# dasongli1/Shift-Net

Hardware: AMD Instinct MI355X
Metric: restored frames/sec at 1280x720 T=16 bf16 (higher is better)
Workload: dtype bf16; 1 GPU; Shift-Net-s (gshift_deblur2), 1280x720, one_len=16 (T_in=20), one window per GPU, synthetic checkpoint; parallelism=clip-parallel x1, gsts_schedule=unit-major, one stream

## Files before the change

include/shiftnet_hip.h:

```cpp
#ifndef SHIFTNET_HIP_H
#define SHIFTNET_HIP_H
#include <stdint.h>

#ifdef __cplusplus
extern "C" {
#endif

#define SN_ABI_VERSION 20

#define SN_F32 0
#define SN_F16 1
#define SN_BF16 2

int sn_abi_version(void);

int sn_selftest_mfma(const float* a, const float* b, float* d, void* stream);

int sn_ingest(const void* src, int src_dtype, const void* noise, void* dst, int T, int C, int H, int W, void* stream);

typedef struct sn_conv_desc {
    const void* in[3];
    int n_in;
    int cs_in;
    int T, h_in, w_in;
    int in_mode;
    int k, stride, pad;
    int h_out, w_out;
    const void* wfrag;
    int mt, ks;
    const float* bias;
    int act;
    float prelu;
    const void* res;
    void* out;
    int cs_out;
    int out_mode;
    int c_out;
    int nchw_dtype;
    const void* sc;
    int sc_dtype;
    float* pool;
    const float* oscale;
    int oscale_stride;
    const void* res2;
    int flags;
    int clip_n, clip_T, clip_lo;
} sn_conv_desc;
#define SN_CONV_TILE_KERNEL 1
int sn_conv2d(const sn_conv_desc* d, void* stream);
int sn_conv_pool_blocks(const sn_conv_desc* d);
#define SN_CONV_K_GENERIC 1
#define SN_CONV_K_FAST    2
#define SN_CONV_K_STATS   3
#define SN_CONV_K_STREAM  4
#define SN_CONV_ROUTE(kernel, mt, a, d, mode, rl) (((kernel) << 24) | ((mt) << 20) | ((a) << 12) | ((d) << 8) | ((mode) << 4) | (rl))
int sn_conv2d_route(const sn_conv_desc* d, int lines_len, int ncu, int* plan);

int sn_upsample2_add(const void* lo, const void* res, void* out, int T, int hs, int ws, int cs, void* stream);

int sn_ca_mlp(const float* partial, int nblk, int cpad, int c, int cr, float inv_hw,
              const float* wa, const float* wb, float* ca, int T, unsigned* bad, void* stream);

int sn_cab_ca_scratch_floats(int T);
int sn_cab_ca(const float* partial, int nblk, int cpad, const void* mid, int cs, int c, int cr, int h, int w,
              const float* w2, const float* wa, const float* wb, float* scratch, float* ca, int T, void* stream);
int sn_cab_fused_supported(const sn_conv_desc* conv1, const sn_conv_desc* conv2);
int sn_cab_stats(const sn_conv_desc* conv1, int lines_len, void* stream);
int sn_cab_ca_lines(const float* partial, int nblk, int cpad, const void* lines, int lines_len, int cs, int c, int cr, int h, int w,
                    const float* w2, const float* wa, const float* wb, float* scratch, float* ca, int T, void* stream);
int sn_cab_fused(const sn_conv_desc* conv1, const sn_conv_desc* conv2, int tile_rows, void* stream);

int sn32_cab_ca(const float* partial, int nblk, int cpad, const float* mid, int c, int cr, int h, int w,
                const float* w2, const float* wa, const float* wb, float* scratch, float* ca, int T, void* stream);

typedef struct sn_unit_src {
    const void* x;
    int T, h, w, C;
    int mode;
    int wrap;
    const void* halo;
    int t0, nt;
    int clip;
} sn_unit_src;

int sn_gsts_gather(const sn_unit_src* s, const int8_t* offs, void* u, void* stream);

int sn_temporal_roll(const sn_unit_src* s, void* y, void* stream);

int sn_gsts_shiftconv(const sn_unit_src* s, const int8_t* offs, const uint32_t* w1, void* hw, void* stream);
int sn_gsts_shiftconv_mfma(const sn_unit_src* s, const int8_t* offs, const uint32_t* w1, void* hw, void* stream);

int sn_ln_gemm_gate(const sn_unit_src* s, const void* hw, const void* wfrag, const float* bias, const uint32_t* wdw,
                    void* g1, float* pool, int g1_blocked, void* stream);
int sn_lngate_blocks(int h, int w);

int sn_grp5_gemm_gate(const void* g1, const float* ca_in, const void* wgrp, const void* wfrag, void* g2, float* pool,
                      int T, int h, int w, int C, void* stream);
int sn_grp5_blocks(int h, int w);

int sn_planar_pitch(int w);
int sn_nhwc_to_planar(const void* x, void* xp, int T, int h, int w, int C, void* stream);

int sn_dw5m_blocks(int h, int w);
int sn_dw5m_gemm_gate(const void* g1p, const float* ca_in, const void* ttab, const void* wfrag, void* g2, float* pool,
                      int T, int h, int w, int C, void* stream);

typedef struct sn_phase1_weights {
    const void* wfrag1;
    const uint32_t* w3;
    const void* wgrp;
    const void* wfrag2;
} sn_phase1_weights;
typedef struct sn_se_fold {
    const float* wa;
    const float* wb;
    int c, cr;
    unsigned* ticket;
    float* ca;
    unsigned* bad;
} sn_se_fold;
typedef struct sn_phase1_opts {
    const float* g1_scale;
    int g1_sums;
    int team;
    void* g1_store;
} sn_phase1_opts;
int sn_phase1_pool_blocks(int T, int h, int w);
int sn_phase1_g1_store_bytes(int T, int h, int w, int C, long long* bytes);
int sn_gsts_cab2_phase1(const sn_unit_src* s, const void* hw, const sn_phase1_weights* wt, void* g2, float* pool, const sn_se_fold* se,
                        const sn_phase1_opts* opt, void* stream);
int sn_cab1_phase1(const sn_unit_src* s, const sn_phase1_weights* wt, void* g2, float* pool, const sn_se_fold* se, const sn_phase1_opts* opt, void* stream);
int sn_p1r_plan(int nfr, int h, int w, int ncu, int team, int* out7);
int sn_p1r_strip_begin(const int* plan7, int s, int w);

int sn_gsts_cab2_phase2(const sn_unit_src* s, const void* g2, const float* ca, const void* wfrag, const float* bias, void* y, void* stream);
int sn_cab1_phase2(const sn_unit_src* s, const void* g2, const float* ca, const void* wfrag, const float* bias, void* y, void* stream);

int sn_cab2_phase2_cab1_phase1_supported(const sn_unit_src* s);
int sn_cab2_phase2_cab1_phase1(const sn_unit_src* s, const void* g2_in, const float* ca, const void* wfrag, const float* bias, void* y,
                               const sn_phase1_weights* wt, void* g2, float* pool, const sn_se_fold* se, const sn_phase1_opts* opt, void* stream);


typedef struct sn32_conv_desc {
    const float* in[3];
    int c_in[3];
    int cs_in[3];
    int n_in;
    int T, h_in, w_in;
    int in_mode;
    int k, stride, pad, groups;
    int h_out, w_out, c_out;
    const float* w;
    const float* bias;
    int act; float prelu;
    const float* oscale; int oscale_stride;
    const float* res; int cs_res;
    void* out; int cs_out;
    int out_mode;
    int nchw_dtype; const void* sc;
    const void* wsplit;
    const float* iscale; int iscale_stride;
    const float* rscale; int rscale_stride;
    const float* ln_w; const float* ln_b;
    float* csum; int csum_cpad;
    int clip_n, clip_T, clip_lo;
} sn32_conv_desc;
int sn32_conv_csum_tiles(int h_out, int w_out);
int sn32_conv2d(const sn32_conv_desc* d, void* stream);
#define SN32_K_1X1      1
#define SN32_K_SPLIT    2
#define SN32_K_SPLIT_G8 3
#define SN32_K_EXACT    4
#define SN32_K_DW       5
#define SN32_K_DIRECT   6
#define SN32_ROUTE(kernel, a, b) (((kernel) << 16) | ((a) << 8) | (b))
int sn32_conv2d_route(const sn32_conv_desc* d);
int sn32_gsts_gather(const sn_unit_src* s, const int8_t* offs, float* u, float* u2, void* stream);
int sn32_gsts_shiftconv(const sn_unit_src* s, const int8_t* offs, const float* w, float* vin, float* u, void* stream);
int sn32_layernorm(const float* x, int cs_x, int K, const float* w, const float* b, float* out, int cs_out, long long npix, void* stream);
int sn32_gate(const float* a, int C, int mode, float* out, long long npix, void* stream);
int sn32_gate_sum(const float* a, int C, int cpad, int mode, float* out, int T, int hw, int nblk, float* partial, void* stream);
int sn32_conv1x1_gate2(const float* x, int cs_x, int cin, const void* wsplit, int C, int cpad, float* out, int T, int hw, float* partial, void* stream);
int sn32_dw_gate(const float* a, int cs_a, const float* w, int C, int cpad, float* out, int T, int h, int wd, int nblk, float* partial, void* stream);
int sn32_chan_sum(const float* x, int cs, int C, int cpad, int T, int hw, int nblk, float* partial, void* stream);
int sn32_scale_residual(const float* r, const float* x, const float* ca, int ca_stride, float* out, int T, int hw, int C, void* stream);
int sn32_ingest(const void* src, int src_dtype, const void* noise, float* dst, int T, int C, int H, int W, void* stream);


int sn_ingest_u8(const uint8_t* src, void* dst, int dst_dtype, int T, int H, int W, void* stream);
int sn_egress_blocks(void);
int sn_egress_u8(const void* out, int out_dtype, const uint8_t* gt, uint8_t* img, float* sse, int T, int H, int W, void* stream);
int sn_ssim_blocks(void);
int sn_ssim_u8(const void* out, int out_dtype, const uint8_t* gt, float* scratch, float* partial, int T, int H, int W, void* stream);

#define SN_YUV_444 0
#define SN_YUV_420_CENTER 1
#define SN_YUV_420_LEFT 2
#define SN_YUV_BT601 0
#define SN_YUV_BT709 1
#define SN_YUV_LIMITED 0
#define SN_YUV_FULL 1
typedef struct sn_yuv_fmt {
    int bits;
    int chroma;
    int matrix;
    int range;
} sn_yuv_fmt;
int sn_ingest_yuv(const uint8_t* src, const sn_yuv_fmt* fmt, void* dst, int dst_dtype, int T, int H, int W, int Hp, int Wp, void* stream);
int sn_egress_yuv(const void* out, int out_dtype, const sn_yuv_fmt* fmt, uint8_t* dst, int T, int H, int W, int Hp, int Wp, void* stream);

int sn_yuv_thumb(const uint8_t* src, const sn_yuv_fmt* fmt, uint16_t* dst, int T, int H, int W, void* stream);

int sn_yuv_noise_hist(const uint8_t* src, const sn_yuv_fmt* fmt, uint32_t* dst, int lo, int hi, int T, int H, int W, void* stream);

#ifdef __cplusplus
}
#endif
#endif
```

shift-net_amd/csrc/sn_common.h:

```cpp
#pragma once
#include <hip/hip_runtime.h>
#include <hip/hip_fp16.h>
#include <stdint.h>

typedef __bf16 bf16x8_t __attribute__((ext_vector_type(8)));
typedef __bf16 bf16x2_t __attribute__((ext_vector_type(2)));
typedef float f32x4_t __attribute__((ext_vector_type(4)));
typedef float f32x2_t __attribute__((ext_vector_type(2)));
typedef uint16_t bf16_t;

#define SN_OK 0
#define SN_EINVAL (-22)
#define SN_ELAUNCH (-5)

__device__ __forceinline__ float bf_lo(uint32_t u) { return __uint_as_float(u << 16); }
__device__ __forceinline__ float bf_hi(uint32_t u) { return __uint_as_float(u & 0xffff0000u); }
__device__ __forceinline__ float bf_to_f(bf16_t h) { return __uint_as_float(((uint32_t)h) << 16); }

__device__ __forceinline__ uint32_t pack_bf2(float lo, float hi) {
    f32x2_t v = {lo, hi};
    bf16x2_t h = __builtin_convertvector(v, bf16x2_t);
    return __builtin_bit_cast(uint32_t, h);
}
typedef _Float16 h2_t __attribute__((ext_vector_type(2)));
__device__ __forceinline__ uint32_t pack_h2(float lo, float hi) {
    const h2_t h = {(_Float16)lo, (_Float16)hi};
    return __builtin_bit_cast(uint32_t, h);
}
__device__ __forceinline__ bf16_t f_to_bf(float f) { return (bf16_t)(pack_bf2(f, 0.f) & 0xffffu); }

__device__ __forceinline__ void unpack8(const uint4 q, float* v) {
    v[0] = bf_lo(q.x); v[1] = bf_hi(q.x); v[2] = bf_lo(q.y); v[3] = bf_hi(q.y);
    v[4] = bf_lo(q.z); v[5] = bf_hi(q.z); v[6] = bf_lo(q.w); v[7] = bf_hi(q.w);
}
__device__ __forceinline__ uint4 pack8(const float* v) {
    uint4 q;
    q.x = pack_bf2(v[0], v[1]); q.y = pack_bf2(v[2], v[3]); q.z = pack_bf2(v[4], v[5]); q.w = pack_bf2(v[6], v[7]);
    return q;
}
__device__ __forceinline__ bf16x8_t as_frag(const uint4 q) { return __builtin_bit_cast(bf16x8_t, q); }

__device__ __forceinline__ f32x4_t mfma16(const bf16x8_t a, const bf16x8_t b, const f32x4_t c) {
    return __builtin_amdgcn_mfma_f32_16x16x32_bf16(a, b, c, 0, 0, 0);
}

__device__ __forceinline__ float dot2bf(uint32_t a, uint32_t b, float acc) {
    return __builtin_amdgcn_fdot2_f32_bf16(__builtin_bit_cast(bf16x2_t, a), __builtin_bit_cast(bf16x2_t, b), acc, false);
}

__device__ __forceinline__ float sigmoidf_(float x) { return __builtin_amdgcn_rcpf(1.0f + __expf(-x)); }

template <int CTRL> __device__ __forceinline__ float dpp_mov(float x) {
    return __builtin_bit_cast(float, __builtin_amdgcn_update_dpp(0, __builtin_bit_cast(int, x), CTRL, 0xf, 0xf, true));
}
template <int CTRL> __device__ __forceinline__ int dpp_movi(int x) { return __builtin_amdgcn_update_dpp(0, x, CTRL, 0xf, 0xf, true); }
__device__ __forceinline__ float row_sum16(float x) {
    x += dpp_mov<0xB1>(x);
    x += dpp_mov<0x4E>(x);
    x += dpp_mov<0x141>(x);
    x += dpp_mov<0x140>(x);
    return x;
}

__device__ __forceinline__ float sum_rows4(float x) {
    float a = x, b = x;
    asm volatile("s_nop 1\n\tv_permlane16_swap_b32 %0, %1" : "+v"(a), "+v"(b));
    const float s = a + b;
    float c = s, d = s;
    asm volatile("s_nop 1\n\tv_permlane32_swap_b32 %0, %1" : "+v"(c), "+v"(d));
    return c + d;
}

#define SN_FRAME_RANGE(s, T0, NT) const int T0 = (s)->nt > 0 ? (s)->t0 : 0, NT = (s)->nt > 0 ? (s)->nt : (s)->T; \
    if (T0 < 0 || NT < 1 || T0 + NT > (s)->T || !sn_clip_ok((s)->T, (s)->clip, (s)->wrap)) return SN_EINVAL
static inline bool sn_clip_ok(int T, int clip, int wrap) { return clip == 0 || (clip > 0 && T % clip == 0 && wrap != 2); }
static inline int sn_clip_len(int T, int clip) { return clip > 0 ? clip : T; }
template <typename E> struct SnSlabs { const E* p0; const E* p1; const E* pb; int s0, s1, sb; };
template <typename E>
__device__ __forceinline__ SnSlabs<E> sn_unit_slabs(const E* x, const E* halo, int T, int hw, int C, int mode, int wrap, int clip, int t) {
    if (clip < T) {
        const int base = t / clip * clip;
        x += (ptrdiff_t)base * hw * C; t -= base; T = clip;
    }
    const int Ch = C >> 1;
    const E* xt = x + (ptrdiff_t)t * hw * C;
    SnSlabs<E> s;
    s.p0 = xt; s.p1 = xt + Ch; s.pb = xt; s.s0 = s.s1 = s.sb = C;
    if (mode == 1) {
        if (t > 0 || wrap == 1) { s.p0 = x + (ptrdiff_t)(t > 0 ? t - 1 : T - 1) * hw * C + Ch; s.p1 = xt; s.pb = s.p0; }
        else if (wrap == 2) { s.p0 = halo; s.s0 = Ch; s.p1 = xt; s.pb = halo; s.sb = Ch; }
        else s.pb = xt;
    } else if (mode == 2) {
        if (t < T - 1 || wrap == 1) { s.p0 = xt + Ch; s.p1 = x + (ptrdiff_t)(t < T - 1 ? t + 1 : 0) * hw * C; s.pb = s.p1; }
        else if (wrap == 2) { s.p0 = xt + Ch; s.p1 = halo; s.s1 = Ch; s.pb = halo; s.sb = Ch; }
        else s.pb = xt + Ch;
    }
    return s;
}

__host__ __device__ __forceinline__ int sn_remap_frame(int t, int n, int T, int lo) {
    if (n == 0) return t;
    const int q = t / n;
    return q * T + lo + (t - q * n);
}
static inline bool sn_remap_set(int n, int T, int lo) { return n != 0 || T != 0 || lo != 0; }
static inline bool sn_remap_ok(int Tout, int n, int T, int lo) { return !sn_remap_set(n, T, lo) || (n > 0 && lo >= 0 && lo + n <= T && Tout % n == 0); }

struct SeFold { const float* wa; const float* wb; float* ca; unsigned* ticket; unsigned* bad; float inv_hw; int c, cr; };
__device__ __forceinline__ void sn_flag_nonfinite(unsigned* bad, float v) {
    if (bad && !(fabsf(v) <= 3.0e38f)) __hip_atomic_store(bad, 1u, __ATOMIC_RELAXED, __HIP_MEMORY_SCOPE_AGENT);
}
__device__ __forceinline__ void sn_pool_store(float* p, float v) { __hip_atomic_store(p, v, __ATOMIC_RELAXED, __HIP_MEMORY_SCOPE_AGENT); }
__device__ __forceinline__ void sn_se_tail(const SeFold& S, const float* pool_t, int nblk, int narrive, int cpad, int t, float* lds, int tid, int nthreads) {
    asm volatile("s_waitcnt vmcnt(0)" ::: "memory");
    __syncthreads();
    unsigned* flag = (unsigned*)lds;
    if (tid == 0) *flag = __hip_atomic_fetch_add(S.ticket + t, 1u, __ATOMIC_RELAXED, __HIP_MEMORY_SCOPE_AGENT) == (unsigned)(narrive - 1) ? 1u : 0u;
    __syncthreads();
    if (!*flag) return;
    if (tid == 0) {
        __builtin_amdgcn_fence(__ATOMIC_ACQUIRE, "agent");
        __hip_atomic_store(S.ticket + t, 0u, __ATOMIC_RELAXED, __HIP_MEMORY_SCOPE_AGENT);
    }
    __syncthreads();
    const int nq = cpad >> 2, parts = nthreads / nq, cq = tid % nq, part = tid / nq;
    float* acc = lds + 16; float* mean = acc + parts * cpad; float* hid = mean + 128;
    if (part < parts) {
        float s0 = 0.f, s1 = 0.f, s2 = 0.f, s3 = 0.f;
#pragma unroll 4
        for (int b = part; b < nblk; b += parts) {
            const float* r = pool_t + (size_t)b * cpad + 4 * cq;
            s0 += __hip_atomic_load(r, __ATOMIC_RELAXED, __HIP_MEMORY_SCOPE_AGENT);
            s1 += __hip_atomic_load(r + 1, __ATOMIC_RELAXED, __HIP_MEMORY_SCOPE_AGENT);
            s2 += __hip_atomic_load(r + 2, __ATOMIC_RELAXED, __HIP_MEMORY_SCOPE_AGENT);
            s3 += __hip_atomic_load(r + 3, __ATOMIC_RELAXED, __HIP_MEMORY_SCOPE_AGENT);
        }
        float* a = acc + part * cpad + 4 * cq;
        a[0] = s0; a[1] = s1; a[2] = s2; a[3] = s3;
    }
    __syncthreads();
    if (tid < cpad) {
        float m = 0.f;
        for (int q = 0; q < parts; ++q) m += acc[q * cpad + tid];
        sn_flag_nonfinite(S.bad, m);
        mean[tid] = m * S.inv_hw;
    }
    __syncthreads();
    if (tid < S.cr) {
        float hsum = 0.f;
        for (int j = 0; j < S.c; ++j) hsum += S.wa[tid * S.c + j] * mean[j];
        hid[tid] = hsum > 0.f ? hsum : 0.f;
    }
    __syncthreads();
    if (tid < cpad) {
        float o = 0.f;
        if (tid < S.c) {
            for (int j = 0; j < S.cr; ++j) o += S.wb[tid * S.cr + j] * hid[j];
            o = sigmoidf_(o);
        }
        S.ca[(size_t)t * cpad + tid] = o;
    }
}

__device__ __forceinline__ int wave_id() { return __builtin_amdgcn_readfirstlane((int)(threadIdx.x >> 6)); }

#ifndef SN_XCD_TILES
#define SN_XCD_TILES 1
#endif
struct XcdTiles { int ntx, nty, nrf, chunk; uint32_t inv_nty; };
static inline XcdTiles sn_xcd_tiles(int ntx, int nty, int T) {
    XcdTiles g; g.ntx = ntx; g.nty = nty; g.nrf = nty * T;
    g.chunk = SN_XCD_TILES ? (g.nrf + 7) / 8 : g.nrf;
    g.inv_nty = nty > 1 ? (uint32_t)((0x100000000ull + (uint32_t)nty - 1) / (uint32_t)nty) : 0u;
    return g;
}
static inline dim3 sn_xcd_grid(const XcdTiles& g) { return SN_XCD_TILES ? dim3(8u * g.ntx, g.chunk, 1) : dim3(g.ntx, g.nrf, 1); }
__host__ __device__ inline bool sn_xcd_decode(const XcdTiles& g, uint32_t bx, uint32_t by, int& t, int& ty, int& tx) {
#if SN_XCD_TILES
    tx = (int)(bx >> 3);
    const uint32_t rf = (bx & 7) * (uint32_t)g.chunk + by;
#else
    tx = (int)bx;
    const uint32_t rf = by;
#endif
    if (rf >= (uint32_t)g.nrf) return false;
    t = g.inv_nty ? (int)(((uint64_t)rf * g.inv_nty) >> 32) : (int)rf;
    ty = (int)rf - t * g.nty;
    return true;
}
__device__ __forceinline__ bool sn_xcd_tile(const XcdTiles& g, int& t, int& ty, int& tx) {
    return sn_xcd_decode(g, blockIdx.x, blockIdx.y, t, ty, tx);
}

static inline void sn_clear_error() { (void)hipGetLastError(); }
static inline int sn_check_launch() {
    hipError_t e = hipGetLastError();
    return e == hipSuccess ? SN_OK : SN_ELAUNCH;
}
```

shift-net_amd/csrc/sn_conv.hip:

```cpp
#include "sn_common.h"
#include "../../include/shiftnet_hip.h"

int sn_conv3p_key(const sn_conv_desc* d, bool want_pool);
int sn_conv3p_pool_rows(const sn_conv_desc* d);
int sn_conv3p_route(const sn_conv_desc* d, int lines_len, int ncu, int* plan8);
int sn_conv3p_launch(const sn_conv_desc* d, int lines_len, int route, const int* plan8, void* stream);

namespace {

struct ConvK {
    const bf16_t* in0; const bf16_t* in1; const bf16_t* in2;
    int n_in, cs, cv;
    int hin, win, in_mode, k, stride, pad, hout, wout;
    const uint4* wfrag; int ks;
    const float* bias; int act; float prelu;
    const bf16_t* res; bf16_t* out; int cs_out, out_mode, c_out, nchw_dtype, sc_dtype;
    const void* sc; float* pool; const float* oscale; int oscale_stride; const bf16_t* res2;
    int rh, rw, ps;
    int clip_n, clip_T, clip_lo;
    int lines_len;
    XcdTiles xg;
    unsigned m_nblk8, m_rw, m_csb, m_cv, m_k;
};

constexpr __host__ __device__ int sn_lds_slots(int npb) {
    const int k = npb <= 2 ? 2 : 4 * ((npb - 2 + 3) / 4) + 2;
    return k <= npb + 1 ? k : ((npb & 1) ? npb : npb + 1);
}

__device__ __forceinline__ int fdiv(int x, unsigned magic) { return (int)(((unsigned)x * (unsigned long long)magic) >> 24); }

__device__ __forceinline__ uint4 ld_bilinear(const bf16_t* src, int t, int hs, int ws, int cs, int cb, int gy, int gx) {
    float sy = gy * 0.5f - 0.25f; if (sy < 0.f) sy = 0.f;
    float sx = gx * 0.5f - 0.25f; if (sx < 0.f) sx = 0.f;
    int y0 = (int)sy, x0 = (int)sx;
    int y1 = min(y0 + 1, hs - 1), x1 = min(x0 + 1, ws - 1);
    float ly = sy - y0, lx = sx - x0, hy = 1.f - ly, hx = 1.f - lx;
    const bf16_t* b = src + (size_t)t * hs * ws * cs + cb * 8;
    float v00[8], v01[8], v10[8], v11[8], o[8];
    unpack8(*(const uint4*)(b + ((size_t)y0 * ws + x0) * cs), v00);
    unpack8(*(const uint4*)(b + ((size_t)y0 * ws + x1) * cs), v01);
    unpack8(*(const uint4*)(b + ((size_t)y1 * ws + x0) * cs), v10);
    unpack8(*(const uint4*)(b + ((size_t)y1 * ws + x1) * cs), v11);
#pragma unroll
    for (int j = 0; j < 8; ++j) o[j] = hy * (hx * v00[j] + lx * v01[j]) + ly * (hx * v10[j] + lx * v11[j]);
    return pack8(o);
}

constexpr int sn_conv_waves(int mt) {
    return mt == 1 ? 6 : mt == 2 ? 5 : mt == 3 ? 4 : mt == 4 ? 3 : 2;
}
constexpr int sn_conv3_waves(int mt, int cs) {
    return mt == 1 ? 7 : mt == 2 ? 6 : mt == 3 ? (cs == 48 ? 3 : 4) : mt == 4 ? 3 : 2;
}

template <int MT, int TH, int TW>
__global__ __launch_bounds__(256, sn_conv_waves(MT)) void conv_mfma_kernel(const ConvK P) {
    extern __shared__ __attribute__((aligned(16))) char smem[];
    constexpr int NTW = (TH * TW) / 64;
    constexpr int XB = TW / 16;
    const int tid = threadIdx.x, lane = tid & 63, wv = wave_id();
    const int g = lane >> 4, p = lane & 15;
    int t, tyi, txi;
    if (!sn_xcd_tile(P.xg, t, tyi, txi)) return;
    const int ti = sn_remap_frame(t, P.clip_n, P.clip_T, P.clip_lo);
    const int oy0 = tyi * TH, ox0 = txi * TW;
    const int tile_bytes = P.rh * P.rw * P.ps;
    int* tapoff = (int*)(smem + tile_bytes);
    float* red = (float*)(smem + tile_bytes + ((P.ks * 4 * 4 + 15) & ~15));

    for (int e = tid; e < P.ks * 4; e += 256) {
        const int kk0 = e * 8, K = P.k * P.k * P.cv;
        int off = 0;
        if (kk0 < K) {
            const int tap = fdiv(kk0, P.m_cv), cc0 = kk0 - tap * P.cv;
            const int dy = fdiv(tap, P.m_k), dx = tap - dy * P.k;
            off = (dy * P.rw + dx) * P.ps + cc0 * 2;
        }
        tapoff[e] = off;
    }
    {
        const int nblk8 = P.cv >> 3, csb = P.cs >> 3, total = P.rh * P.rw * nblk8;
        const int iy0 = oy0 * P.stride - P.pad, ix0 = ox0 * P.stride - P.pad;
        for (int idx0 = tid; idx0 < total; idx0 += 4 * 256) {
            uint4 v[4];
            int dst[4];
#pragma unroll
            for (int u = 0; u < 4; ++u) {
                const int idx = idx0 + u * 256;
                const int idc = idx < total ? idx : tid;
                const int pix = fdiv(idc, P.m_nblk8), blk = idc - pix * nblk8;
                const int ry = fdiv(pix, P.m_rw), rx = pix - ry * P.rw;
                const int ii = fdiv(blk, P.m_csb), cb = blk - ii * csb;
                const bf16_t* src = ii == 0 ? P.in0 : (ii == 1 ? P.in1 : P.in2);
                const int gy = iy0 + ry, gx = ix0 + rx;
                const bool in = gy >= 0 && gy < P.hin && gx >= 0 && gx < P.win;
                dst[u] = idx < total ? (in ? pix * P.ps + blk * 16 : -(pix * P.ps + blk * 16) - 1) : 0x7fffffff;
                if (P.in_mode == 0) v[u] = *(const uint4*)(src + (in ? (((size_t)ti * P.hin + gy) * P.win + gx) * P.cs + cb * 8 : 0));
                else v[u] = in ? ld_bilinear(src, ti, P.hin >> 1, P.win >> 1, P.cs, cb, gy, gx) : make_uint4(0, 0, 0, 0);
            }
#pragma unroll
            for (int u = 0; u < 4; ++u) {
                if (dst[u] == 0x7fffffff) continue;
                const bool in = dst[u] >= 0;
                *(uint4*)(smem + (in ? dst[u] : -(dst[u] + 1))) = in ? v[u] : make_uint4(0, 0, 0, 0);
            }
        }
    }
    bf16x8_t a_cur[MT];
#pragma unroll
    for (int m = 0; m < MT; ++m) a_cur[m] = as_frag(P.wfrag[(m * P.ks) * 64 + lane]);
    __syncthreads();

    f32x4_t acc[MT][NTW];
#pragma unroll
    for (int m = 0; m < MT; ++m)
#pragma unroll
        for (int n = 0; n < NTW; ++n) acc[m][n] = (f32x4_t){0.f, 0.f, 0.f, 0.f};
    int pixbase[NTW];
#pragma unroll
    for (int n = 0; n < NTW; ++n) {
        const int nn = wv * NTW + n, row = nn / XB, xb = nn - row * XB;
        pixbase[n] = ((row * P.stride) * P.rw + (xb * 16 + p) * P.stride) * P.ps;
    }
    constexpr bool PRE_RES = MT == 1;
    uint2 rres[PRE_RES ? MT : 1][PRE_RES ? NTW : 1];
    if constexpr (PRE_RES) {
        const bf16_t* rb = P.res ? P.res : (const bf16_t*)P.wfrag;
#pragma unroll
        for (int n = 0; n < NTW; ++n) {
            const int nn = wv * NTW + n, row = nn / XB, xb = nn - row * XB;
            const int oy = oy0 + row, ox = ox0 + xb * 16 + p;
            const bool valid = P.res && (oy < P.hout) && (ox < P.wout);
            const size_t opix = ((size_t)t * P.hout + oy) * P.wout + ox;
#pragma unroll
            for (int m = 0; m < MT; ++m) {
                const int co0 = g * 4 * MT + m * 4;
                rres[m][n] = *(const uint2*)(rb + ((valid && co0 < P.cs_out) ? opix * P.cs_out + co0 : 0));
            }
        }
    }
    for (int s = 0; s < P.ks; ++s) {
        const int toff = tapoff[s * 4 + g];
        const int sn = s + 1 < P.ks ? s + 1 : s;
        bf16x8_t a_nxt[MT];
#pragma unroll
        for (int m = 0; m < MT; ++m) a_nxt[m] = as_frag(P.wfrag[(m * P.ks + sn) * 64 + lane]);
        bf16x8_t b[NTW];
#pragma unroll
        for (int n = 0; n < NTW; ++n) b[n] = as_frag(*(const uint4*)(smem + pixbase[n] + toff));
#pragma unroll
        for (int m = 0; m < MT; ++m)
#pragma unroll
            for (int n = 0; n < NTW; ++n) acc[m][n] = mfma16(a_cur[m], b[n], acc[m][n]);
#pragma unroll
        for (int m = 0; m < MT; ++m) a_cur[m] = a_nxt[m];
    }

    float psum[MT][4];
#pragma unroll
    for (int m = 0; m < MT; ++m)
#pragma unroll
        for (int r = 0; r < 4; ++r) psum[m][r] = 0.f;

    float4 bia[MT], osc[MT];
#pragma unroll
    for (int m = 0; m < MT; ++m) {
        const int co0 = g * 4 * MT + m * 4;
        bia[m] = P.bias ? *(const float4*)(P.bias + co0) : make_float4(0.f, 0.f, 0.f, 0.f);
        osc[m] = P.oscale ? *(const float4*)(P.oscale + (size_t)t * P.oscale_stride + co0) : make_float4(1.f, 1.f, 1.f, 1.f);
    }
#pragma unroll
    for (int n = 0; n < NTW; ++n) {
        const int nn = wv * NTW + n, row = nn / XB, xb = nn - row * XB;
        const int oy = oy0 + row, ox = ox0 + xb * 16 + p;
        const bool valid = (oy < P.hout) && (ox < P.wout);
        const size_t opix = ((size_t)t * P.hout + oy) * P.wout + ox;
        uint2 shuf[MT];
#pragma unroll
        for (int m = 0; m < MT; ++m) {
            const int co0 = g * 4 * MT + m * 4;
            float v[4] = {acc[m][n][0], acc[m][n][1], acc[m][n][2], acc[m][n][3]};
            v[0] += bia[m].x; v[1] += bia[m].y; v[2] += bia[m].z; v[3] += bia[m].w;
            if (P.act == 1) {
#pragma unroll
                for (int r = 0; r < 4; ++r) v[r] = v[r] >= 0.f ? v[r] : v[r] * P.prelu;
            }
            v[0] *= osc[m].x; v[1] *= osc[m].y; v[2] *= osc[m].z; v[3] *= osc[m].w;
            if constexpr (PRE_RES) {
                if (P.res && valid && co0 < P.cs_out) {
                    const uint2 rr = rres[m][n];
                    v[0] += bf_lo(rr.x); v[1] += bf_hi(rr.x); v[2] += bf_lo(rr.y); v[3] += bf_hi(rr.y);
                }
            } else if (P.res && valid && co0 < P.cs_out) {
                const uint2 rr = *(const uint2*)(P.res + opix * P.cs_out + co0);
                v[0] += bf_lo(rr.x); v[1] += bf_hi(rr.x); v[2] += bf_lo(rr.y); v[3] += bf_hi(rr.y);
            }
            if (P.res2 && valid && co0 < P.cs_out) {
                const uint2 rr = *(const uint2*)(P.res2 + opix * P.cs_out + co0);
                v[0] += bf_lo(rr.x); v[1] += bf_hi(rr.x); v[2] += bf_lo(rr.y); v[3] += bf_hi(rr.y);
            }
            if (valid) {
#pragma unroll
                for (int r = 0; r < 4; ++r) psum[m][r] += v[r];
                if (P.out_mode == 0) {
                    if (co0 < P.cs_out) {
                        uint2 o; o.x = pack_bf2(v[0], v[1]); o.y = pack_bf2(v[2], v[3]);
                        *(uint2*)(P.out + opix * P.cs_out + co0) = o;
                    }
                } else if (P.out_mode == 1) {
                    shuf[m].x = pack_bf2(v[0], v[1]); shuf[m].y = pack_bf2(v[2], v[3]);
                } else {
#pragma unroll
                    for (int r = 0; r < 4; ++r) {
                        const int co = co0 + r;
                        if (co < P.c_out) {
                            const size_t oi = (((size_t)t * P.c_out + co) * P.hout + oy) * P.wout + ox;
                            const float scv = P.sc_dtype == SN_F32 ? ((const float*)P.sc)[oi]
                                            : (P.sc_dtype == SN_F16 ? __half2float(((const __half*)P.sc)[oi]) : bf_to_f(((const bf16_t*)P.sc)[oi]));
                            if (P.nchw_dtype == SN_F32) ((float*)P.out)[oi] = v[r] + scv;
                            else if (P.nchw_dtype == SN_F16) ((__half*)P.out)[oi] = __float2half(v[r] + scv);
                            else ((bf16_t*)P.out)[oi] = f_to_bf(v[r] + scv);
                        }
                    }
                }
            }
        }
        if (P.out_mode == 1 && valid) {
            bf16_t* dst = P.out + (((size_t)t * 2 * P.hout + 2 * oy + (g >> 1)) * (2 * P.wout) + 2 * ox + (g & 1)) * P.cs_out;
#pragma unroll
            for (int m = 0; m + 1 < MT; m += 2) *(uint4*)(dst + m * 4) = make_uint4(shuf[m].x, shuf[m].y, shuf[m + 1].x, shuf[m + 1].y);
            if constexpr (MT & 1) *(uint2*)(dst + (MT - 1) * 4) = shuf[MT - 1];
        }
    }

    if (P.pool) {
#pragma unroll
        for (int m = 0; m < MT; ++m)
#pragma unroll
            for (int r = 0; r < 4; ++r) {
                float s = psum[m][r];
                s = row_sum16(s);
                if (p == 0) red[wv * 16 * MT + g * 4 * MT + m * 4 + r] = s;
            }
        __syncthreads();
        if (tid < 16 * MT) {
            const float s = red[tid] + red[16 * MT + tid] + red[2 * 16 * MT + tid] + red[3 * 16 * MT + tid];
            const int nblk = P.xg.ntx * P.xg.nty, blk = tyi * P.xg.ntx + txi;
            P.pool[((size_t)t * nblk + blk) * (16 * MT) + tid] = s;
        }
    }
}

template <int MT, int CS, int TH, bool STATS = false>
__global__ __launch_bounds__(256, sn_conv3_waves(MT, CS)) void conv3_fast_kernel(const ConvK P) {
    extern __shared__ __attribute__((aligned(16))) char smem[];
    constexpr int TW = 32, RH = TH + 2, RW = TW + 2, NPB = CS / 8;
    constexpr int PS = 16 * sn_lds_slots(NPB);
    constexpr int KTOT = 9 * CS, KS = (KTOT + 31) / 32;
    constexpr int NTW = (TH * TW) / 64, XB = TW / 16;
    constexpr int ROWP = RW * NPB, NITEM = RH * ROWP, NIT = (NITEM + 255) / 256;
    constexpr int TILE_BYTES = RH * RW * PS;
    const int tid = threadIdx.x & 255, lane = tid & 63, wv = wave_id();
    const int g = lane >> 4, p = lane & 15;
    int t, tyi, txi;
    if (!sn_xcd_tile(P.xg, t, tyi, txi)) return;
    const int oy0 = tyi * TH, ox0 = txi * TW;
    float* red = (float*)(smem + TILE_BYTES);

    {
        const int iy0 = oy0 - 1, ix0 = ox0 - 1;
        const bf16_t* inb = P.in0 + (size_t)t * P.hin * P.win * CS;
        const bool interior = iy0 >= 0 && iy0 + RH <= P.hin && ix0 >= 0 && ix0 + RW <= P.win;
        uint4 v[NIT];
        if (interior) {
#pragma unroll
            for (int k = 0; k < NIT; ++k) {
                const int idx = tid + k * 256, idc = idx < NITEM ? idx : NITEM - 1;
                const int r = idc / ROWP, i = idc - r * ROWP;
                v[k] = *(const uint4*)(inb + ((size_t)iy0 * P.win + ix0) * CS + (size_t)r * P.win * CS + i * 8);
            }
#pragma unroll
            for (int k = 0; k < NIT; ++k) {
                const int idx = tid + k * 256;
                const int r = idx / ROWP, i = idx - r * ROWP, px = i / NPB, blk = i - px * NPB;
                if (idx < NITEM) *(uint4*)(smem + (r * RW + px) * PS + blk * 16) = v[k];
            }
        } else {
            bool in[NIT];
#pragma unroll
            for (int k = 0; k < NIT; ++k) {
                const int idx = tid + k * 256, idc = idx < NITEM ? idx : NITEM - 1;
                const int r = idc / ROWP, i = idc - r * ROWP, px = i / NPB, blk = i - px * NPB;
                const int gy = iy0 + r, gx = ix0 + px;
                in[k] = gy >= 0 && gy < P.hin && gx >= 0 && gx < P.win;
                v[k] = *(const uint4*)(inb + (in[k] ? ((size_t)gy * P.win + gx) * CS + blk * 8 : 0));
            }
#pragma unroll
            for (int k = 0; k < NIT; ++k) {
                const int idx = tid + k * 256;
                const int r = idx / ROWP, i = idx - r * ROWP, px = i / NPB, blk = i - px * NPB;
                if (idx < NITEM) *(uint4*)(smem + (r * RW + px) * PS + blk * 16) = in[k] ? v[k] : make_uint4(0, 0, 0, 0);
            }
        }
    }

    const bool full = (oy0 + TH <= P.hout) && (ox0 + TW <= P.wout);
    const size_t tbase = (((size_t)t * P.hout + oy0) * P.wout + ox0) * P.cs_out;
    bf16_t* const outb = P.out + tbase;
    const bf16_t* const resb = P.res ? P.res + tbase : nullptr;
    const bf16_t* const res2b = P.res2 ? P.res2 + tbase : nullptr;
    const int c0 = g * 4 * MT;
    int loff[NTW];
    bool valid[NTW];
#pragma unroll
    for (int n = 0; n < NTW; ++n) {
        const int nn = wv * NTW + n, row = nn / XB, xb = nn - row * XB;
        loff[n] = (row * P.wout + xb * 16 + p) * P.cs_out + c0;
        valid[n] = full || ((oy0 + row < P.hout) && (ox0 + xb * 16 + p < P.wout));
    }
    constexpr bool PRE_RES = MT == 1;
    uint2 rres[PRE_RES ? NTW : 1];
    if constexpr (PRE_RES) {
        const bf16_t* rb = resb ? resb : (const bf16_t*)P.wfrag;
#pragma unroll
        for (int n = 0; n < NTW; ++n) rres[n] = *(const uint2*)(rb + ((resb && valid[n] && c0 < P.cs_out) ? loff[n] : 0));
    }
    __syncthreads();

    f32x4_t acc[MT][NTW];
#pragma unroll
    for (int m = 0; m < MT; ++m) {
        const float4 b4 = P.bias ? *(const float4*)(P.bias + c0 + m * 4) : make_float4(0.f, 0.f, 0.f, 0.f);
#pragma unroll
        for (int n = 0; n < NTW; ++n) acc[m][n] = (f32x4_t){b4.x, b4.y, b4.z, b4.w};
    }
    int pixbase[NTW];
#pragma unroll
    for (int n = 0; n < NTW; ++n) {
        const int nn = wv * NTW + n, row = nn / XB, xb = nn - row * XB;
        pixbase[n] = (row * RW + xb * 16 + p) * PS;
    }
#pragma unroll
    for (int s = 0; s < KS; ++s) {
        int toff = 0;
#pragma unroll
        for (int gg = 0; gg < 4; ++gg) {
            const int kk0 = (s * 4 + gg) * 8;
            const int tap = kk0 / CS, cc0 = kk0 - tap * CS, dy = tap / 3, dx = tap - dy * 3;
            const int o = kk0 < KTOT ? (dy * RW + dx) * PS + cc0 * 2 : 0;
            toff = g == gg ? o : toff;
        }
        bf16x8_t a[MT];
#pragma unroll
        for (int m = 0; m < MT; ++m) a[m] = as_frag(P.wfrag[(m * KS + s) * 64 + lane]);
        bf16x8_t b[NTW];
#pragma unroll
        for (int n = 0; n < NTW; ++n) b[n] = as_frag(*(const uint4*)(smem + pixbase[n] + toff));
#pragma unroll
        for (int m = 0; m < MT; ++m)
#pragma unroll
            for (int n = 0; n < NTW; ++n) acc[m][n] = mfma16(a[m], b[n], acc[m][n]);
    }

    float psum[MT][4];
#pragma unroll
    for (int m = 0; m < MT; ++m)
#pragma unroll
        for (int r = 0; r < 4; ++r) psum[m][r] = 0.f;
    float4 osc[MT];
    const bool has_osc = P.oscale != nullptr;
#pragma unroll
    for (int m = 0; m < MT; ++m)
        osc[m] = has_osc ? *(const float4*)(P.oscale + (size_t)t * P.oscale_stride + c0 + m * 4) : make_float4(1.f, 1.f, 1.f, 1.f);
    const float slope = P.prelu;
    const int act = P.act != 1 ? 0 : ((slope >= 0.f && slope <= 1.f) ? 1 : 2);
#pragma unroll
    for (int n = 0; n < NTW; ++n) {
        float v[MT][4];
#pragma unroll
        for (int m = 0; m < MT; ++m) {
            v[m][0] = acc[m][n][0]; v[m][1] = acc[m][n][1]; v[m][2] = acc[m][n][2]; v[m][3] = acc[m][n][3];
            if (act == 1) {
#pragma unroll
                for (int r = 0; r < 4; ++r) v[m][r] = fmaxf(v[m][r], slope * v[m][r]);
            } else if (act == 2) {
#pragma unroll
                for (int r = 0; r < 4; ++r) v[m][r] = fmaf(slope, fminf(v[m][r], 0.f), fmaxf(v[m][r], 0.f));
            }
            if (has_osc) { v[m][0] *= osc[m].x; v[m][1] *= osc[m].y; v[m][2] *= osc[m].z; v[m][3] *= osc[m].w; }
        }
        const bool ok = valid[n];
        if constexpr (PRE_RES) {
            if (resb && ok && c0 < P.cs_out) {
                const uint2 rr = rres[n];
                v[0][0] += bf_lo(rr.x); v[0][1] += bf_hi(rr.x); v[0][2] += bf_lo(rr.y); v[0][3] += bf_hi(rr.y);
            }
        }
        if (ok) {
            const bf16_t* rp[2] = {PRE_RES ? nullptr : resb, res2b};
#pragma unroll
            for (int q = 0; q < 2; ++q) {
                if (!rp[q]) continue;
                const bf16_t* src = rp[q] + loff[n];
                if constexpr (MT == 2 || MT == 4) {
#pragma unroll
                    for (int m = 0; m < MT; m += 2) {
                        if (c0 + m * 4 < P.cs_out) {
                            const uint4 rr = *(const uint4*)(src + m * 4);
                            v[m][0] += bf_lo(rr.x); v[m][1] += bf_hi(rr.x); v[m][2] += bf_lo(rr.y); v[m][3] += bf_hi(rr.y);
                            v[m + 1][0] += bf_lo(rr.z); v[m + 1][1] += bf_hi(rr.z); v[m + 1][2] += bf_lo(rr.w); v[m + 1][3] += bf_hi(rr.w);
                        }
                    }
                } else {
#pragma unroll
                    for (int m = 0; m < MT; ++m) {
                        if (c0 + m * 4 < P.cs_out) {
                            const uint2 rr = *(const uint2*)(src + m * 4);
                            v[m][0] += bf_lo(rr.x); v[m][1] += bf_hi(rr.x); v[m][2] += bf_lo(rr.y); v[m][3] += bf_hi(rr.y);
                        }
                    }
                }
            }
            bf16_t* dst = outb + loff[n];
            if (P.pool) {
#pragma unroll
                for (int m = 0; m < MT; ++m)
#pragma unroll
                    for (int r = 0; r < 4; ++r) psum[m][r] += v[m][r];
            }
            if constexpr (STATS) {
                const int nn = wv * NTW + n, row = nn / XB, xb = nn - row * XB;
                const int oy = oy0 + row, ox = ox0 + xb * 16 + p;
                bf16_t* const lb = P.out + (size_t)t * 4 * P.lines_len * P.cs_out + c0;
                bf16_t* tgt[4] = {oy == 0 ? lb + (size_t)ox * P.cs_out : nullptr,
                                  oy == P.hout - 1 ? lb + ((size_t)P.lines_len + ox) * P.cs_out : nullptr,
                                  ox == 0 ? lb + ((size_t)2 * P.lines_len + oy) * P.cs_out : nullptr,
                                  ox == P.wout - 1 ? lb + ((size_t)3 * P.lines_len + oy) * P.cs_out : nullptr};
#pragma unroll
                for (int q = 0; q < 4; ++q) {
                    if (!tgt[q]) continue;
#pragma unroll
                    for (int m = 0; m < MT; ++m)
                        if (c0 + m * 4 < P.cs_out) {
                            uint2 o; o.x = pack_bf2(v[m][0], v[m][1]); o.y = pack_bf2(v[m][2], v[m][3]);
                            *(uint2*)(tgt[q] + m * 4) = o;
                        }
                }
                continue;
            }
            if constexpr (MT == 2 || MT == 4) {
#pragma unroll
                for (int m = 0; m < MT; m += 2)
                    if (c0 + m * 4 < P.cs_out)
                        *(uint4*)(dst + m * 4) = make_uint4(pack_bf2(v[m][0], v[m][1]), pack_bf2(v[m][2], v[m][3]),
                                                            pack_bf2(v[m + 1][0], v[m + 1][1]), pack_bf2(v[m + 1][2], v[m + 1][3]));
            } else {
#pragma unroll
                for (int m = 0; m < MT; ++m)
                    if (c0 + m * 4 < P.cs_out) {
                        uint2 o; o.x = pack_bf2(v[m][0], v[m][1]); o.y = pack_bf2(v[m][2], v[m][3]);
                        *(uint2*)(dst + m * 4) = o;
                    }
            }
        }
    }
    if (P.pool) {
#pragma unroll
        for (int m = 0; m < MT; ++m)
#pragma unroll
            for (int r = 0; r < 4; ++r) {
                float sm = psum[m][r];
                sm = row_sum16(sm);
                if (p == 0) red[wv * 16 * MT + g * 4 * MT + m * 4 + r] = sm;
            }
        __syncthreads();
        if (tid < 16 * MT) {
            const float sm = red[tid] + red[16 * MT + tid] + red[2 * 16 * MT + tid] + red[3 * 16 * MT + tid];
            const int nblk = P.xg.ntx * P.xg.nty, blk = tyi * P.xg.ntx + txi;
            P.pool[((size_t)t * nblk + blk) * (16 * MT) + tid] = sm;
        }
    }
}


template <int MT, int CS, bool STATS = false>
int launch_conv3_fast(const ConvK& K, int T, hipStream_t st) {
    constexpr int TH = 8, TW = 32, NPB = CS / 8, PS = 16 * sn_lds_slots(NPB);
    ConvK P = K; P.xg = sn_xcd_tiles((K.wout + TW - 1) / TW, (K.hout + TH - 1) / TH, T);
    const dim3 grid = sn_xcd_grid(P.xg);
    const size_t lds = (size_t)(TH + 2) * (TW + 2) * PS + 4 * 16 * MT * sizeof(float);
    if (lds > 64 * 1024) {
        if (hipFuncSetAttribute((const void*)conv3_fast_kernel<MT, CS, TH, STATS>, hipFuncAttributeMaxDynamicSharedMemorySize, (int)lds) != hipSuccess)
            return SN_ELAUNCH;
    }
    hipLaunchKernelGGL((conv3_fast_kernel<MT, CS, TH, STATS>), grid, dim3(256), lds, st, P);
    return sn_check_launch();
}

size_t conv_generic_lds(int th, int tw, int stride, int k, int ps, int ks, int mt) {
    return (size_t)((th - 1) * stride + k) * ((tw - 1) * stride + k) * ps + ((ks * 16 + 15) & ~15) + 4 * 16 * mt * sizeof(float);
}

template <int TH, int TW>
int launch_conv(const ConvK& K, int mt, int T, hipStream_t st) {
    const int rh = (TH - 1) * K.stride + K.k, rw = (TW - 1) * K.stride + K.k;
    ConvK P = K; P.rh = rh; P.rw = rw;
    P.xg = sn_xcd_tiles((K.wout + TW - 1) / TW, (K.hout + TH - 1) / TH, T);
    const dim3 grid = sn_xcd_grid(P.xg);
    auto magic = [](int d) { return (unsigned)(((1u << 24) + d - 1) / d); };
    P.m_nblk8 = magic(P.cv >> 3); P.m_rw = magic(rw); P.m_csb = magic(P.cs >> 3); P.m_cv = magic(P.cv); P.m_k = magic(P.k);
    const size_t lds = conv_generic_lds(TH, TW, K.stride, K.k, P.ps, P.ks, mt);
#define SN_CONV_CASE(M) case M: \
        if (lds > 64 * 1024 && hipFuncSetAttribute((const void*)conv_mfma_kernel<M, TH, TW>, hipFuncAttributeMaxDynamicSharedMemorySize, (int)lds) != hipSuccess) return SN_ELAUNCH; \
        hipLaunchKernelGGL((conv_mfma_kernel<M, TH, TW>), grid, dim3(256), lds, st, P); break;
    switch (mt) {
        SN_CONV_CASE(1) SN_CONV_CASE(2) SN_CONV_CASE(3) SN_CONV_CASE(4) SN_CONV_CASE(5) SN_CONV_CASE(6)
        default: return SN_EINVAL;
    }
#undef SN_CONV_CASE
    return sn_check_launch();
}

__global__ void ingest_kernel(const void* src, int dt, const void* noise, uint4* dst, int C, int HW) {
    const int t = blockIdx.y;
    const int i = blockIdx.x * blockDim.x + threadIdx.x;
    if (i >= HW) return;
    float v[8] = {0, 0, 0, 0, 0, 0, 0, 0};
    for (int c = 0; c < C; ++c) {
        const size_t idx = ((size_t)t * C + c) * HW + i;
        v[c] = dt == SN_F32 ? ((const float*)src)[idx] : (dt == SN_F16 ? __half2float(((const __half*)src)[idx]) : bf_to_f(((const bf16_t*)src)[idx]));
    }
    if (noise) {
        const size_t idx = (size_t)t * HW + i;
        v[C] = dt == SN_F32 ? ((const float*)noise)[idx] : (dt == SN_F16 ? __half2float(((const __half*)noise)[idx]) : bf_to_f(((const bf16_t*)noise)[idx]));
    }
    dst[(size_t)t * HW + i] = pack8(v);
}

__global__ __launch_bounds__(1024) void ca_mlp_kernel(const float* partial, int nblk, int cpad, int c, int cr, float inv_hw,
                                                   const float* wa, const float* wb, float* ca, unsigned* bad) {
    __shared__ float acc[1024];
    __shared__ float mean[128];
    __shared__ float hid[128];
    const int t = blockIdx.x, tid = threadIdx.x;
    const int nsplit = 1024 / cpad;
    const int ch = tid % cpad, part = tid / cpad;
    float s = 0.f;
    if (part < nsplit) {
        const float* pp = partial + (size_t)t * nblk * cpad + ch;
        for (int b = part; b < nblk; b += nsplit) s += pp[(size_t)b * cpad];
    }
    acc[tid] = s;
    __syncthreads();
    if (tid < cpad) {
        float m = 0.f;
        for (int q = 0; q < nsplit; ++q) m += acc[q * cpad + tid];
        sn_flag_nonfinite(bad, m);
        mean[tid] = m * inv_hw;
    }
    __syncthreads();
    if (tid < cr) {
        float h = 0.f;
        for (int j = 0; j < c; ++j) h += wa[tid * c + j] * mean[j];
        hid[tid] = h > 0.f ? h : 0.f;
    }
    __syncthreads();
    if (tid < cpad) {
        float o = 0.f;
        if (tid < c) {
            for (int j = 0; j < cr; ++j) o += wb[tid * cr + j] * hid[j];
            o = sigmoidf_(o);
        }
        ca[(size_t)t * cpad + tid] = o;
    }
}

#define SN_CABCA_NS 16
__device__ __forceinline__ float cab_ldf(const bf16_t* p) { return bf_to_f(*p); }
__device__ __forceinline__ float cab_ldf(const float* p) { return *p; }
template <typename E>
__device__ __forceinline__ const E* cab_px(const E* mt, int L, int w, int cs, int line, int y, int x) {
    return L > 0 ? mt + ((size_t)line * L + (line < 2 ? x : y)) * cs : mt + ((size_t)y * w + x) * cs;
}
template <typename E>
__global__ __launch_bounds__(256) void cab_ca_part_kernel(const float* partial, int nblk, int cpad, const E* mid, int cs,
                                                        int h, int w, float* scratch, int L) {
    __shared__ float acc[256];
    const int t = blockIdx.y, sidx = blockIdx.x, tid = threadIdx.x;
    const E* mt = mid + (L > 0 ? (size_t)t * 4 * L * cs : (size_t)t * h * w * cs);
    float* out = scratch + ((size_t)t * SN_CABCA_NS + sidx) * 5 * 128;
    {
        const int nsplit = 256 / cpad, ch = tid % cpad, part = tid / cpad;
        float sm = 0.f;
        if (part < nsplit) {
            const float* pp = partial + (size_t)t * nblk * cpad + ch;
            for (int bb = sidx * nsplit + part; bb < nblk; bb += SN_CABCA_NS * nsplit) sm += pp[(size_t)bb * cpad];
        }
        acc[tid] = sm;
        __syncthreads();
        if (tid < cpad) {
            float m = 0.f;
            for (int q = 0; q < nsplit; ++q) m += acc[q * cpad + tid];
            if (tid < 128) out[tid] = m;
        }
        __syncthreads();
    }
    for (int line = 0; line < 4; ++line) {
        const int len = line < 2 ? w : h;
        const int nseg = 256 / cs, ch = tid % cs, seg = tid / cs;
        float sm = 0.f;
        if (seg < nseg)
            for (int i = sidx * nseg + seg; i < len; i += SN_CABCA_NS * nseg) {
                const int y = line == 0 ? 0 : (line == 1 ? h - 1 : i), x = line == 2 ? 0 : (line == 3 ? w - 1 : i);
                sm += cab_ldf(cab_px(mt, L, w, cs, line, y, x) + ch);
            }
        acc[tid] = sm;
        __syncthreads();
        if (tid < cs) {
            float m = 0.f;
            for (int q = 0; q < nseg; ++q) m += acc[q * cs + tid];
            out[(1 + line) * 128 + tid] = m;
        }
        __syncthreads();
    }
}

template <typename E>
__global__ __launch_bounds__(1024) void cab_ca_kernel(const float* scratch, int cpad, const E* mid, int cs, int c, int cr,
                                                     int h, int w, const float* w2, const float* wa, const float* wb, float* ca, int L) {
    __shared__ float acc[1024];
    __shared__ float S[9][128];
    __shared__ float mean[128];
    __shared__ float hid[128];
    const int t = blockIdx.x, tid = threadIdx.x;
    const E* mt = mid + (L > 0 ? (size_t)t * 4 * L * cs : (size_t)t * h * w * cs);
    if (tid < 5 * 128) {
        const int k = tid >> 7, ch = tid & 127;
        float m = 0.f;
        if (ch < (k == 0 ? cpad : cs)) {
            const float* sp = scratch + (size_t)t * SN_CABCA_NS * 5 * 128 + tid;
            for (int q = 0; q < SN_CABCA_NS; ++q) m += sp[q * 5 * 128];
        }
        S[k][ch] = m;
    }
    if (tid < cs) {
        S[5][tid] = cab_ldf(cab_px(mt, L, w, cs, 0, 0, 0) + tid);
        S[6][tid] = cab_ldf(cab_px(mt, L, w, cs, 0, 0, w - 1) + tid);
        S[7][tid] = cab_ldf(cab_px(mt, L, w, cs, 1, h - 1, 0) + tid);
        S[8][tid] = cab_ldf(cab_px(mt, L, w, cs, 1, h - 1, w - 1) + tid);
    }
    __syncthreads();
    {
        const int nsplit = 1024 / cpad, co = tid % cpad, part = tid / cpad;
        float r = 0.f;
        if (part < nsplit)
            for (int cin = part; cin < c; cin += nsplit) {
                const float tot = S[0][cin], r0 = S[1][cin], r1 = S[2][cin], c0 = S[3][cin], c1 = S[4][cin];
                const float k00 = S[5][cin], k01 = S[6][cin], k10 = S[7][cin], k11 = S[8][cin];
                const float* wk = w2 + (size_t)cin * 9 * cpad + co;
                const float rowex[3] = {r1, 0.f, r0}, colex[3] = {c1, 0.f, c0};
                const float cor[3][3] = {{k11, 0.f, k10}, {0.f, 0.f, 0.f}, {k01, 0.f, k00}};
#pragma unroll
                for (int ky = 0; ky < 3; ++ky)
#pragma unroll
                    for (int kx = 0; kx < 3; ++kx) r += wk[(ky * 3 + kx) * cpad] * (tot - rowex[ky] - colex[kx] + cor[ky][kx]);
            }
        acc[tid] = r;
        __syncthreads();
        if (tid < cpad) {
            float m = 0.f;
            for (int q = 0; q < nsplit; ++q) m += acc[q * cpad + tid];
            if (tid < 128) mean[tid] = m / ((float)h * (float)w);
        }
    }
    __syncthreads();
    if (tid < cr) {
        float hh = 0.f;
        for (int j = 0; j < c; ++j) hh += wa[tid * c + j] * mean[j];
        hid[tid] = hh > 0.f ? hh : 0.f;
    }
    __syncthreads();
    if (tid < cpad) {
        float o = 0.f;
        if (tid < c) {
            for (int j = 0; j < cr; ++j) o += wb[tid * cr + j] * hid[j];
            o = sigmoidf_(o);
        }
        ca[(size_t)t * cpad + tid] = o;
    }
}

__global__ void selftest_mfma_kernel(const float* a, const float* b, float* d) {
    const int lane = threadIdx.x, g = lane >> 4, m = lane & 15;
    float av[8], bv[8];
#pragma unroll
    for (int j = 0; j < 8; ++j) {
        av[j] = a[m * 32 + g * 8 + j];
        bv[j] = b[(g * 8 + j) * 16 + m];
    }
    f32x4_t acc = {0.f, 0.f, 0.f, 0.f};
    acc = mfma16(as_frag(pack8(av)), as_frag(pack8(bv)), acc);
#pragma unroll
    for (int r = 0; r < 4; ++r) d[(g * 4 + r) * 16 + m] = acc[r];
}

__global__ __launch_bounds__(256) void upsample2_add_kernel(const bf16_t* __restrict__ lo, const bf16_t* __restrict__ res, bf16_t* __restrict__ out,
                                                            int hs, int ws, int npb) {
    const int w2 = 2 * ws, cs = npb * 8, i = (int)blockIdx.y, t = (int)blockIdx.z;
    const int e = (int)blockIdx.x * 256 + (int)threadIdx.x;
    if (e >= w2 * npb) return;
    const int x = e / npb, piece = e - x * npb;
    float sx = x * 0.5f - 0.25f; if (sx < 0.f) sx = 0.f;
    const int x0 = (int)sx, x1 = min(x0 + 1, ws - 1);
    const float lx = sx - x0, hx = 1.f - lx;
    const int ra = max(i - 1, 0), rc = min(i + 1, hs - 1);
    const bf16_t* b = lo + (size_t)t * hs * ws * cs + piece * 8;
    const uint4 qa0 = *(const uint4*)(b + ((size_t)ra * ws + x0) * cs), qa1 = *(const uint4*)(b + ((size_t)ra * ws + x1) * cs);
    const uint4 qb0 = *(const uint4*)(b + ((size_t)i * ws + x0) * cs), qb1 = *(const uint4*)(b + ((size_t)i * ws + x1) * cs);
    const uint4 qc0 = *(const uint4*)(b + ((size_t)rc * ws + x0) * cs), qc1 = *(const uint4*)(b + ((size_t)rc * ws + x1) * cs);
    const size_t o0 = (((size_t)t * 2 * hs + 2 * i) * w2 + x) * cs + piece * 8, o1 = o0 + (size_t)w2 * cs;
    const uint4 r0 = *(const uint4*)(res + o0), r1 = *(const uint4*)(res + o1);
    float a0[8], a1[8], b0[8], b1[8], c0[8], c1[8], f0[8], f1[8], u0[8], u1[8];
    unpack8(qa0, a0); unpack8(qa1, a1); unpack8(qb0, b0); unpack8(qb1, b1); unpack8(qc0, c0); unpack8(qc1, c1); unpack8(r0, f0); unpack8(r1, f1);
    const float ly0 = i > 0 ? 0.75f : 0.f, hy0 = 1.f - ly0;
#pragma unroll
    for (int j = 0; j < 8; ++j) {
        const float va = hx * a0[j] + lx * a1[j], vb = hx * b0[j] + lx * b1[j], vc = hx * c0[j] + lx * c1[j];
        u0[j] = (hy0 * va + ly0 * vb) + f0[j];
        u1[j] = (0.75f * vb + 0.25f * vc) + f1[j];
    }
    *(uint4*)(out + o0) = pack8(u0);
    *(uint4*)(out + o1) = pack8(u1);
}

}

extern "C" {

int sn_abi_version(void) { return SN_ABI_VERSION; }

int sn_selftest_mfma(const float* a, const float* b, float* d, void* stream) {
    sn_clear_error();
    hipLaunchKernelGGL(selftest_mfma_kernel, dim3(1), dim3(64), 0, (hipStream_t)stream, a, b, d);
    return sn_check_launch();
}

int sn_ingest(const void* src, int dt, const void* noise, void* dst, int T, int C, int H, int W, void* stream) {
    sn_clear_error();
    if (!src || !dst || C < 1 || C + (noise ? 1 : 0) > 8 || dt < 0 || dt > 2) return SN_EINVAL;
    const int hw = H * W;
    hipLaunchKernelGGL(ingest_kernel, dim3((hw + 255) / 256, T), dim3(256), 0, (hipStream_t)stream, src, dt, noise, (uint4*)dst, C, hw);
    return sn_check_launch();
}

static int conv3_key(const sn_conv_desc* d) {
    if (!(d->k == 3 && d->stride == 1 && d->pad == 1 && d->in_mode == 0 && d->out_mode == 0 && d->n_in == 1 && d->ks == (9 * d->cs_in + 31) / 32)) return 0;
    const int key = d->mt * 1000 + d->cs_in;
    return (key == 1016 || key == 2024 || key == 4064 || key == 3040 || key == 3048 || key == 5080) ? key : 0;
}
static void conv_tile(const sn_conv_desc* d, int* th, int* tw) {
    if (d->stride == 1) { *tw = 32; *th = 8; }
    else if (d->n_in * d->cs_in <= 24 && !(d->flags & (1 << 15))) { *th = 8; *tw = 32; }
    else { *th = 4; *tw = 16; }
}

int sn_conv_pool_blocks(const sn_conv_desc* d) {
    if (!d) return SN_EINVAL;
    if (!(d->flags & SN_CONV_TILE_KERNEL)) {
        const int rows = sn_conv3p_pool_rows(d);
        if (rows > 0) return rows;
    }
    int th, tw; conv_tile(d, &th, &tw);
    return ((d->h_out + th - 1) / th) * ((d->w_out + tw - 1) / tw);
}

static int conv_ps(const sn_conv_desc* d) {
    const int blocks = d->n_in * d->cs_in >> 3;
    return d->stride == 1 ? 16 * sn_lds_slots(blocks) : ((blocks & 1) ? blocks * 16 : blocks * 16 + 16);
}

static int conv_route(const sn_conv_desc* d, int lines_len, int ncu, int* plan8) {
    if (!d) return SN_EINVAL;
    const bool stream_ok = !(d->flags & SN_CONV_TILE_KERNEL);
    if (lines_len > 0) {
        if (!d->out || !d->pool || !d->wfrag || !d->in[0] || d->res || d->res2 || d->oscale || d->cs_in != d->cs_out ||
            sn_remap_set(d->clip_n, d->clip_T, d->clip_lo)) return SN_EINVAL;
        if (lines_len < (d->h_out > d->w_out ? d->h_out : d->w_out) || d->h_out < 2 || d->w_out < 2) return SN_EINVAL;
        if (stream_ok) {
            const int r = sn_conv3p_route(d, lines_len, ncu, plan8);
            if (r >= 0) return r;
        }
        const int key = conv3_key(d);
        if (key != 1016 && key != 2024) return SN_EINVAL;
        return SN_CONV_ROUTE(SN_CONV_K_STATS, key / 1000, key % 1000, 0, 0, 0);
    }
    if (d->n_in < 1 || d->n_in > 3 || (d->cs_in & 7) || (d->cs_out & 7) || !d->wfrag) return SN_EINVAL;
    if (!d->out) return SN_EINVAL;
    if (d->k < 1 || d->k > 5 || (d->stride != 1 && d->stride != 2) || d->mt < 1 || d->mt > 6 || d->ks < 1) return SN_EINVAL;
    if (d->in_mode == 1 && ((d->h_in | d->w_in) & 1)) return SN_EINVAL;
    if (d->out_mode == 2 && (!d->sc || d->c_out > 4 * d->mt || d->nchw_dtype < 0 || d->nchw_dtype > 2 || d->sc_dtype < 0 || d->sc_dtype > 2)) return SN_EINVAL;
    if (d->ks * 32 < d->k * d->k * d->n_in * d->cs_in) return SN_EINVAL;
    if (d->oscale && d->oscale_stride < 16 * d->mt) return SN_EINVAL;
    if ((d->res || d->res2) && d->out_mode != 0) return SN_EINVAL;
    if (d->out_mode == 1 && d->cs_out != 4 * d->mt) return SN_EINVAL;
    const bool remap = sn_remap_set(d->clip_n, d->clip_T, d->clip_lo);
    if (!sn_remap_ok(d->T, d->clip_n, d->clip_T, d->clip_lo) || (remap && (conv3_key(d) || (stream_ok && sn_conv3p_key(d, false)))))
        return SN_EINVAL;
    if (stream_ok && sn_conv3p_key(d, false)) {
        const int r = sn_conv3p_route(d, 0, ncu, plan8);
        if (r >= 0) return r;
    }
    const int key = conv3_key(d);
    if (key) return SN_CONV_ROUTE(SN_CONV_K_FAST, key / 1000, key % 1000, 0, 0, 0);
    int th, tw; conv_tile(d, &th, &tw);
    if (conv_generic_lds(th, tw, d->stride, d->k, conv_ps(d), d->ks, d->mt) > 160 * 1024) return SN_EINVAL;
    return SN_CONV_ROUTE(SN_CONV_K_GENERIC, d->mt, th, 0, 0, 0);
}

int sn_conv2d_route(const sn_conv_desc* d, int lines_len, int ncu, int* plan) {
    sn_clear_error();
    return conv_route(d, lines_len, ncu, plan);
}

int sn_conv2d(const sn_conv_desc* d, void* stream) {
    sn_clear_error();
    int plan8[8];
    const int route = conv_route(d, 0, 0, plan8);
    if (route < 0) return route;
    ConvK K;
    K.in0 = (const bf16_t*)d->in[0]; K.in1 = (const bf16_t*)d->in[1]; K.in2 = (const bf16_t*)d->in[2];
    K.n_in = d->n_in; K.cs = d->cs_in; K.cv = d->n_in * d->cs_in;
    K.hin = d->h_in; K.win = d->w_in; K.in_mode = d->in_mode; K.k = d->k; K.stride = d->stride; K.pad = d->pad;
    K.hout = d->h_out; K.wout = d->w_out;
    K.wfrag = (const uint4*)d->wfrag; K.ks = d->ks; K.bias = d->bias; K.act = d->act; K.prelu = d->prelu;
    K.res = (const bf16_t*)d->res; K.out = (bf16_t*)d->out; K.cs_out = d->cs_out; K.out_mode = d->out_mode;
    K.c_out = d->c_out; K.nchw_dtype = d->nchw_dtype; K.sc_dtype = d->sc_dtype; K.sc = d->sc; K.pool = d->pool; K.oscale = d->oscale; K.oscale_stride = d->oscale_stride; K.res2 = (const bf16_t*)d->res2;
    K.ps = conv_ps(d);
    K.rh = K.rw = 0; K.lines_len = 0;
    K.clip_n = d->clip_n; K.clip_T = d->clip_T; K.clip_lo = d->clip_lo;
    hipStream_t st = (hipStream_t)stream;
    const int mt = (route >> 20) & 15, a = (route >> 12) & 255;
    switch (route >> 24) {
        case SN_CONV_K_STREAM: return sn_conv3p_launch(d, 0, route, plan8, stream);
        case SN_CONV_K_FAST:
            switch (mt * 1000 + a) {
                case 1016: return launch_conv3_fast<1, 16>(K, d->T, st);
                case 2024: return launch_conv3_fast<2, 24>(K, d->T, st);
                case 4064: return launch_conv3_fast<4, 64>(K, d->T, st);
                case 3040: return launch_conv3_fast<3, 40>(K, d->T, st);
                case 3048: return launch_conv3_fast<3, 48>(K, d->T, st);
                case 5080: return launch_conv3_fast<5, 80>(K, d->T, st);
                default: return SN_EINVAL;
            }
        case SN_CONV_K_GENERIC: return a == 8 ? launch_conv<8, 32>(K, mt, d->T, st) : launch_conv<4, 16>(K, mt, d->T, st);
        default: return SN_EINVAL;
    }
}


int sn_ca_mlp(const float* partial, int nblk, int cpad, int c, int cr, float inv_hw,
              const float* wa, const float* wb, float* ca, int T, unsigned* bad, void* stream) {
    sn_clear_error();
    if (!partial || !wa || !wb || !ca || cpad < 16 || cpad > 128 || c > cpad || cr > 128 || cr < 1 || nblk < 1) return SN_EINVAL;
    hipLaunchKernelGGL(ca_mlp_kernel, dim3(T), dim3(1024), 0, (hipStream_t)stream, partial, nblk, cpad, c, cr, inv_hw, wa, wb, ca, bad);
    return sn_check_launch();
}

int sn_cab_ca_scratch_floats(int T) { return T * SN_CABCA_NS * 5 * 128; }

static int cab_ca_launch(const float* partial, int nblk, int cpad, const void* mid, int lines_len, int cs, int c, int cr, int h, int w,
                         const float* w2, const float* wa, const float* wb, float* scratch, float* ca, int T, void* stream) {
    sn_clear_error();
    if (!partial || !mid || !w2 || !wa || !wb || !ca || !scratch || cpad < 16 || cpad > 128 || cs > 128 || (cs & 7) || c > cs ||
        c > cpad || cr < 1 || cr > 128 || nblk < 1 || h < 2 || w < 2 || (lines_len != 0 && lines_len < (h > w ? h : w))) return SN_EINVAL;
    hipLaunchKernelGGL(cab_ca_part_kernel<bf16_t>, dim3(SN_CABCA_NS, T), dim3(256), 0, (hipStream_t)stream, partial, nblk, cpad,
                       (const bf16_t*)mid, cs, h, w, scratch, lines_len);
    hipLaunchKernelGGL(cab_ca_kernel<bf16_t>, dim3(T), dim3(1024), 0, (hipStream_t)stream, (const float*)scratch, cpad, (const bf16_t*)mid, cs,
                       c, cr, h, w, w2, wa, wb, ca, lines_len);
    return sn_check_launch();
}

int sn_cab_ca(const float* partial, int nblk, int cpad, const void* mid, int cs, int c, int cr, int h, int w,
              const float* w2, const float* wa, const float* wb, float* scratch, float* ca, int T, void* stream) {
    return cab_ca_launch(partial, nblk, cpad, mid, 0, cs, c, cr, h, w, w2, wa, wb, scratch, ca, T, stream);
}

int sn_cab_ca_lines(const float* partial, int nblk, int cpad, const void* lines, int lines_len, int cs, int c, int cr, int h, int w,
                    const float* w2, const float* wa, const float* wb, float* scratch, float* ca, int T, void* stream) {
    if (lines_len < 1) return SN_EINVAL;
    return cab_ca_launch(partial, nblk, cpad, lines, lines_len, cs, c, cr, h, w, w2, wa, wb, scratch, ca, T, stream);
}

int sn_cab_stats(const sn_conv_desc* d, int lines_len, void* stream) {
    sn_clear_error();
    if (lines_len < 1) return SN_EINVAL;
    int plan8[8];
    const int route = conv_route(d, lines_len, 0, plan8);
    if (route < 0) return route;
    if ((route >> 24) == SN_CONV_K_STREAM) return sn_conv3p_launch(d, lines_len, route, plan8, stream);
    const int key = ((route >> 20) & 15) * 1000 + ((route >> 12) & 255);
    ConvK K;
    K.in0 = (const bf16_t*)d->in[0]; K.in1 = K.in2 = nullptr;
    K.n_in = 1; K.cs = d->cs_in; K.cv = d->cs_in;
    K.hin = d->h_in; K.win = d->w_in; K.in_mode = 0; K.k = 3; K.stride = 1; K.pad = 1; K.hout = d->h_out; K.wout = d->w_out;
    K.wfrag = (const uint4*)d->wfrag; K.ks = d->ks; K.bias = d->bias; K.act = d->act; K.prelu = d->prelu;
    K.res = nullptr; K.out = (bf16_t*)d->out; K.cs_out = d->cs_out; K.out_mode = 0; K.c_out = d->c_out; K.nchw_dtype = 0; K.sc_dtype = 0; K.sc = nullptr;
    K.pool = d->pool; K.oscale = nullptr; K.oscale_stride = 0; K.res2 = nullptr;
    K.ps = 16 * sn_lds_slots(K.cv >> 3); K.rh = K.rw = 0; K.lines_len = lines_len; K.clip_n = K.clip_T = K.clip_lo = 0;
    hipStream_t st = (hipStream_t)stream;
    return key == 1016 ? launch_conv3_fast<1, 16, true>(K, d->T, st) : launch_conv3_fast<2, 24, true>(K, d->T, st);
}

int sn32_cab_ca(const float* partial, int nblk, int cpad, const float* mid, int c, int cr, int h, int w,
                const float* w2, const float* wa, const float* wb, float* scratch, float* ca, int T, void* stream) {
    sn_clear_error();
    if (!partial || !mid || !w2 || !wa || !wb || !ca || !scratch || cpad < 16 || cpad > 128 || c < 1 || c > cpad || cr < 1 || cr > 128 ||
        nblk < 1 || h < 2 || w < 2) return SN_EINVAL;
    hipLaunchKernelGGL(cab_ca_part_kernel<float>, dim3(SN_CABCA_NS, T), dim3(256), 0, (hipStream_t)stream, partial, nblk, cpad, mid, c, h, w, scratch, 0);
    hipLaunchKernelGGL(cab_ca_kernel<float>, dim3(T), dim3(1024), 0, (hipStream_t)stream, (const float*)scratch, cpad, mid, c, c, cr, h, w, w2, wa, wb, ca, 0);
    return sn_check_launch();
}

}

int sn_upsample2_add(const void* lo, const void* res, void* out, int T, int hs, int ws, int cs, void* stream) {
    sn_clear_error();
    if (!lo || !res || !out || T < 1 || hs < 1 || ws < 1 || cs < 8 || (cs & 7)) return SN_EINVAL;
    if (hs > 65535 || T > 65535 || (long)2 * ws * (cs / 8) > 0x7fffffffL) return SN_EINVAL;
    hipLaunchKernelGGL(upsample2_add_kernel, dim3((unsigned)((2 * ws * (cs / 8) + 255) / 256), (unsigned)hs, (unsigned)T), dim3(256), 0, (hipStream_t)stream,
                       (const bf16_t*)lo, (const bf16_t*)res, (bf16_t*)out, hs, ws, cs / 8);
    return sn_check_launch();
}
```

shift-net_amd/csrc/sn_conv3p.hip:

```cpp
#include "sn_common.h"
#include "../../include/shiftnet_hip.h"

namespace {

typedef __attribute__((address_space(3))) void lds_void_t;

struct C3P {
    const bf16_t* in; const bf16_t* res; bf16_t* out;
    const uint4* wfrag; const float* bias; const float* oscale; int oscale_stride;
    const uint4* w2; const float* b2;
    float* pool; int pool_rows;
    int act; float prelu;
    int T, h, w, ntx, nty;
    int dbg;
    int lines_len;
    int S, nseg, nsg, qs;
};

__device__ __forceinline__ float max_bare(float a, float b) {
    float r;
    asm("v_max_f32 %0, %1, %2" : "=v"(r) : "v"(a), "v"(b));
    return r;
}

__device__ __forceinline__ float mul_then_add(float a, float b, float c) {
    float r;
    asm("v_mul_f32 %0, %1, %2\n\tv_add_f32 %0, %0, %3" : "=&v"(r) : "v"(a), "v"(b), "v"(c));
    return r;
}

__device__ __forceinline__ void dma16(const __amdgpu_buffer_rsrc_t rs, char* dst, int voffset) {
    __builtin_amdgcn_raw_ptr_buffer_load_lds(rs, (lds_void_t*)dst, 16, voffset, 0, 0, 0);
}

template <typename V> __device__ __forceinline__ void pin(V& x) { asm volatile("" : "+v"(x)); }

template <int N> __device__ __forceinline__ void wait_vmcnt() { asm volatile("s_waitcnt vmcnt(%0)" ::"n"(N) : "memory"); }

__device__ __forceinline__ __amdgpu_buffer_rsrc_t frame_rsrc(const bf16_t* base, int frame_bytes) {
    return __builtin_amdgcn_make_buffer_rsrc((void*)base, 0, frame_bytes, 0x00020000);
}

constexpr int c3p_waves(int mt) { return mt == 1 ? 4 : mt == 2 ? 3 : 2; }

template <int MT, int CS, int TH, int D, int MODE, bool RL = false>
__global__ __launch_bounds__(320, c3p_waves(MT)) void conv3p_kernel(const C3P P) {
    extern __shared__ __attribute__((aligned(16))) char smem[];
    constexpr int TW = 32, RH = TH + 2, RW = TW + 2, NPB = CS / 8, PSB = CS * 2;
    constexpr int KTOT = 9 * CS, KS = (KTOT + 31) / 32;
    constexpr int ROWP = RW * NPB, NITEM = RH * ROWP, NDMA = (NITEM + 63) / 64, XBUF = NDMA * 1024;
    static_assert(!RL || MODE == 2, "residual staging belongs to MODE 2");
    constexpr int RDMA = RL ? (TH * TW * NPB) / 64 : 0;
    constexpr int NBUF = D + 1, BUFSZ = XBUF + RDMA * 1024, NL = NDMA + RDMA;
    constexpr bool WLDS = MT * KS > 16;
    constexpr int WBYTES = WLDS ? MT * KS * 1024 : 0;
    constexpr int RPW = TH / 4, NTW = RPW * 2;
    constexpr int NH = MT == 1 ? (NTW < 4 ? NTW : 4) : 2;
    static_assert(NTW % NH == 0 && NTW <= 4 * NH, "passes");
    static_assert(TH % 4 == 0 && NL * (D - 1) <= 63 && D >= 1, "tile / prefetch shape");
    const int lane = threadIdx.x & 63, wv = wave_id();
    const int G = (int)gridDim.x, c = ((int)blockIdx.x & 7) * (G >> 3) + ((int)blockIdx.x >> 3);
    const int fseg = c * P.qs, nsegs = min(P.qs, P.nsg - fseg);
    if (nsegs <= 0) return;
    int t = fseg / (P.ntx * P.nseg), tx, ty, n = 0;
    {
        const int rem = fseg - t * (P.ntx * P.nseg);
        tx = rem / P.nseg;
        const int sg = rem - tx * P.nseg;
        ty = sg * P.S;
        const int tail = P.nty - (P.nseg - 1) * P.S;
        for (int k = 0, g2 = sg; k < nsegs; ++k) { n += g2 == P.nseg - 1 ? tail : P.S; if (++g2 == P.nseg) g2 = 0; }
    }
    n = __builtin_amdgcn_readfirstlane(n);
    t = __builtin_amdgcn_readfirstlane(t); tx = __builtin_amdgcn_readfirstlane(tx); ty = __builtin_amdgcn_readfirstlane(ty);
    const int rowpitch = P.w * PSB, frame_bytes = P.h * rowpitch;
    const size_t frame_elems = (size_t)P.h * P.w * CS;
    char* const xbufs = smem + WBYTES;
    if constexpr (WLDS) {
        for (int i = (int)threadIdx.x; i < MT * KS * 64; i += 320) *(uint4*)(smem + i * 16) = P.wfrag[i];
        __syncthreads();
    }

    if (wv == 4) {
        int voff[NDMA], pxk[NDMA];
#pragma unroll
        for (int k = 0; k < NDMA; ++k) {
            const int i = k * 64 + lane, ic = i < NITEM ? i : NITEM - 1;
            const int r = ic / ROWP, j = ic - r * ROWP;
            voff[k] = r * rowpitch + j * 16;
            pxk[k] = j / NPB;
        }
        int rvoff[RL ? RDMA : 1];
        if constexpr (RL) {
#pragma unroll
            for (int k = 0; k < RDMA; ++k) {
                const int i = k * 64 + lane, row = i / (TW * NPB), rem = i - row * (TW * NPB);
                rvoff[k] = row * rowpitch + rem * 16;
            }
        }
        int ft = t, ftx = tx, fty = ty;
        for (int i = -D; i < n; ++i) {
            if (i >= 0) {
                if (n - 1 - i >= D - 1) wait_vmcnt<NL * (D - 1)>(); else wait_vmcnt<0>();
                __builtin_amdgcn_s_barrier();
            }
            const int j = i + D;
            if (j < n && !(P.dbg & 1)) {
                const __amdgpu_buffer_rsrc_t rs = frame_rsrc(P.in + (size_t)ft * frame_elems, frame_bytes);
                const int ix0 = ftx * TW - 1;
                const int o = ((fty * TH - 1) * P.w + ix0) * PSB;
                const bool edge = ftx == 0 || ix0 + RW > P.w;
                char* const dst = xbufs + (j % NBUF) * BUFSZ;
#pragma unroll
                for (int k = 0; k < NDMA; ++k) {
                    int vo = voff[k] + o;
                    if (edge) { const int gx = ix0 + pxk[k]; vo = (gx < 0 || gx >= P.w) ? (int)0x80000000 : vo; }
                    dma16(rs, dst + k * 1024, vo);
                }
                if constexpr (RL) {
                    const __amdgpu_buffer_rsrc_t rr = frame_rsrc(P.res + (size_t)ft * frame_elems, frame_bytes);
                    const int o2 = ((fty * TH) * P.w + ftx * TW) * PSB;
#pragma unroll
                    for (int k = 0; k < RDMA; ++k)
                        dma16(rr, dst + XBUF + k * 1024, rvoff[k] + o2);
                }
                if (++fty == P.nty) { fty = 0; if (++ftx == P.ntx) { ftx = 0; ++ft; } }
            }
        }
        return;
    }

    const int g = lane >> 4, p = lane & 15;
    const int c0 = g * 4 * MT;
    int addr_s[KS];
    const int lane_base = ((wv * RPW) * RW + p) * PSB;
#pragma unroll
    for (int s = 0; s < KS; ++s) {
        int toff = 0;
#pragma unroll
        for (int gg = 0; gg < 4; ++gg) {
            const int kk0 = (s * 4 + gg) * 8;
            const int tap = kk0 / CS, cc0 = kk0 - tap * CS, dy = tap / 3, dx = tap - dy * 3;
            const int o = kk0 < KTOT ? (dy * RW + dx) * PSB + cc0 * 2 : 0;
            toff = g == gg ? o : toff;
        }
        addr_s[s] = lane_base + toff;
    }
    bf16x8_t A[WLDS ? 1 : MT][WLDS ? 1 : KS];
    if constexpr (!WLDS) {
#pragma unroll
        for (int m = 0; m < MT; ++m)
#pragma unroll
            for (int s = 0; s < KS; ++s) A[m][s] = as_frag(P.wfrag[(m * KS + s) * 64 + lane]);
    }
    const char* const wl = smem + lane * 16;
    f32x4_t biasv[MT];
#pragma unroll
    for (int m = 0; m < MT; ++m) {
        const float4 b4 = P.bias ? *(const float4*)(P.bias + c0 + m * 4) : make_float4(0.f, 0.f, 0.f, 0.f);
        biasv[m] = (f32x4_t){b4.x, b4.y, b4.z, b4.w};
    }
    const float slope = P.prelu;
    float4 osc[MT];
    auto load_osc = [&](int ft) {
        if constexpr (MODE == 2) {
#pragma unroll
            for (int m = 0; m < MT; ++m) osc[m] = *(const float4*)(P.oscale + (size_t)ft * P.oscale_stride + c0 + m * 4);
        }
    };
    load_osc(t);
    auto pin_loaded = [&]() __attribute__((always_inline)) {
        if constexpr (!WLDS) {
#pragma unroll
            for (int m = 0; m < MT; ++m)
#pragma unroll
                for (int s = 0; s < KS; ++s) pin(A[m][s]);
        }
#pragma unroll
        for (int m = 0; m < MT; ++m) {
            pin(biasv[m]);
            if constexpr (MODE == 2) { pin(osc[m].x); pin(osc[m].y); pin(osc[m].z); pin(osc[m].w); }
        }
    };
    pin_loaded();
    constexpr int OOR = (int)0x80000000;
    constexpr int PIECE = (MT == 2 || MT == 4) ? 16 : 8;
    constexpr int NP = (MT * 8) / PIECE;
    typedef unsigned rword_t __attribute__((ext_vector_type(PIECE / 4)));
    int ooff[RPW][NP];
#pragma unroll
    for (int rr = 0; rr < RPW; ++rr)
#pragma unroll
        for (int q = 0; q < NP; ++q)
            ooff[rr][q] = (c0 + q * (PIECE / 2) < CS) ? ((wv * RPW + rr) * P.w + p) * PSB + c0 * 2 + q * PIECE : OOR;
    typedef rword_t rset_t[(MODE == 2 && !RL) ? NTW : 1][(MODE == 2 && !RL) ? NP : 1];
    rset_t rA, rB;
    auto load_res = [&](rset_t& rnxt, int ft, int ftx, int fty) __attribute__((always_inline)) {
        if constexpr (MODE == 2 && !RL) {
            const __amdgpu_buffer_rsrc_t rr = frame_rsrc(P.res + (size_t)ft * frame_elems, frame_bytes);
            const int o2 = ((fty * TH) * P.w + ftx * TW) * PSB;
#pragma unroll
            for (int nn = 0; nn < NTW; ++nn)
#pragma unroll
                for (int q = 0; q < NP; ++q) {
                    const int vo = o2 + ooff[nn >> 1][q] + (nn & 1) * 16 * PSB;
                    if constexpr (PIECE == 16) rnxt[nn][q] = __builtin_amdgcn_raw_buffer_load_b128(rr, vo, 0, 0);
                    else rnxt[nn][q] = __builtin_amdgcn_raw_buffer_load_b64(rr, vo, 0, 0);
                }
        }
    };
    load_res(rA, t, tx, ty);
    float psum[MT][4];
#pragma unroll
    for (int m = 0; m < MT; ++m)
#pragma unroll
        for (int r = 0; r < 4; ++r) psum[m][r] = 0.f;
    auto flush_pool = [&](int ft, int ftx, int fsg) {
        if constexpr (MODE == 1 || MODE == 3) {
            const int row = (ftx * P.nseg + fsg) * 4 + wv;
            float* dst = P.pool + ((size_t)ft * P.pool_rows + row) * (16 * MT);
#pragma unroll
            for (int m = 0; m < MT; ++m)
#pragma unroll
                for (int r = 0; r < 4; ++r) {
                    const float sm = row_sum16(psum[m][r]);
                    if (p == 0) dst[c0 + m * 4 + r] = sm;
                    psum[m][r] = 0.f;
                }
        }
    };

    const int raddr = XBUF + ((wv * RPW) * TW + p) * PSB + c0 * 2;
    auto finish = [&](const f32x4_t (&acc)[MT][NH], const rset_t& rres, const char* xs, const int N0, const __amdgpu_buffer_rsrc_t ro, int o2, const bool MASKED,
                      int ylim, int xlim) __attribute__((always_inline)) {
#pragma unroll
        for (int nh = 0; nh < NH; ++nh) {
            const int nn = N0 + nh, rr = nn >> 1, xb = nn & 1;
            float v[MT][4];
#pragma unroll
            for (int m = 0; m < MT; ++m) {
                v[m][0] = acc[m][nh][0]; v[m][1] = acc[m][nh][1]; v[m][2] = acc[m][nh][2]; v[m][3] = acc[m][nh][3];
                if constexpr (MODE == 1 || MODE == 3) {
#pragma unroll
                    for (int r = 0; r < 4; ++r) {
                        v[m][r] = max_bare(v[m][r], slope * v[m][r]);
                    }
                }
            }
            if constexpr (MODE == 2) {
#pragma unroll
                for (int m = 0; m < MT; ++m) {
                    rword_t qv;
                    if constexpr (RL) qv = *(const rword_t*)(xs + raddr + (rr * TW + xb * 16) * PSB + ((m * 8) / PIECE) * PIECE);
                    else qv = rres[nn][(m * 8) / PIECE];
                    const unsigned lo = qv[((m * 8) % PIECE) / 4], hi = qv[((m * 8) % PIECE) / 4 + 1];
                    v[m][0] = mul_then_add(v[m][0], osc[m].x, bf_lo(lo)); v[m][1] = mul_then_add(v[m][1], osc[m].y, bf_hi(lo));
                    v[m][2] = mul_then_add(v[m][2], osc[m].z, bf_lo(hi)); v[m][3] = mul_then_add(v[m][3], osc[m].w, bf_hi(hi));
                }
            }
            bool ok = true;
            if (MASKED) ok = (rr < ylim) && (xb * 16 < xlim);
            if constexpr (MODE == 1 || MODE == 3) {
#pragma unroll
                for (int m = 0; m < MT; ++m)
#pragma unroll
                    for (int r = 0; r < 4; ++r) psum[m][r] += (MASKED && !ok) ? 0.f : v[m][r];
            }
            if constexpr (MODE == 3) {
                if (MASKED && ok && c0 < CS) {
                    const int oy = ty * TH + wv * RPW + rr, ox = tx * TW + xb * 16 + p;
                    bf16_t* const lb = P.out + (size_t)t * 4 * P.lines_len * CS + c0;
                    bf16_t* tgt[4] = {oy == 0 ? lb + (size_t)ox * CS : nullptr, oy == P.h - 1 ? lb + ((size_t)P.lines_len + ox) * CS : nullptr,
                                      ox == 0 ? lb + ((size_t)2 * P.lines_len + oy) * CS : nullptr, ox == P.w - 1 ? lb + ((size_t)3 * P.lines_len + oy) * CS : nullptr};
#pragma unroll
                    for (int e = 0; e < 4; ++e) {
                        if (!tgt[e]) continue;
#pragma unroll
                        for (int m = 0; m < MT; ++m)
                            if (c0 + m * 4 < CS) *(uint2*)(tgt[e] + m * 4) = make_uint2(pack_bf2(v[m][0], v[m][1]), pack_bf2(v[m][2], v[m][3]));
                    }
                }
                continue;
            }
#pragma unroll
            for (int q = 0; q < NP; ++q) {
                int vo = o2 + ooff[rr][q] + xb * 16 * PSB;
                if (MASKED) vo = ok ? vo : OOR;
                if (P.dbg & 4) vo = OOR;
                if constexpr (PIECE == 16) {
                    const int m = q * 2;
                    const rword_t d = {pack_bf2(v[m][0], v[m][1]), pack_bf2(v[m][2], v[m][3]), pack_bf2(v[m + 1][0], v[m + 1][1]), pack_bf2(v[m + 1][2], v[m + 1][3])};
                    __builtin_amdgcn_raw_buffer_store_b128(d, ro, vo, 0, 0);
                } else {
                    const rword_t d = {pack_bf2(v[q][0], v[q][1]), pack_bf2(v[q][2], v[q][3])};
                    __builtin_amdgcn_raw_buffer_store_b64(d, ro, vo, 0, 0);
                }
            }
        }
    };

    int sgi = ty / P.S, sleft = min(P.S, P.nty - ty);
    int t2 = t, tx2 = tx, ty2 = ty;
    auto advance2 = [&]() { if (++ty2 == P.nty) { ty2 = 0; if (++tx2 == P.ntx) { tx2 = 0; ++t2; } } };
    advance2();
    auto tile = [&](const int i, const rset_t& rres, rset_t& rnxt) __attribute__((always_inline)) {
        __builtin_amdgcn_s_barrier();
        const char* const xs = xbufs + (i % NBUF) * BUFSZ;
        if (i + 1 < n) load_res(rnxt, t2, tx2, ty2);
        const int oy0 = ty * TH, ox0 = tx * TW;
        const __amdgpu_buffer_rsrc_t ro = frame_rsrc(P.out + (size_t)t * frame_elems, frame_bytes);
        const int o2 = (oy0 * P.w + ox0) * PSB;
        const bool full = (oy0 + TH <= P.h) && (ox0 + TW <= P.w);
#pragma unroll
        for (int ps = 0; ps < NTW / NH; ++ps) {
            const int N0 = ps * NH;
            f32x4_t acc[MT][NH];
            bf16x8_t bq[2][NH], aq[2][WLDS ? MT : 1];
#pragma unroll
            for (int m = 0; m < MT; ++m)
#pragma unroll
                for (int nh = 0; nh < NH; ++nh) acc[m][nh] = biasv[m];
            if (!(P.dbg & 2)) {
#pragma unroll
            for (int nh = 0; nh < NH; ++nh)
                bq[0][nh] = as_frag(*(const uint4*)(xs + addr_s[0] + (((N0 + nh) >> 1) * RW + ((N0 + nh) & 1) * 16) * PSB));
            if constexpr (WLDS) {
#pragma unroll
                for (int m = 0; m < MT; ++m) aq[0][m] = as_frag(*(const uint4*)(wl + (m * KS) * 1024));
            }
#pragma unroll
            for (int s = 0; s < KS; ++s) {
                if (s + 1 < KS) {
#pragma unroll
                    for (int nh = 0; nh < NH; ++nh)
                        bq[(s + 1) & 1][nh] = as_frag(*(const uint4*)(xs + addr_s[s + 1] + (((N0 + nh) >> 1) * RW + ((N0 + nh) & 1) * 16) * PSB));
                    if constexpr (WLDS) {
#pragma unroll
                        for (int m = 0; m < MT; ++m) aq[(s + 1) & 1][m] = as_frag(*(const uint4*)(wl + (m * KS + s + 1) * 1024));
                    }
                }
                __builtin_amdgcn_sched_barrier(0);
#pragma unroll
                for (int m = 0; m < MT; ++m)
#pragma unroll
                    for (int nh = 0; nh < NH; ++nh)
                        acc[m][nh] = mfma16(WLDS ? aq[s & 1][m] : A[WLDS ? 0 : m][WLDS ? 0 : s], bq[s & 1][nh], s == 0 ? biasv[m] : acc[m][nh]);
                __builtin_amdgcn_sched_barrier(0);
            }
            }
            const bool plain = full && !(MODE == 3 && (ty == 0 || ty == P.nty - 1 || tx == 0 || tx == P.ntx - 1));
            if (plain) finish(acc, rres, xs, N0, ro, o2, false, 0, 0);
            else finish(acc, rres, xs, N0, ro, o2, true, P.h - oy0 - wv * RPW, P.w - ox0 - p);
        }
        if (--sleft == 0) {
            flush_pool(t, tx, sgi);
            ++sgi;
            sleft = min(P.S, P.nty - ty - 1);
        }
        if (++ty == P.nty) {
            ty = 0; sgi = 0; sleft = min(P.S, P.nty);
            if (++tx == P.ntx) {
                tx = 0;
                ++t;
                if (i + 1 < n) {
                    load_osc(t);
                    if constexpr (MODE == 2) {
#pragma unroll
                        for (int m = 0; m < MT; ++m) { pin(osc[m].x); pin(osc[m].y); pin(osc[m].z); pin(osc[m].w); }
                    }
                }
            }
        }
        advance2();
    };
    for (int i = 0; i < n; i += 2) {
        tile(i, rA, rB);
        if (i + 1 < n) tile(i + 1, rB, rA);
    }
}

template <int MT, int CS, int TH, int D, int WR>
__global__ __launch_bounds__(320, c3p_waves(MT)) void cabp_kernel(const C3P P) {
    extern __shared__ __attribute__((aligned(16))) char smem[];
    constexpr int TW = 32, RH = TH + 4, RW = TW + 4, MH = TH + 2, MW = TW + 2, NPB = CS / 8, PSB = CS * 2;
    constexpr int KTOT = 9 * CS, KS = (KTOT + 31) / 32;
    constexpr int ROWP = RW * NPB, NITEM = RH * ROWP, NDMA = (NITEM + 63) / 64, XBUF = NDMA * 1024;
    constexpr int NBUF = D + 1, NL = NDMA;
    constexpr bool W1L = !(WR & 1), W2L = !(WR & 2);
    constexpr int WSET = MT * KS * 1024, W2OFF = W1L ? WSET : 0, WBYTES = W2OFF + (W2L ? WSET : 0);
    constexpr int NM = MH * MW, NT1 = (NM + 15) / 16, PER1 = (NT1 + 3) / 4;
    constexpr int NH1 = MT == 1 ? 3 : 2;
    constexpr int RPW = TH / 4, NTW = RPW * 2, NH = MT == 1 ? (NTW < 4 ? NTW : 4) : 2;
    constexpr int MIDB = (NM * PSB + 15) / 16 * 16;
    static_assert(TH % 4 == 0 && NL * (D - 1) <= 63 && D >= 1 && PER1 % NH1 == 0 && NTW % NH == 0, "tile / prefetch shape");
    const int lane = threadIdx.x & 63, wv = wave_id();
    const int G = (int)gridDim.x, c = ((int)blockIdx.x & 7) * (G >> 3) + ((int)blockIdx.x >> 3);
    const int fseg = c * P.qs, nsegs = min(P.qs, P.nsg - fseg);
    if (nsegs <= 0) return;
    int t = fseg / (P.ntx * P.nseg), tx, ty, n = 0;
    {
        const int rem = fseg - t * (P.ntx * P.nseg);
        tx = rem / P.nseg;
        const int sg = rem - tx * P.nseg;
        ty = sg * P.S;
        const int tail = P.nty - (P.nseg - 1) * P.S;
        for (int k = 0, g2 = sg; k < nsegs; ++k) { n += g2 == P.nseg - 1 ? tail : P.S; if (++g2 == P.nseg) g2 = 0; }
    }
    n = __builtin_amdgcn_readfirstlane(n);
    t = __builtin_amdgcn_readfirstlane(t); tx = __builtin_amdgcn_readfirstlane(tx); ty = __builtin_amdgcn_readfirstlane(ty);
    const int rowpitch = P.w * PSB, frame_bytes = P.h * rowpitch;
    const size_t frame_elems = (size_t)P.h * P.w * CS;
    char* const mids = smem + WBYTES;
    char* const xbufs = mids + MIDB;
    if constexpr (W1L || W2L) {
        for (int i = (int)threadIdx.x; i < MT * KS * 64; i += 320) {
            if constexpr (W1L) *(uint4*)(smem + i * 16) = P.wfrag[i];
            if constexpr (W2L) *(uint4*)(smem + W2OFF + i * 16) = P.w2[i];
        }
        __syncthreads();
    }

    if (wv == 4) {
        int voff[NDMA], pxk[NDMA];
#pragma unroll
        for (int k = 0; k < NDMA; ++k) {
            const int i = k * 64 + lane, ic = i < NITEM ? i : NITEM - 1;
            const int r = ic / ROWP, j = ic - r * ROWP;
            voff[k] = r * rowpitch + j * 16;
            pxk[k] = j / NPB;
        }
        int ft = t, ftx = tx, fty = ty;
        for (int i = -D; i < n; ++i) {
            if (i >= 0) {
                if (n - 1 - i >= D - 1) wait_vmcnt<NL * (D - 1)>(); else wait_vmcnt<0>();
                __builtin_amdgcn_s_barrier();
            }
            const int j = i + D;
            if (j < n) {
                const __amdgpu_buffer_rsrc_t rs = frame_rsrc(P.in + (size_t)ft * frame_elems, frame_bytes);
                const int ix0 = ftx * TW - 2;
                const int o = ((fty * TH - 2) * P.w + ix0) * PSB;
                const bool edge = ftx == 0 || ix0 + RW > P.w;
                char* const dst = xbufs + (j % NBUF) * XBUF;
#pragma unroll
                for (int k = 0; k < NDMA; ++k) {
                    int vo = voff[k] + o;
                    if (edge) { const int gx = ix0 + pxk[k]; vo = (gx < 0 || gx >= P.w) ? (int)0x80000000 : vo; }
                    dma16(rs, dst + k * 1024, vo);
                }
                if (++fty == P.nty) { fty = 0; if (++ftx == P.ntx) { ftx = 0; ++ft; } }
            }
            if (i >= 0) __builtin_amdgcn_s_barrier();
        }
        return;
    }

    const int g = lane >> 4, p = lane & 15;
    const int c0 = g * 4 * MT;
    int toff1[KS], addr2[KS];
    const int lane_base2 = ((wv * RPW) * MW + p) * PSB;
#pragma unroll
    for (int s = 0; s < KS; ++s) {
        int o1 = 0, o2 = 0;
#pragma unroll
        for (int gg = 0; gg < 4; ++gg) {
            const int kk0 = (s * 4 + gg) * 8;
            const int tap = kk0 / CS, cc0 = kk0 - tap * CS, dy = tap / 3, dx = tap - dy * 3;
            const int a = kk0 < KTOT ? (dy * RW + dx) * PSB + cc0 * 2 : 0, b = kk0 < KTOT ? (dy * MW + dx) * PSB + cc0 * 2 : 0;
            o1 = g == gg ? a : o1; o2 = g == gg ? b : o2;
        }
        toff1[s] = o1;
        addr2[s] = lane_base2 + o2;
    }
    int pix1[PER1], mwr[PER1];
#pragma unroll
    for (int i = 0; i < PER1; ++i) {
        const int q = (wv + 4 * i) * 16 + p, qc = q < NM ? q : NM - 1;
        const int my = qc / MW, mx = qc - my * MW;
        pix1[i] = (my * RW + mx) * PSB;
        mwr[i] = (q < NM && c0 < CS) ? qc * PSB + c0 * 2 : -1;
    }
    bf16x8_t A1[W1L ? 1 : MT][W1L ? 1 : KS], A2[W2L ? 1 : MT][W2L ? 1 : KS];
    if constexpr (!W1L) {
#pragma unroll
        for (int m = 0; m < MT; ++m)
#pragma unroll
            for (int s = 0; s < KS; ++s) A1[m][s] = as_frag(P.wfrag[(m * KS + s) * 64 + lane]);
    }
    if constexpr (!W2L) {
#pragma unroll
        for (int m = 0; m < MT; ++m)
#pragma unroll
            for (int s = 0; s < KS; ++s) A2[m][s] = as_frag(P.w2[(m * KS + s) * 64 + lane]);
    }
    const char* const wl = smem + lane * 16;
    f32x4_t bias1[MT], bias2[MT];
#pragma unroll
    for (int m = 0; m < MT; ++m) {
        const float4 a4 = P.bias ? *(const float4*)(P.bias + c0 + m * 4) : make_float4(0.f, 0.f, 0.f, 0.f);
        const float4 b4 = P.b2 ? *(const float4*)(P.b2 + c0 + m * 4) : make_float4(0.f, 0.f, 0.f, 0.f);
        bias1[m] = (f32x4_t){a4.x, a4.y, a4.z, a4.w};
        bias2[m] = (f32x4_t){b4.x, b4.y, b4.z, b4.w};
    }
    const float slope = P.prelu;
    float4 osc[MT];
    auto load_osc = [&](int ft) {
#pragma unroll
        for (int m = 0; m < MT; ++m) osc[m] = *(const float4*)(P.oscale + (size_t)ft * P.oscale_stride + c0 + m * 4);
    };
    load_osc(t);
    auto pin_osc = [&]() __attribute__((always_inline)) {
#pragma unroll
        for (int m = 0; m < MT; ++m) { pin(osc[m].x); pin(osc[m].y); pin(osc[m].z); pin(osc[m].w); }
    };
#pragma unroll
    for (int m = 0; m < MT; ++m) {
        pin(bias1[m]); pin(bias2[m]);
        if constexpr (!W1L) {
#pragma unroll
            for (int s = 0; s < KS; ++s) pin(A1[m][s]);
        }
        if constexpr (!W2L) {
#pragma unroll
            for (int s = 0; s < KS; ++s) pin(A2[m][s]);
        }
    }
    pin_osc();
    constexpr int OOR = (int)0x80000000;
    constexpr int PIECE = (MT == 2 || MT == 4) ? 16 : 8, NP = (MT * 8) / PIECE;
    typedef unsigned rword_t __attribute__((ext_vector_type(PIECE / 4)));
    int ooff[RPW][NP];
#pragma unroll
    for (int rr = 0; rr < RPW; ++rr)
#pragma unroll
        for (int q = 0; q < NP; ++q)
            ooff[rr][q] = (c0 + q * (PIECE / 2) < CS) ? ((wv * RPW + rr) * P.w + p) * PSB + c0 * 2 + q * PIECE : OOR;
    const int raddr = ((wv * RPW + 2) * RW + p + 2) * PSB + c0 * 2;

    for (int i = 0; i < n; ++i) {
        __builtin_amdgcn_s_barrier();
        const char* const xs = xbufs + (i % NBUF) * XBUF;
        const int oy0 = ty * TH, ox0 = tx * TW;
        const bool inner = oy0 >= 1 && oy0 + TH + 1 <= P.h && ox0 >= 1 && ox0 + TW + 1 <= P.w;
#pragma unroll
        for (int ps = 0; ps < PER1 / NH1; ++ps) {
            f32x4_t acc[MT][NH1];
            bf16x8_t bq[2][NH1], aq[2][W1L ? MT : 1];
#pragma unroll
            for (int nh = 0; nh < NH1; ++nh) bq[0][nh] = as_frag(*(const uint4*)(xs + pix1[ps * NH1 + nh] + toff1[0]));
            if constexpr (W1L) {
#pragma unroll
                for (int m = 0; m < MT; ++m) aq[0][m] = as_frag(*(const uint4*)(wl + (m * KS) * 1024));
            }
#pragma unroll
            for (int s = 0; s < KS; ++s) {
                if (s + 1 < KS) {
#pragma unroll
                    for (int nh = 0; nh < NH1; ++nh) bq[(s + 1) & 1][nh] = as_frag(*(const uint4*)(xs + pix1[ps * NH1 + nh] + toff1[s + 1]));
                    if constexpr (W1L) {
#pragma unroll
                        for (int m = 0; m < MT; ++m) aq[(s + 1) & 1][m] = as_frag(*(const uint4*)(wl + (m * KS + s + 1) * 1024));
                    }
                }
                __builtin_amdgcn_sched_barrier(0);
#pragma unroll
                for (int m = 0; m < MT; ++m)
#pragma unroll
                    for (int nh = 0; nh < NH1; ++nh)
                        acc[m][nh] = mfma16(W1L ? aq[s & 1][m] : A1[W1L ? 0 : m][W1L ? 0 : s], bq[s & 1][nh], s == 0 ? bias1[m] : acc[m][nh]);
                __builtin_amdgcn_sched_barrier(0);
            }
#pragma unroll
            for (int nh = 0; nh < NH1; ++nh) {
                const int i1 = ps * NH1 + nh;
                bool in = true;
                if (!inner) {
                    const int pq = pix1[i1] / PSB, my = pq / RW, mx = pq - my * RW;
                    const int gy = oy0 - 1 + my, gx = ox0 - 1 + mx;
                    in = gy >= 0 && gy < P.h && gx >= 0 && gx < P.w;
                }
                unsigned wd[MT][2];
#pragma unroll
                for (int m = 0; m < MT; ++m) {
                    float v[4] = {acc[m][nh][0], acc[m][nh][1], acc[m][nh][2], acc[m][nh][3]};
#pragma unroll
                    for (int r = 0; r < 4; ++r) v[r] = max_bare(v[r], slope * v[r]);
                    wd[m][0] = in ? pack_bf2(v[0], v[1]) : 0u;
                    wd[m][1] = in ? pack_bf2(v[2], v[3]) : 0u;
                }
                if (mwr[i1] >= 0) {
                    char* dst = mids + mwr[i1];
                    if constexpr (MT == 2 || MT == 4) {
#pragma unroll
                        for (int m = 0; m < MT; m += 2)
                            if (c0 + m * 4 < CS) *(uint4*)(dst + m * 8) = make_uint4(wd[m][0], wd[m][1], wd[m + 1][0], wd[m + 1][1]);
                    } else {
#pragma unroll
                        for (int m = 0; m < MT; ++m)
                            if (c0 + m * 4 < CS) *(uint2*)(dst + m * 8) = make_uint2(wd[m][0], wd[m][1]);
                    }
                }
            }
        }
        __builtin_amdgcn_s_barrier();
        const __amdgpu_buffer_rsrc_t ro = frame_rsrc(P.out + (size_t)t * frame_elems, frame_bytes);
        const int o2 = (oy0 * P.w + ox0) * PSB;
        const bool full = (oy0 + TH <= P.h) && (ox0 + TW <= P.w);
        const int ylim = P.h - oy0 - wv * RPW, xlim = P.w - ox0 - p;
#pragma unroll
        for (int ps = 0; ps < NTW / NH; ++ps) {
            const int N0 = ps * NH;
            f32x4_t acc[MT][NH];
            bf16x8_t bq[2][NH], aq[2][W2L ? MT : 1];
#pragma unroll
            for (int nh = 0; nh < NH; ++nh)
                bq[0][nh] = as_frag(*(const uint4*)(mids + addr2[0] + (((N0 + nh) >> 1) * MW + ((N0 + nh) & 1) * 16) * PSB));
            if constexpr (W2L) {
#pragma unroll
                for (int m = 0; m < MT; ++m) aq[0][m] = as_frag(*(const uint4*)(wl + W2OFF + (m * KS) * 1024));
            }
#pragma unroll
            for (int s = 0; s < KS; ++s) {
                if (s + 1 < KS) {
#pragma unroll
                    for (int nh = 0; nh < NH; ++nh)
                        bq[(s + 1) & 1][nh] = as_frag(*(const uint4*)(mids + addr2[s + 1] + (((N0 + nh) >> 1) * MW + ((N0 + nh) & 1) * 16) * PSB));
                    if constexpr (W2L) {
#pragma unroll
                        for (int m = 0; m < MT; ++m) aq[(s + 1) & 1][m] = as_frag(*(const uint4*)(wl + W2OFF + (m * KS + s + 1) * 1024));
                    }
                }
                __builtin_amdgcn_sched_barrier(0);
#pragma unroll
                for (int m = 0; m < MT; ++m)
#pragma unroll
                    for (int nh = 0; nh < NH; ++nh)
                        acc[m][nh] = mfma16(W2L ? aq[s & 1][m] : A2[W2L ? 0 : m][W2L ? 0 : s], bq[s & 1][nh], s == 0 ? bias2[m] : acc[m][nh]);
                __builtin_amdgcn_sched_barrier(0);
            }
#pragma unroll
            for (int nh = 0; nh < NH; ++nh) {
                const int nn = N0 + nh, rr = nn >> 1, xb = nn & 1;
                float v[MT][4];
#pragma unroll
                for (int m = 0; m < MT; ++m) {
                    const rword_t qv = *(const rword_t*)(xs + raddr + (rr * RW + xb * 16) * PSB + ((m * 8) / PIECE) * PIECE);
                    const unsigned lo = qv[((m * 8) % PIECE) / 4], hi = qv[((m * 8) % PIECE) / 4 + 1];
                    v[m][0] = mul_then_add(acc[m][nh][0], osc[m].x, bf_lo(lo)); v[m][1] = mul_then_add(acc[m][nh][1], osc[m].y, bf_hi(lo));
                    v[m][2] = mul_then_add(acc[m][nh][2], osc[m].z, bf_lo(hi)); v[m][3] = mul_then_add(acc[m][nh][3], osc[m].w, bf_hi(hi));
                }
                const bool ok = full || ((rr < ylim) && (xb * 16 < xlim));
#pragma unroll
                for (int q = 0; q < NP; ++q) {
                    int vo = o2 + ooff[rr][q] + xb * 16 * PSB;
                    vo = ok ? vo : OOR;
                    if constexpr (PIECE == 16) {
                        const int m = q * 2;
                        const rword_t d = {pack_bf2(v[m][0], v[m][1]), pack_bf2(v[m][2], v[m][3]), pack_bf2(v[m + 1][0], v[m + 1][1]), pack_bf2(v[m + 1][2], v[m + 1][3])};
                        __builtin_amdgcn_raw_buffer_store_b128(d, ro, vo, 0, 0);
                    } else {
                        const rword_t d = {pack_bf2(v[q][0], v[q][1]), pack_bf2(v[q][2], v[q][3])};
                        __builtin_amdgcn_raw_buffer_store_b64(d, ro, vo, 0, 0);
                    }
                }
            }
        }
        if (++ty == P.nty) {
            ty = 0;
            if (++tx == P.ntx) { tx = 0; ++t; if (i + 1 < n) { load_osc(t); pin_osc(); } }
        }
    }
}

int c3p_segment(int h, int w, int th, int wgs_model) {
    const int ntx = (w + 31) / 32, nty = (h + th - 1) / th;
    const int cand[6] = {8, 6, 4, 3, 2, 1}, Ts[5] = {12, 16, 20, 36, 52};
    double best = 1e30;
    int bestS = 1;
    for (int k = 0; k < 6; ++k) {
        const int S = cand[k] < nty ? cand[k] : nty;
        const int nseg = (nty + S - 1) / S;
        double cost = 0.0;
        for (int j = 0; j < 5; ++j) {
            const long ntiles = (long)ntx * nty * Ts[j];
            long g = 256L * wgs_model;
            if (g > (ntiles + 7) / 8) g = (ntiles + 7) / 8;
            if (g < 1) g = 1;
            const long nsg = (long)nseg * ntx * Ts[j], qs = (nsg + g - 1) / g;
            cost += (1.0 + 0.25 / S) * (double)(qs * S) * (double)g / (double)ntiles;
        }
        if (cost < best - 1e-9) { best = cost; bestS = S; }
    }
    return bestS;
}

struct C3PPlan { int ntx, nty, S, nseg, nsg, qs, grid, pool_rows; };

C3PPlan c3p_plan(int T, int h, int w, int th, int ncu, int wgs, int S) {
    C3PPlan p;
    p.ntx = (w + 31) / 32; p.nty = (h + th - 1) / th;
    const long ntiles = (long)p.ntx * p.nty * T;
    long g = (long)ncu * wgs;
    if (g > (ntiles + 7) / 8) g = (ntiles + 7) / 8;
    if (g < 1) g = 1;
    p.S = S < p.nty ? S : p.nty;
    p.nseg = (p.nty + p.S - 1) / p.S;
    const long nsg = (long)p.nseg * p.ntx * T;
    p.nsg = (int)nsg;
    p.qs = (int)((nsg + g - 1) / g);
    const int chunks = (p.nsg + p.qs - 1) / p.qs;
    p.grid = (chunks + 7) / 8 * 8;
    p.pool_rows = 4 * p.ntx * p.nseg;
    return p;
}

template <int MT, int CS, int TH, int D, int MODE, bool RL>
int launch_conv3p_mode(const C3P& K, const C3PPlan& pl, hipStream_t st) {
    constexpr int NPB = CS / 8, NDMA = ((TH + 2) * 34 * NPB + 63) / 64, KS = (9 * CS + 31) / 32, RDMA = RL ? (TH * 32 * NPB) / 64 : 0;
    C3P P = K;
    P.ntx = pl.ntx; P.nty = pl.nty; P.S = pl.S; P.nseg = pl.nseg; P.nsg = pl.nsg; P.qs = pl.qs; P.pool_rows = pl.pool_rows;
    const size_t lds = (size_t)(D + 1) * (NDMA + RDMA) * 1024 + (MT * KS > 16 ? MT * KS * 1024 : 0);
    if (lds > 160 * 1024) return SN_EINVAL;
    if (lds > 64 * 1024 && hipFuncSetAttribute((const void*)conv3p_kernel<MT, CS, TH, D, MODE, RL>, hipFuncAttributeMaxDynamicSharedMemorySize, (int)lds) != hipSuccess)
        return SN_ELAUNCH;
    hipLaunchKernelGGL((conv3p_kernel<MT, CS, TH, D, MODE, RL>), dim3(pl.grid), dim3(320), lds, st, P);
    return sn_check_launch();
}

template <int MT, int CS, int TH, int D, int D2, bool RL2>
int launch_conv3p(const C3P& K, const C3PPlan& pl, int mode, hipStream_t st) {
    switch (mode) {
        case 0: return launch_conv3p_mode<MT, CS, TH, D, 0, false>(K, pl, st);
        case 1: return launch_conv3p_mode<MT, CS, TH, D, 1, false>(K, pl, st);
        case 2: return launch_conv3p_mode<MT, CS, TH, D2, 2, RL2>(K, pl, st);
        case 3: return launch_conv3p_mode<MT, CS, TH, D, 3, false>(K, pl, st);
        default: return SN_EINVAL;
    }
}

template <int MT, int CS, int TH, int D, int WR = 0>
int launch_cabp(const C3P& K, const C3PPlan& pl, hipStream_t st) {
    constexpr int NPB = CS / 8, NDMA = ((TH + 4) * 36 * NPB + 63) / 64, KS = (9 * CS + 31) / 32;
    C3P P = K;
    P.ntx = pl.ntx; P.nty = pl.nty; P.S = pl.S; P.nseg = pl.nseg; P.nsg = pl.nsg; P.qs = pl.qs; P.pool_rows = 0;
    const size_t lds = (size_t)(D + 1) * NDMA * 1024 + ((TH + 2) * 34 * CS * 2 + 15) / 16 * 16 + ((WR & 1) ? 0 : MT * KS * 1024) + ((WR & 2) ? 0 : MT * KS * 1024);
    if (lds > 160 * 1024) return SN_EINVAL;
    if (lds > 64 * 1024 && hipFuncSetAttribute((const void*)cabp_kernel<MT, CS, TH, D, WR>, hipFuncAttributeMaxDynamicSharedMemorySize, (int)lds) != hipSuccess)
        return SN_ELAUNCH;
    hipLaunchKernelGGL((cabp_kernel<MT, CS, TH, D, WR>), dim3(pl.grid), dim3(320), lds, st, P);
    return sn_check_launch();
}

int c3p_mode(const sn_conv_desc* d, bool want_pool = false) {
    if (d->res2) return -1;
    const bool pool = d->pool != nullptr || want_pool;
    if (d->act == 0 && !pool && !d->oscale && !d->res) return 0;
    if (d->act == 1 && d->prelu >= 0.f && d->prelu <= 1.f && pool && !d->oscale && !d->res) return 1;
    if (d->act == 0 && !pool && d->oscale && d->res) return 2;
    return -1;
}

}

int sn_conv3p_key(const sn_conv_desc* d, bool want_pool) {
    if (!(d->k == 3 && d->stride == 1 && d->pad == 1 && d->in_mode == 0 && d->out_mode == 0 && d->n_in == 1 && d->cs_in == d->cs_out &&
          d->ks == (9 * d->cs_in + 31) / 32 && d->h_in == d->h_out && d->w_in == d->w_out) || c3p_mode(d, want_pool) < 0) return 0;
    if ((size_t)d->h_out * d->w_out * d->cs_out * 2 >= 0x7fffffffull) return 0;
    const int key = d->mt * 1000 + d->cs_in;
    if (key == 1016 && c3p_mode(d, want_pool) == 2 && !(d->flags & 256)) return 0;
    return (key == 1016 || key == 2024 || key == 3040 || key == 3048 || key == 4064) ? key : 0;
}

static int c3p_ncu() {
    int dev = 0, ncu = 0;
    if (hipGetDevice(&dev) != hipSuccess || hipDeviceGetAttribute(&ncu, hipDeviceAttributeMultiprocessorCount, dev) != hipSuccess || ncu < 1) {
        (void)hipGetLastError();
        return 0;
    }
    return ncu;
}
static bool c3p_rl(const sn_conv_desc* d, int key, int mode) { return mode == 2 && (key == 1016 || key == 2024) && !(d->flags & 512); }
static int c3p_wgs_default(int key) { return key == 1016 ? 3 : key == 2024 ? 2 : 1; }
static int c3p_wgs(const sn_conv_desc* d, int key, int mode) {
    const int o = (d->flags >> 4) & 15;
    if (o) return o;
    if (key == 1016) return c3p_rl(d, key, mode) ? 2 : 3;
    return key == 2024 ? 2 : 1;
}

int sn_conv3p_pool_rows(const sn_conv_desc* d) {
    const int key = sn_conv3p_key(d, true), ncu = key ? c3p_ncu() : 0;
    if (!key || !ncu) return 0;
    return c3p_plan(d->T, d->h_out, d->w_out, 8, ncu, c3p_wgs(d, key, 1), c3p_segment(d->h_out, d->w_out, 8, c3p_wgs_default(key))).pool_rows;
}

int sn_conv3p_route(const sn_conv_desc* d, int lines_len, int ncu, int* plan8) {
    const int key = sn_conv3p_key(d, false);
    if (!key) return SN_EINVAL;
    if (ncu == 0) ncu = c3p_ncu();
    if (ncu < 1) return SN_EINVAL;
    const int mode = lines_len > 0 ? 3 : c3p_mode(d);
    if (mode < 0 || (lines_len > 0 && c3p_mode(d) != 1)) return SN_EINVAL;
    const int mt = key / 1000, cs = key % 1000, depth = (d->flags >> 10) & 3;
    bool rl = c3p_rl(d, key, mode);
    int D = 2;
    if (key == 1016 && (depth == 1 || depth == 2)) { D = depth + 2; rl = false; }
    else if (key == 2024 && rl) D = 1;
    else if (key == 4064) D = 1;
    const int npb = cs / 8, ndma = (10 * 34 * npb + 63) / 64, ks = (9 * cs + 31) / 32, rdma = rl ? (8 * 32 * npb) / 64 : 0;
    const size_t lds = (size_t)(D + 1) * (ndma + rdma) * 1024 + (mt * ks > 16 ? mt * ks * 1024 : 0);
    if (lds > 160 * 1024) return SN_EINVAL;
    if (plan8) {
        const C3PPlan pl = c3p_plan(d->T, d->h_out, d->w_out, 8, ncu, c3p_wgs(d, key, mode), c3p_segment(d->h_out, d->w_out, 8, c3p_wgs_default(key)));
        const int v[8] = {pl.ntx, pl.nty, pl.S, pl.nseg, pl.nsg, pl.qs, pl.grid, pl.pool_rows};
        for (int i = 0; i < 8; ++i) plan8[i] = v[i];
    }
    return SN_CONV_ROUTE(SN_CONV_K_STREAM, mt, cs, D, mode, rl ? 1 : 0);
}

template <int MT, int CS, int D>
int launch_conv3p_rf(const C3P& K, const C3PPlan& pl, int mode, hipStream_t st) {
    return launch_conv3p<MT, CS, 8, D, D, false>(K, pl, mode, st);
}

int sn_conv3p_launch(const sn_conv_desc* d, int lines_len, int route, const int* plan8, void* stream) {
    if ((route >> 24) != SN_CONV_K_STREAM || !plan8) return SN_EINVAL;
    C3P K;
    K.in = (const bf16_t*)d->in[0]; K.res = (const bf16_t*)d->res; K.out = (bf16_t*)d->out;
    K.wfrag = (const uint4*)d->wfrag; K.bias = d->bias; K.oscale = d->oscale; K.oscale_stride = d->oscale_stride;
    K.pool = d->pool; K.pool_rows = 0; K.act = d->act; K.prelu = d->prelu;
    K.T = d->T; K.h = d->h_out; K.w = d->w_out; K.lines_len = lines_len; K.dbg = (d->flags >> 12) & 7;
    const C3PPlan pl = {plan8[0], plan8[1], plan8[2], plan8[3], plan8[4], plan8[5], plan8[6], plan8[7]};
    hipStream_t st = (hipStream_t)stream;
    const int mt = (route >> 20) & 15, cs = (route >> 12) & 255, D = (route >> 8) & 15, mode = (route >> 4) & 15;
    const bool rl = route & 1;
    switch (mt * 1000 + cs) {
        case 1016:
            if (rl) return launch_conv3p_mode<1, 16, 8, 2, 2, true>(K, pl, st);
            return D == 3 ? launch_conv3p_rf<1, 16, 3>(K, pl, mode, st) : (D == 4 ? launch_conv3p_rf<1, 16, 4>(K, pl, mode, st)
                                                                                  : launch_conv3p_rf<1, 16, 2>(K, pl, mode, st));
        case 2024: return rl ? launch_conv3p_mode<2, 24, 8, 1, 2, true>(K, pl, st) : launch_conv3p_rf<2, 24, 2>(K, pl, mode, st);
        case 3040: return launch_conv3p_rf<3, 40, 2>(K, pl, mode, st);
        case 3048: return launch_conv3p_rf<3, 48, 2>(K, pl, mode, st);
        case 4064: return launch_conv3p_rf<4, 64, 1>(K, pl, mode, st);
        default: return SN_EINVAL;
    }
}

int sn_cabp_launch(const sn_conv_desc* a, const sn_conv_desc* b, void* stream) {
    const int key = a->mt * 1000 + a->cs_in, ncu = c3p_ncu();
    if (!ncu || !(key == 1016 || key == 2024) || a->act != 1 || !(a->prelu >= 0.f && a->prelu <= 1.f) || !b->oscale || b->res2) return SN_EINVAL;
    if ((size_t)a->h_out * a->w_out * a->cs_out * 2 >= 0x7fffffffull) return SN_EINVAL;
    C3P K;
    K.in = (const bf16_t*)a->in[0]; K.res = nullptr; K.out = (bf16_t*)b->out;
    K.wfrag = (const uint4*)a->wfrag; K.bias = a->bias; K.w2 = (const uint4*)b->wfrag; K.b2 = b->bias;
    K.oscale = b->oscale; K.oscale_stride = b->oscale_stride; K.pool = nullptr; K.pool_rows = 0; K.act = 1; K.prelu = a->prelu;
    K.T = a->T; K.h = a->h_out; K.w = a->w_out; K.lines_len = 0; K.dbg = 0;
    const int o = (a->flags >> 4) & 15;
    const bool shallow = ((a->flags >> 10) & 3) == 3;
    const C3PPlan pl = c3p_plan(a->T, a->h_out, a->w_out, 8, ncu, o ? o : (key == 1016 ? (shallow ? 3 : 2) : 1), c3p_segment(a->h_out, a->w_out, 8, c3p_wgs_default(key)));
    hipStream_t st = (hipStream_t)stream;
    if (shallow) return key == 1016 ? launch_cabp<1, 16, 8, 1>(K, pl, st) : launch_cabp<2, 24, 8, 1>(K, pl, st);
    if (key == 1016 && !((b->flags >> 12) & 1)) return launch_cabp<1, 16, 8, 2, 2>(K, pl, st);
    return key == 1016 ? launch_cabp<1, 16, 8, 2>(K, pl, st) : launch_cabp<2, 24, 8, 2>(K, pl, st);
}
```

shift-net_amd/shiftnet_amd/engine.py:

```python
from __future__ import annotations

import contextlib
import ctypes as C
import os
from collections import OrderedDict
from dataclasses import dataclass
from typing import Dict, List, Optional, Sequence, Tuple

import torch

from . import lib as L
from . import prep
from .spec import UNIT_NAMES, Variant, shift_table


@dataclass
class Act:
    t: torch.Tensor
    c: int

    @property
    def dims(self) -> Tuple[int, int, int, int]:
        return tuple(self.t.shape)


def _dtype_code(dt: torch.dtype) -> int:
    return {torch.float32: L.SN_F32, torch.float16: L.SN_F16, torch.bfloat16: L.SN_BF16}[dt]


def host_f32_copy(sd: Dict[str, torch.Tensor]) -> Dict[str, torch.Tensor]:
    keys = list(sd.keys())
    if not keys:
        return {}
    dev_keys = [k for k in keys if sd[k].device.type != "cpu"]
    out = {k: sd[k].detach().float() for k in keys if sd[k].device.type == "cpu"}
    if dev_keys:
        flat = torch.cat([sd[k].detach().reshape(-1).float() for k in dev_keys]).cpu()
        o = 0
        for k in dev_keys:
            n = sd[k].numel()
            out[k] = flat[o:o + n].reshape(sd[k].shape)
            o += n
    return {k: out[k] for k in keys}


class Plan:

    def __init__(self, V: Variant, sd: Dict[str, torch.Tensor], device: torch.device) -> None:
        self.V = V
        self.device = device
        self.sd = host_f32_copy(sd)
        self.convs: Dict[str, Dict[str, object]] = {}
        self.cas: Dict[str, Dict[str, object]] = {}
        self.units: Dict[str, Dict[str, object]] = {}
        self.offs = prep.shift_offsets_i8(shift_table(V.c1)).to(device)
        self.k0_mfma_ok = all(dx % 4 == 0 and abs(dy) <= 8 and abs(dx) <= 8 for dy, dx in shift_table(V.c1))
        self._build()

    def _dev(self, t: Optional[torch.Tensor]) -> Optional[torch.Tensor]:
        return None if t is None else t.contiguous().to(self.device)

    def add_conv(self, name: str, key: str, cins: Sequence[int], shuffle: bool = False) -> None:
        w = self.sd[key + "weight"]
        b = self.sd.get(key + "bias")
        cs_in = prep.ceil8(max(cins))
        p = prep.pack_conv(w, b, cins, cs_in, shuffle)
        p["wfrag"] = self._dev(p["wfrag"])
        p["bias"] = self._dev(p["bias"])
        self.convs[name] = p

    def add_ca(self, name: str, key: str) -> None:
        wa = self.sd[key + "conv_du.0.weight"]
        wb = self.sd[key + "conv_du.2.weight"]
        cr, c = wa.shape[0], wa.shape[1]
        self.cas[name] = {"wa": self._dev(wa.reshape(cr, c)), "wb": self._dev(wb.reshape(c, cr)), "c": c, "cr": cr}

    def scalar(self, key: str) -> float:
        return float(self.sd[key].reshape(-1)[0])

    def add_cab(self, pre: str, c: int) -> None:
        self.add_conv(pre + "body.0", pre + "body.0.", [c])
        self.add_conv(pre + "body.2", pre + "body.2.", [c])
        self.add_ca(pre + "CA", pre + "CA.")
        cpad = 16 * int(self.convs[pre + "body.2"]["mt"])
        w2 = torch.zeros((c, 9, cpad), dtype=torch.float32)
        w2[:, :, :c] = self.sd[pre + "body.2.weight"].to(torch.bfloat16).float().reshape(c, c, 9).permute(1, 2, 0)
        self.cas[pre + "CA"]["w2"] = self._dev(w2)

    def add_naf(self, pre: str, c: int, with_shift: bool) -> None:
        V, sd = self.V, self.sd
        u: Dict[str, object] = {}
        i = 0
        if with_shift:
            w1 = sd[pre + "conv1.weight"].reshape(c // 2, 9)
            u["w1"] = self._dev((w1.to(torch.bfloat16).view(torch.int16).to(torch.int32) & 0xFFFF).contiguous())
        g = prep.pack_ln_gemm(sd[f"{pre}body.{i}.weight"], sd[pre + "norm.weight"], sd[pre + "norm.bias"], c); i += 1
        u["w_ln"], u["b_ln"] = self._dev(g["wfrag"]), self._dev(g["bias"])
        w3 = prep.pack_dw3_gate(sd[f"{pre}body.{i}.conv_2.weight"], c); i += 1
        u["w_dw3_h2"] = self._dev(prep.pk_f16_words(w3))
        i += 1
        if V.denoise:
            self.add_ca(f"{pre}ca1", f"{pre}body.{i}."); i += 1
        if V.grouped_rep:
            u["w_grp"] = self._dev(prep.pack_grouped_frag(sd[f"{pre}body.{i}.conv_1.weight"], sd[f"{pre}body.{i}.conv_2.weight"]))
        else:
            w5 = prep.pack_dw5(sd[f"{pre}body.{i}.conv_1.weight"], sd[f"{pre}body.{i}.conv_2.weight"])
            u["w_toep5"] = self._dev(prep.pack_toeplitz(w5, 5))
        i += 1
        u["w_gate"] = self._dev(prep.pack_gate_gemm(sd[f"{pre}body.{i}.weight"], c))
        d = {k: self._dev(v) for k, v in prep.pack_phase1r(
            sd[f"{pre}body.0.weight"], sd[pre + "norm.weight"], sd[pre + "norm.bias"], sd[f"{pre}body.1.conv_2.weight"],
            sd[f"{pre}body.{i - 1}.conv_1.weight"], sd[f"{pre}body.{i - 1}.conv_2.weight"], sd[f"{pre}body.{i}.weight"], c).items()}
        d["desc"] = L.Phase1Weights(d["wfrag1"].data_ptr(), d["w3"].data_ptr(), d["wgrp"].data_ptr(), d["wfrag2"].data_ptr())
        u["p1r"] = d
        i += 1
        i += 1
        self.add_ca(f"{pre}ca2", f"{pre}body.{i}."); i += 1
        o = prep.pack_out_gemm(sd[f"{pre}body.{i}.weight"], sd[pre + "beta"], sd.get(f"{pre}body.{i}.bias"), c)
        u["w_out"], u["b_out"] = self._dev(o["wfrag"]), self._dev(o["bias"])
        self.units[pre] = u

    def add_shift_block(self, pre: str, c: int) -> None:
        for k in range(self.V.units):
            self.add_naf(f"{pre}{UNIT_NAMES[k]}.0.", c, True)
            self.add_naf(f"{pre}{UNIT_NAMES[k]}.1.", c, False)

    def add_down(self, pre: str, cin: int) -> None:
        self.add_conv(pre + "down", pre + ("down.0." if self.V.denoise else "down."), [cin])

    def add_unet(self, pre: str) -> None:
        V = self.V
        c = [V.c0, V.c0 + V.unet_step, V.c0 + 2 * V.unet_step]
        for lvl, n in ((1, 1), (2, 3), (3, 3)):
            for i in range(n):
                self.add_cab(f"{pre}encoder_level{lvl}.{i}.", c[lvl - 1])
                self.add_cab(f"{pre}decoder_level{lvl}.{i}.", c[lvl - 1])
        self.add_down(pre + "down12.", c[0])
        self.add_down(pre + "down23.", c[1])
        self.add_cab(pre + "skip_attn1.", c[0])
        self.add_cab(pre + "skip_attn2.", c[1])
        self.add_conv(pre + "up21", pre + "up21.up.1.", [c[1]])
        self.add_conv(pre + "up32", pre + "up32.up.1.", [c[2]])

    def _build(self) -> None:
        V = self.V
        c0, c1 = V.c0, V.c1
        self.add_conv("feat_extract.0", "feat_extract.0.", [V.in_ch])
        self.add_cab("feat_extract.1.", c0)
        self.add_conv("conv_trans", "conv_trans.", [c0])
        self.add_conv("conv_last", "conv_last.", [c0])
        self.add_conv("rconcat", "rconcat.", [c0, c0, c0])
        for i in range(1, V.n_orb + 1):
            self.add_unet(f"orb{i}.")
            self.add_unet(f"rorb{i}.")
        p = "stage1."
        self.add_cab(p + "concat.", c0)
        self.add_conv(p + "down01", p + "down01.0.", [c0])
        self.add_down(p + "down12.", c1)
        if V.topo == "small":
            blocks = ["encoder_level1", "encoder_level1_1", "encoder_level1_2", "encoder_level2", "encoder_level2_1",
                      "encoder_level2_2", "decoder_level2", "decoder_level2_1", "decoder_level2_2",
                      "decoder_level1", "decoder_level1_1", "decoder_level1_2"]
        else:
            self.add_down(p + "down23.", c1)
            if V.shift_cab:
                self.add_cab(p + "encoder_level0.", c0)
                self.add_cab(p + "encoder_level0_1.", c0)
            for n in ("encoder_level1", "encoder_level1_1", "encoder_level2", "encoder_level2_1",
                      "encoder_level3", "encoder_level3_1"):
                self.add_cab(f"{p}{n}.", c1)
            self.add_cab(p + "skip_attn2.", c1)
            self.add_conv(p + "up32", p + "up32.up.1.", [c1])
            blocks = ["decoder_level3", "decoder_level3_1", "decoder_level2", "decoder_level2_1",
                      "decoder_level1", "decoder_level1_1", "decoder_level1_2"]
        for b in blocks:
            self.add_shift_block(f"{p}{b}.", c1)
        self.add_cab(p + "skip_attn1.", c1)
        self.add_conv(p + "up21", p + "up21.up.1.", [c1])
        self.add_conv(p + "upsample0", p + "upsample0.upsample_conv.", [c1], shuffle=True)
        self.add_cab(p + "skip_conv.", c0)
        self.add_cab(p + "out_conv.", c0)
        self.add_conv(p + "conv_hr0", p + "conv_hr0.", [c0, c0] if V.hr_cat else [c0])


class Engine:

    def __init__(self, plan: Plan, dtype: torch.dtype = torch.bfloat16) -> None:
        self.P = plan
        self.dtype = dtype
        self.V = plan.V
        self.lib = L.load()
        self.dev = plan.device
        self.prof: Optional[list] = None
        self._meta: Tuple = ()
        self._unit: Optional[Tuple] = None
        self._k4_meta: Tuple = ()
        self.split = None
        self._side = None
        self._tickets = None
        self._old_tickets: List[torch.Tensor] = []
        self._clip = 0
        self._bad = None
        self.fallbacks = 0
        if self.phase1 not in ("auto", "r", "0"):
            raise ValueError(f"SN_PHASE1={self.phase1!r}: expected auto, r (fused kernel) or 0 (two-kernel bf16 chain)")
        if self.k4_fuse not in ("0", "1"):
            raise ValueError(f"SN_K4_FUSE={self.k4_fuse!r}: expected 1 (CAB2's phase 2 inside CAB1's phase 1, four launches per unit) or 0 (five launches)")
        g = os.environ.get("SN_GRAPH", "auto")
        self.use_graph = g == "1"
        self.graph_auto = g not in ("0", "1")
        self._graphs: "OrderedDict[Tuple, object]" = OrderedDict()

    def _stream(self) -> int:
        return torch.cuda.current_stream(self.dev).cuda_stream

    def _call(self, fn: str, label: str, *args) -> None:
        f = getattr(self.lib, fn)
        if self.prof is None:
            L.check(f(*args), label)
            return
        e0, e1 = torch.cuda.Event(enable_timing=True), torch.cuda.Event(enable_timing=True)
        e0.record()
        L.check(f(*args), label)
        e1.record()
        meta = self._meta
        if self._unit is not None and not (meta and meta[0] == "naf"):
            meta = tuple(meta) + ("unit",) + self._unit
        if fn == "sn_cab2_phase2_cab1_phase1":
            self.prof.append(("sn_gsts_cab2_phase2", "sn_gsts_cab2_phase2 [in sn_cab1_phase1]", self._k4_meta, e0, e0))
            fn = "sn_cab1_phase1"
        self.prof.append((fn, label, meta, e0, e1))

    act_dtype = torch.bfloat16

    def _new(self, T: int, h: int, w: int, cs: int) -> torch.Tensor:
        return torch.empty((T, h, w, cs), dtype=self.act_dtype, device=self.dev)

    conv_tiles = os.environ.get("SN_CONV_TILES", "0") == "1"
    conv_stream_all = os.environ.get("SN_CONV_STREAM_ALL", "0") == "1"
    conv_res_regs = os.environ.get("SN_CONV_RES_REGS", "0") == "1"
    conv_dbg = int(os.environ.get("SN_CONV_DBG", "0"))
    conv_depth = int(os.environ.get("SN_CONV_DEPTH", "0"))
    conv_wgs = int(os.environ.get("SN_CONV_WGS", "0"))
    conv_s2_small = os.environ.get("SN_CONV_S2_SMALL", "0") == "1"

    def conv(self, name: str, ins: Sequence[Act], *, stride: int = 1, pad: Optional[int] = None, prelu: Optional[float] = None,
             res: Optional[Act] = None, out_mode: int = 0, pool: bool = False, in_mode: int = 0, oscale: Optional[torch.Tensor] = None,
             nchw_out: Optional[torch.Tensor] = None, nchw_sc: Optional[torch.Tensor] = None, res2: Optional[Act] = None,
             remap: Optional[Tuple[int, int, int]] = None):
        p = self.P.convs[name]
        k, cout = int(p["k"]), int(p["cout"])
        T, hs, ws, cs_in = ins[0].dims
        if remap is not None:
            T = T // remap[1] * remap[0]
        assert cs_in == p["cs_in"] and len(ins) == p["n_in"], (name, cs_in, p["cs_in"])
        h_in, w_in = (2 * hs, 2 * ws) if in_mode == 1 else (hs, ws)
        if pad is None:
            pad = k // 2
        h_out = (h_in + 2 * pad - k) // stride + 1
        w_out = (w_in + 2 * pad - k) // stride + 1
        d = L.ConvDesc()
        for i in range(3):
            d.inp[i] = ins[i].t.data_ptr() if i < len(ins) else None
        d.n_in, d.cs_in, d.T, d.h_in, d.w_in, d.in_mode = len(ins), cs_in, T, h_in, w_in, in_mode
        d.k, d.stride, d.pad, d.h_out, d.w_out = k, stride, pad, h_out, w_out
        d.wfrag, d.mt, d.ks = p["wfrag"].data_ptr(), int(p["mt"]), int(p["ks"])
        d.bias = p["bias"].data_ptr() if p["bias"] is not None else None
        d.act, d.prelu = (1, prelu) if prelu is not None else (0, 0.0)
        pool_buf = None
        out_act: Optional[Act] = None
        if out_mode == 2:
            assert nchw_out is not None and nchw_sc is not None
            d.out, d.sc, d.cs_out = nchw_out.data_ptr(), nchw_sc.data_ptr(), 8
            d.c_out, d.nchw_dtype, d.sc_dtype = cout, _dtype_code(nchw_out.dtype), _dtype_code(nchw_sc.dtype)
        else:
            c_log = cout // 4 if out_mode == 1 else cout
            cs_out = prep.ceil8(c_log)
            o = self._new(T, 2 * h_out, 2 * w_out, cs_out) if out_mode == 1 else self._new(T, h_out, w_out, cs_out)
            out_act = Act(o, c_log)
            d.out, d.cs_out, d.c_out = o.data_ptr(), cs_out, cout
        d.out_mode = out_mode
        d.flags = L.SN_CONV_TILE_KERNEL if self.conv_tiles else ((self.conv_wgs << 4) | (256 if self.conv_stream_all else 0) | (512 if self.conv_res_regs else 0) | (self.conv_depth << 10) | (self.conv_dbg << 12))
        if self.conv_s2_small:
            d.flags |= 1 << 15
        if res is not None:
            assert out_mode == 0 and res.dims == out_act.dims
            d.res = res.t.data_ptr()
        if res2 is not None:
            assert out_mode == 0 and res2.dims == out_act.dims
            d.res2 = res2.t.data_ptr()
        if oscale is not None:
            d.oscale, d.oscale_stride = oscale.data_ptr(), oscale.shape[1]
        if remap is not None:
            d.clip_n, d.clip_T, d.clip_lo = remap
        if pool:
            nblk = self.lib.sn_conv_pool_blocks(C.byref(d))
            pool_buf = torch.empty((T, nblk, 16 * d.mt), dtype=torch.float32, device=self.dev)
            d.pool = pool_buf.data_ptr()
        self._meta = ("conv", T, h_out, w_out, len(ins) * cs_in, int(d.cs_out), k, stride, in_mode, out_mode)
        self._call("sn_conv2d", f"sn_conv2d[{name}]", C.byref(d), self._stream())
        if pool:
            return out_act, pool_buf, h_out * w_out
        return out_act

    def ca_mlp(self, name: str, pool: torch.Tensor, npix: int) -> torch.Tensor:
        p = self.P.cas[name]
        T, nblk, cpad = pool.shape
        ca = torch.empty((T, cpad), dtype=torch.float32, device=self.dev)
        self._call("sn_ca_mlp", f"sn_ca_mlp[{name}]", pool.data_ptr(), nblk, cpad, p["c"], p["cr"], 1.0 / npix, p["wa"].data_ptr(),
                                   p["wb"].data_ptr(), ca.data_ptr(), T, None, self._stream())
        return ca

    k0_mfma = os.environ.get("SN_K0_MFMA", "1") != "0"
    g1_store = os.environ.get("SN_G1_STORE", "1") != "0"
    fold_se = True
    phase1 = os.environ.get("SN_PHASE1", "auto")
    k4_fuse = os.environ.get("SN_K4_FUSE", "1")
    range_guard = os.environ.get("SN_RANGE_GUARD", "1") != "0"
    range_guard_async = os.environ.get("SN_RANGE_GUARD", "1") == "async"
    fused_cab_tail = True

    def cab(self, pre: str, x: Act, extra: Optional[Act] = None) -> Act:
        if self.fused_cab_tail:
            p = self.P.cas[pre + "CA"]
            T, h, w, cs = x.dims
            slope = self.P.scalar(pre + "body.1.weight")
            if self.cab_fused in ("8", "16", "s8", "s16") or (self.cab_fused[0] == "p" and extra is None and not self.conv_tiles and
                                                              (self.cab_fused == "p" or (cs == 16 and T * h * w >= self.CAB_FUSED_MIN_PX))):
                out = self._cab_fused(pre, x, extra, slope)
                if out is not None:
                    return out
            scratch = torch.empty((self.lib.sn_cab_ca_scratch_floats(T),), dtype=torch.float32, device=self.dev)
            mid, pool, _ = self.conv(pre + "body.0", [x], prelu=slope, pool=True)
            _, nblk, cpad = pool.shape
            ca = torch.empty((T, cpad), dtype=torch.float32, device=self.dev)
            self._call("sn_cab_ca", f"sn_cab_ca[{pre}]", pool.data_ptr(), nblk, cpad, mid.t.data_ptr(), cs, p["c"], p["cr"], h, w,
                       p["w2"].data_ptr(), p["wa"].data_ptr(), p["wb"].data_ptr(), scratch.data_ptr(), ca.data_ptr(), T, self._stream())
            return self.conv(pre + "body.2", [mid], res=x, oscale=ca, res2=extra)
        r = self.conv(pre + "body.0", [x], prelu=self.P.scalar(pre + "body.1.weight"))
        r, pool, npix = self.conv(pre + "body.2", [r], pool=True)
        return self.scale_residual(r, x, self.ca_mlp(pre + "CA", pool, npix), extra)

    cab_fused = os.environ.get("SN_CAB_FUSED", "p16")
    CAB_FUSED_MIN_PX = 4 << 20

    def _conv_desc(self, name: str, x: Act, *, prelu: Optional[float] = None) -> L.ConvDesc:
        p = self.P.convs[name]
        T, h, w, cs = x.dims
        assert cs == p["cs_in"] and p["n_in"] == 1 and int(p["k"]) == 3
        d = L.ConvDesc()
        d.inp[0] = x.t.data_ptr()
        d.n_in, d.cs_in, d.T, d.h_in, d.w_in, d.in_mode = 1, cs, T, h, w, 0
        d.k, d.stride, d.pad, d.h_out, d.w_out = 3, 1, 1, h, w
        d.wfrag, d.mt, d.ks = p["wfrag"].data_ptr(), int(p["mt"]), int(p["ks"])
        d.bias = p["bias"].data_ptr() if p["bias"] is not None else None
        d.act, d.prelu = (1, prelu) if prelu is not None else (0, 0.0)
        d.cs_out, d.c_out, d.out_mode = prep.ceil8(int(p["cout"])), int(p["cout"]), 0
        d.flags = L.SN_CONV_TILE_KERNEL
        return d

    def _cab_fused(self, pre: str, x: Act, extra: Optional[Act], slope: float) -> Optional[Act]:
        lib = self.lib
        T, h, w, cs = x.dims
        if h < 2 or w < 2:
            return None
        if self.cab_fused[0] == "p" and not 0.0 <= slope <= 1.0:
            return None
        d1 = self._conv_desc(pre + "body.0", x, prelu=slope)
        d2 = self._conv_desc(pre + "body.2", x)
        if self.cab_fused[0] in "sp" and not self.conv_tiles:
            d1.flags = (self.conv_wgs << 4) | (self.conv_depth << 10) | (0 if self.cab_fused[0] == "p" else self.conv_dbg << 12)
            if self.cab_fused[0] == "p":
                d2.flags = (self.conv_dbg & 1) << 12
        if d1.cs_out != cs or d2.cs_out != cs or not lib.sn_cab_fused_supported(C.byref(d1), C.byref(d2)):
            return None
        p = self.P.cas[pre + "CA"]
        ll = max(h, w)
        lines = torch.empty((T, 4, ll, cs), dtype=self.act_dtype, device=self.dev)
        nblk = lib.sn_conv_pool_blocks(C.byref(d1))
        pool = torch.empty((T, nblk, 16 * d1.mt), dtype=torch.float32, device=self.dev)
        scratch = torch.empty((lib.sn_cab_ca_scratch_floats(T),), dtype=torch.float32, device=self.dev)
        ca = torch.empty((T, 16 * d1.mt), dtype=torch.float32, device=self.dev)
        out = self._new(T, h, w, cs)
        d1.out, d1.pool = lines.data_ptr(), pool.data_ptr()
        d2.out, d2.res, d2.oscale, d2.oscale_stride = out.data_ptr(), x.t.data_ptr(), ca.data_ptr(), ca.shape[1]
        if extra is not None:
            assert extra.dims == x.dims
            d2.res2 = extra.t.data_ptr()
        rows = 0 if self.cab_fused[0] == "p" else 16 if self.cab_fused.endswith("16") else 8
        st = self._stream()
        self._meta = ("cabf", T, h, w, cs, 1)
        self._call("sn_cab_stats", f"sn_cab_stats[{pre}]", C.byref(d1), ll, st)
        self._meta = ()
        self._call("sn_cab_ca_lines", f"sn_cab_ca[{pre}]", pool.data_ptr(), nblk, 16 * d1.mt, lines.data_ptr(), ll, cs, p["c"], p["cr"], h, w,
                   p["w2"].data_ptr(), p["wa"].data_ptr(), p["wb"].data_ptr(), scratch.data_ptr(), ca.data_ptr(), T, st)
        self._meta = ("cabf", T, h, w, cs, 3 if extra is not None else 2)
        self._call("sn_cab_fused", f"sn_cab_fused[{pre}]", C.byref(d1), C.byref(d2), rows, st)
        return Act(out, x.c)

    def _wrap_flag(self, mode: int, circular: bool) -> int:
        if self.split is not None and mode:
            return self.split.wrap_flag(mode, circular)
        return 1 if circular else 0

    def _unit_src(self, x: Act, mode: int, *, wrap: Optional[int] = None, halo: Optional[torch.Tensor] = None, t0: int = 0, nt: int = 0) -> L.UnitSrc:
        T, h, w, cs = x.dims
        assert cs == x.c
        wrap = self._wrap_flag(mode, self.V.wrap) if wrap is None else wrap
        return L.UnitSrc(x.t.data_ptr(), T, h, w, x.c, mode, wrap, halo.data_ptr() if halo is not None else None, t0, nt, self._clip)

    def _split_pieces(self, x: Act, mode: int, circular: bool):
        T = x.dims[0]
        flag = self._wrap_flag(mode, circular)
        if self.split is None:
            yield (flag, None, 0, 0)
            return
        main = torch.cuda.current_stream(self.dev)
        ready = main.record_event()
        recv = flag == 2
        bt = 0 if mode == 1 else T - 1
        if recv and T > 1:
            yield (0, None, 1 if mode == 1 else 0, T - 1)
        if self._side is None:
            self._side = torch.cuda.Stream(self.dev)
        with torch.cuda.stream(self._side):
            self._side.wait_event(ready)
            x.t.record_stream(self._side)
            halo = self.split.exchange(x.t, mode, circular)
        if recv:
            main.wait_stream(self._side)
            halo.record_stream(main)
            yield (2, halo, bt, 1)
        else:
            yield (flag, None, 0, 0)

    def temporal_roll(self, x: Act, reverse: bool) -> Act:
        T, h, w, cs = x.dims
        assert cs == x.c, "Shift_CAB widths (24, 80) are stored unpadded"
        y = self._new(T, h, w, cs)
        mode = 2 if reverse else 1
        self._meta = ("roll", T, h, w, cs)
        for wrap, halo, t0, nt in self._split_pieces(x, mode, False):
            s = self._unit_src(x, mode, wrap=wrap, halo=halo, t0=t0, nt=nt)
            self._call("sn_temporal_roll", "sn_temporal_roll", C.byref(s), y.data_ptr(), self._stream())
        return Act(y, x.c)

    def shift_cab(self, pre: str, x: Act, reverse: bool) -> Act:
        return self.cab(pre, self.temporal_roll(x, reverse))

    def _guard_ptr(self) -> Optional[int]:
        if not self.range_guard:
            return None
        if self._bad is None:
            self._bad = torch.zeros((1,), dtype=torch.int32, device=self.dev)
        return self._bad.data_ptr()

    def _fold_ok(self, T: int) -> bool:
        return self.fold_se and (self._clip or T) <= self.MAX_TICKETS

    def _ticket_ptr(self, T: int) -> int:
        if self._tickets is None or self._tickets.numel() < T:
            if self._tickets is not None:
                self._old_tickets.append(self._tickets)
            self._tickets = torch.zeros((max(self.MAX_TICKETS, T),), dtype=torch.int32, device=self.dev)
        return self._tickets.data_ptr()

    def _fused_phase1(self, T: int) -> bool:
        if self.phase1 == "0":
            return False
        return not (self.V.denoise and not self._fold_ok(T))

    def k4_fused(self, T: int, c: int) -> bool:
        return (self.k4_fuse == "1" and self._fused_phase1(T) and self._fold_ok(T) and c == 64 and not self.V.denoise and self.split is None
                and not self._clip and self.schedule == "unit")

    def naf(self, pre: str, x: Act, mode: int, *, frames: Optional[Tuple[int, int]] = None, bufs: Optional[Dict[str, torch.Tensor]] = None,
            defer_k4: bool = False, k4: Optional[Tuple] = None):
        lib, V, P = self.lib, self.V, self.P
        u = P.units[pre]
        T, h, w, c = x.dims
        self._meta = ("naf", frames[1] if frames is not None else T, h, w, c, mode, T)
        fused = self._fused_phase1(T)
        mstencil = not V.grouped_rep
        B = bufs if bufs is not None else self.naf_buffers(T, h, w, c, mode)
        hwb, g2, y, pool2, ca2, ca1, g1, pool1, g1s = (B.get(k) for k in ("hwb", "g2", "y", "pool2", "ca2", "ca1", "g1", "pool1", "g1s"))
        nb2 = pool2.shape[1]
        tickets = self._ticket_ptr(T) if fused and self._fold_ok(T) else None
        b_out = u["b_out"].data_ptr() if u["b_out"] is not None else None
        es = 2
        bad = self._guard_ptr()

        def ca_mlp(name: str, pool: torch.Tensor, ca: torch.Tensor, f0: int, n: int) -> None:
            q = P.cas[name]
            nblk = pool.shape[1]
            self._call("sn_ca_mlp", f"sn_ca_mlp[{name}]", pool.data_ptr() + f0 * nblk * c * 4, nblk, c, q["c"], q["cr"], 1.0 / (h * w),
                       q["wa"].data_ptr(), q["wb"].data_ptr(), ca.data_ptr() + f0 * c * 4, n, bad, self._stream())

        if frames is not None:
            assert self.split is None
            pieces = [(self._wrap_flag(mode, V.wrap) if mode else 0, None, frames[0], frames[1])]
        else:
            pieces = self._split_pieces(x, mode, V.wrap) if mode else [(0, None, 0, 0)]
        for wrap, halo, t0, nt in pieces:
            st = self._stream()
            src = self._unit_src(x, mode, wrap=wrap, halo=halo, t0=t0, nt=nt)
            f0, n = (t0, nt) if nt else (0, T)
            if mode:
                if self.k0_mfma and P.k0_mfma_ok:
                    self._call("sn_gsts_shiftconv_mfma", "sn_gsts_shiftconv", C.byref(src), P.offs.data_ptr(), u["w1"].data_ptr(), hwb.data_ptr(), st)
                else:
                    self._call("sn_gsts_shiftconv", "sn_gsts_shiftconv", C.byref(src), P.offs.data_ptr(), u["w1"].data_ptr(), hwb.data_ptr(), st)
            hw_ptr = hwb.data_ptr() if mode else None
            folded = False
            if fused:
                wt = C.byref(u["p1r"]["desc"])
                sep = None
                if tickets is not None:
                    q = P.cas[pre + "ca2"]
                    se = L.SeFold(q["wa"].data_ptr(), q["wb"].data_ptr(), q["c"], q["cr"], tickets, ca2.data_ptr(), bad)
                    sep = C.byref(se)
                opt = None
                if V.denoise:
                    q1 = P.cas[pre + "ca1"]
                    se1 = L.SeFold(q1["wa"].data_ptr(), q1["wb"].data_ptr(), q1["c"], q1["cr"], tickets, ca1.data_ptr(), bad)
                    g1s_ptr = g1s.data_ptr() if (g1s is not None and self.g1_store) else None
                    o1 = L.Phase1Opts(None, 1, 0, g1s_ptr)
                    fn1 = "sn_gsts_cab2_phase1" if mode else "sn_cab1_phase1"
                    a1 = (C.byref(src), hw_ptr, wt, None, pool2.data_ptr(), C.byref(se1), C.byref(o1), st) if mode else \
                         (C.byref(src), wt, None, pool2.data_ptr(), C.byref(se1), C.byref(o1), st)
                    self._call(fn1, fn1 + "[g1 sums]", *a1)
                    opt = C.byref(L.Phase1Opts(ca1.data_ptr(), 0, 0, g1s_ptr))
                if mode:
                    self._call("sn_gsts_cab2_phase1", "sn_gsts_cab2_phase1", C.byref(src), hw_ptr, wt, g2.data_ptr(), pool2.data_ptr(), sep, opt, st)
                elif k4 is not None:
                    src2, g2_2, ca2_2, w_out2, b_out2, self._k4_meta = k4[:6]
                    self._call("sn_cab2_phase2_cab1_phase1", "sn_cab2_phase2_cab1_phase1", C.byref(src2), g2_2.data_ptr(), ca2_2.data_ptr(), w_out2.data_ptr(),
                               b_out2, x.t.data_ptr(), wt, g2.data_ptr(), pool2.data_ptr(), sep, None, st)
                else:
                    self._call("sn_cab1_phase1", "sn_cab1_phase1", C.byref(src), wt, g2.data_ptr(), pool2.data_ptr(), sep, opt, st)
                folded = sep is not None
            else:
                self._call("sn_ln_gemm_gate", "sn_ln_gemm_gate", C.byref(src), hw_ptr, u["w_ln"].data_ptr(), u["b_ln"].data_ptr(),
                           u["w_dw3_h2"].data_ptr(), g1.data_ptr(), pool1.data_ptr() if pool1 is not None else None, 2 if mstencil else 0, st)
                ca1_ptr = None
                if V.denoise:
                    ca_mlp(pre + "ca1", pool1, ca1, f0, n)
                    ca1_ptr = ca1.data_ptr() + f0 * c * 4
                fr1 = g1.stride(0) * es * f0
                fr2 = g2.stride(0) * es * f0
                k3 = "sn_dw5m_gemm_gate" if mstencil else "sn_grp5_gemm_gate"
                self._call(k3, k3, g1.data_ptr() + fr1, ca1_ptr, u["w_toep5" if mstencil else "w_grp"].data_ptr(), u["w_gate"].data_ptr(),
                           g2.data_ptr() + fr2, pool2.data_ptr() + f0 * nb2 * c * 4, n, h, w, c, st)
            if not folded:
                ca_mlp(pre + "ca2", pool2, ca2, f0, n)
            if defer_k4:
                return Act(y, c), (src, g2, ca2, u["w_out"], b_out, self._meta, B)
            fn4 = "sn_gsts_cab2_phase2" if mode else "sn_cab1_phase2"
            self._call(fn4, fn4, C.byref(src), g2.data_ptr(), ca2.data_ptr(), u["w_out"].data_ptr(), b_out, y.data_ptr(), st)
        return Act(y, c)

    def naf_buffers(self, T: int, h: int, w: int, c: int, mode: int) -> Dict[str, torch.Tensor]:
        lib, V = self.lib, self.V
        fused = self._fused_phase1(T)
        mstencil = not V.grouped_rep
        B: Dict[str, torch.Tensor] = {}
        if mode:
            B["hwb"] = self._new(T, h, w, c // 2)
        B["g2"] = self._new(T, h, w, c)
        B["y"] = self._new(T, h, w, c)
        if fused:
            nb2 = lib.sn_phase1_pool_blocks(T, h, w)
            if nb2 < 1:
                raise L.ShiftNetLibError(f"sn_phase1_pool_blocks failed with code {nb2}")
            if V.denoise and self.g1_store:
                nbytes = C.c_longlong(0)
                L.check(lib.sn_phase1_g1_store_bytes(T, h, w, c, C.byref(nbytes)), "sn_phase1_g1_store_bytes")
                B["g1s"] = torch.empty((nbytes.value,), dtype=torch.uint8, device=self.dev)
        else:
            B["g1"] = (torch.empty((T, h, c, lib.sn_planar_pitch(w)), dtype=torch.bfloat16, device=self.dev) if mstencil else self._new(T, h, w, c))
            nb2 = lib.sn_dw5m_blocks(h, w) if mstencil else lib.sn_grp5_blocks(h, w)
            if V.denoise:
                B["pool1"] = torch.empty((T, lib.sn_lngate_blocks(h, w), c), dtype=torch.float32, device=self.dev)
        if V.denoise:
            B["ca1"] = torch.empty((T, c), dtype=torch.float32, device=self.dev)
        B["pool2"] = torch.empty((T, nb2, c), dtype=torch.float32, device=self.dev)
        B["ca2"] = torch.empty((T, c), dtype=torch.float32, device=self.dev)
        return B

    def gsts_unit(self, pre: str, x: Act, reverse: bool) -> Act:
        if self.k4_fused(x.dims[0], x.c):
            y2, k4 = self.naf(pre + "0.", x, 2 if reverse else 1, defer_k4=True)
            return self.naf(pre + "1.", y2, 0, k4=k4)
        return self.naf(pre + "1.", self.naf(pre + "0.", x, 2 if reverse else 1), 0)

    def shift_block(self, pre: str, x: Act) -> Act:
        for i in range(self.V.units):
            x = self.gsts_unit(f"{pre}{UNIT_NAMES[i]}.", x, reverse=(i % 2 == 1))
        return x

    schedule = os.environ.get("SN_SCHEDULE", "unit")
    frame_group = int(os.environ.get("SN_FRAME_GROUP", "4"))
    stream_groups = int(os.environ.get("SN_STREAM_GROUPS", "2"))
    STREAMS_MIN_PXF = 400_000

    def shift_chain(self, pres: Sequence[str], x: Act) -> Act:
        T = x.dims[0]
        if self.schedule not in ("unit", "frame", "streams") or self.frame_group < 1 or self.stream_groups < 1:
            raise ValueError(f"SN_SCHEDULE={self.schedule!r} / SN_FRAME_GROUP={self.frame_group} / SN_STREAM_GROUPS={self.stream_groups}: "
                             "expected unit, frame or streams, and groups of >= 1 frames")
        ev = None
        if self.prof is not None:
            ev = (torch.cuda.Event(enable_timing=True), torch.cuda.Event(enable_timing=True))
            ev[0].record()
        y = self._shift_chain(pres, x)
        if ev is not None:
            ev[1].record()
            self.prof.append(("gsts_chain", "gsts_chain", ("chain",) + tuple(x.dims) + (len(pres) * self.V.units,), ev[0], ev[1]))
        return y

    def _shift_chain(self, pres: Sequence[str], x: Act) -> Act:
        T = x.dims[0]
        if self.schedule == "streams" and self.split is None and not self._clip and not torch.cuda.is_current_stream_capturing():
            ng = min(self.stream_groups, T // 2)
            if ng >= 2 and (T // ng) * x.dims[1] * x.dims[2] >= self.STREAMS_MIN_PXF:
                return self._shift_chain_streams(pres, x, ng)
        if self.schedule != "frame" or self.split is not None or self._clip or T <= self.frame_group:
            for pre in pres:
                x = self.shift_block(pre, x)
            return x
        _, h, w, c = x.dims
        units = [(f"{pre}{UNIT_NAMES[i]}.", i % 2 == 1) for pre in pres for i in range(self.V.units)]
        G = self.frame_group
        groups = [(t0, min(G, T - t0)) for t0 in range(0, T, G)]
        bufs = [(self.naf_buffers(T, h, w, c, 2 if rev else 1), self.naf_buffers(T, h, w, c, 0)) for _, rev in units]
        ins = [x] + [Act(b1["y"], c) for _, b1 in bufs]
        for u, j in wavefront_order([rev for _, rev in units], T, G, self.V.wrap):
            pre, rev = units[u]
            y2 = self.naf(pre + "0.", ins[u], 2 if rev else 1, frames=groups[j], bufs=bufs[u][0])
            self.naf(pre + "1.", y2, 0, frames=groups[j], bufs=bufs[u][1])
        return ins[-1]

    STREAM_RING = 3

    def _shift_chain_streams(self, pres: Sequence[str], x: Act, ng: int) -> Act:
        T, h, w, c = x.dims
        units = [(f"{pre}{UNIT_NAMES[i]}.", i % 2 == 1) for pre in pres for i in range(self.V.units)]
        R = min(self.STREAM_RING, max(len(units), 2))
        groups, plan = stream_plan([rev for _, rev in units], T, ng, self.V.wrap, R)
        if getattr(self, "_gstreams", None) is None or len(self._gstreams) < ng:
            self._gstreams = [torch.cuda.Stream(self.dev) for _ in range(ng)]
        streams = self._gstreams[:ng]
        main = torch.cuda.current_stream(self.dev)
        sets = [(self.naf_buffers(T, h, w, c, 1), self.naf_buffers(T, h, w, c, 0)) for _ in range(R)]
        if self._fused_phase1(T) and self._fold_ok(T):
            self._ticket_ptr(T)
        self._guard_ptr()
        ready = main.record_event()
        done: List[List[Optional[torch.cuda.Event]]] = [[None] * ng for _ in units]
        cab2: List[List[Optional[torch.cuda.Event]]] = [[None] * ng for _ in units]
        cur = x
        for u, (pre, rev) in enumerate(units):
            b2, b1 = sets[u % R]
            for g, fr in enumerate(groups):
                raw, war = plan[u][g]
                with torch.cuda.stream(streams[g]):
                    s = streams[g]
                    if u == 0:
                        s.wait_event(ready)
                    for uu, gg in raw:
                        s.wait_event(done[uu][gg])
                    for uu, gg in war:
                        s.wait_event(cab2[uu][gg])
                    y2 = self.naf(pre + "0.", cur, 2 if rev else 1, frames=fr, bufs=b2)
                    cab2[u][g] = s.record_event()
                    self.naf(pre + "1.", y2, 0, frames=fr, bufs=b1)
                    done[u][g] = s.record_event()
            cur = Act(b1["y"], c)
        for g in range(ng):
            main.wait_event(done[-1][g])
        return cur

    def down(self, pre: str, x: Act) -> Act:
        if self.V.denoise:
            return self.conv(pre + "down", [x], stride=2, prelu=self.P.scalar(pre + "down.1.weight"))
        return self.conv(pre + "down", [x], stride=2)

    skip_up_lowres = os.environ.get("SN_SKIPUP_LOWRES", "1") != "0"

    def skip_up(self, name: str, x: Act, y: Act) -> Act:
        if not self.skip_up_lowres:
            return self.conv(name, [x], in_mode=1, res=y)
        lo = self.conv(name, [x])
        T, hs, ws, cs = lo.dims
        assert y.dims == (T, 2 * hs, 2 * ws, cs), (y.dims, lo.dims)
        out = self._new(T, 2 * hs, 2 * ws, cs)
        self._meta = ("up2add", T, hs, ws, cs)
        self._call("sn_upsample2_add", f"sn_upsample2_add[{name}]", lo.t.data_ptr(), y.t.data_ptr(), out.data_ptr(), T, hs, ws, cs, self._stream())
        return Act(out, lo.c)
# ... 373 lines not shown
```

shift-net_amd/shiftnet_amd/lib.py:

```python
from __future__ import annotations

import ctypes as C
import os
from typing import Optional

_HERE = os.path.dirname(os.path.abspath(__file__))
LIB_PATH = os.path.join(os.path.dirname(_HERE), "lib", "libshiftnet_hip.so")

SN_F32, SN_F16, SN_BF16 = 0, 1, 2

ABI_VERSION = 20

SYMBOLS = [
    "sn_abi_version", "sn_selftest_mfma", "sn_ingest", "sn_conv2d", "sn_conv_pool_blocks", "sn_conv2d_route","sn_upsample2_add", "sn_ca_mlp",
    "sn_cab_ca", "sn_cab_ca_scratch_floats", "sn_cab_fused_supported", "sn_cab_stats", "sn_cab_ca_lines", "sn_cab_fused", "sn_planar_pitch", "sn_nhwc_to_planar", "sn_dw5m_blocks",
    "sn_dw5m_gemm_gate", "sn_gsts_gather", "sn_temporal_roll", "sn_gsts_shiftconv", "sn_gsts_shiftconv_mfma", "sn_gsts_cab2_phase2", "sn_cab1_phase2",
    "sn_ingest_u8", "sn_egress_blocks", "sn_egress_u8", "sn_ssim_blocks", "sn_ssim_u8",
    "sn_ingest_yuv", "sn_egress_yuv", "sn_yuv_thumb", "sn_yuv_noise_hist",
    "sn32_conv2d", "sn32_conv2d_route", "sn32_gsts_gather", "sn32_layernorm", "sn32_gate", "sn32_gate_sum", "sn32_chan_sum", "sn32_scale_residual", "sn32_ingest", "sn32_cab_ca", "sn32_dw_gate", "sn32_conv1x1_gate2", "sn32_gsts_shiftconv", "sn32_conv_csum_tiles",
    "sn_ln_gemm_gate", "sn_lngate_blocks", "sn_grp5_gemm_gate", "sn_grp5_blocks", "sn_gsts_cab2_phase1", "sn_cab1_phase1", "sn_phase1_pool_blocks", "sn_phase1_g1_store_bytes", "sn_p1r_plan", "sn_p1r_strip_begin",
    "sn_cab2_phase2_cab1_phase1", "sn_cab2_phase2_cab1_phase1_supported",
]


class Phase1Weights(C.Structure):
    _fields_ = [("wfrag1", C.c_void_p), ("w3", C.c_void_p), ("wgrp", C.c_void_p), ("wfrag2", C.c_void_p)]


class SeFold(C.Structure):
    _fields_ = [("wa", C.c_void_p), ("wb", C.c_void_p), ("c", C.c_int), ("cr", C.c_int), ("ticket", C.c_void_p), ("ca", C.c_void_p), ("bad", C.c_void_p)]


class Phase1Opts(C.Structure):
    _fields_ = [("g1_scale", C.c_void_p), ("g1_sums", C.c_int), ("team", C.c_int), ("g1_store", C.c_void_p)]


def cab_phase1(lib, src: "UnitSrc", hw_ptr, wt: "Phase1Weights", g2_ptr, pool_ptr, stream, se: "SeFold" = None, opt: "Phase1Opts" = None) -> int:
    sep = C.byref(se) if se is not None else None
    op = C.byref(opt) if opt is not None else None
    if src.mode:
        return lib.sn_gsts_cab2_phase1(C.byref(src), hw_ptr, C.byref(wt), g2_ptr, pool_ptr, sep, op, stream)
    return lib.sn_cab1_phase1(C.byref(src), C.byref(wt), g2_ptr, pool_ptr, sep, op, stream)


class ConvDesc(C.Structure):
    _fields_ = [
        ("inp", C.c_void_p * 3), ("n_in", C.c_int), ("cs_in", C.c_int),
        ("T", C.c_int), ("h_in", C.c_int), ("w_in", C.c_int), ("in_mode", C.c_int),
        ("k", C.c_int), ("stride", C.c_int), ("pad", C.c_int), ("h_out", C.c_int), ("w_out", C.c_int),
        ("wfrag", C.c_void_p), ("mt", C.c_int), ("ks", C.c_int), ("bias", C.c_void_p),
        ("act", C.c_int), ("prelu", C.c_float), ("res", C.c_void_p), ("out", C.c_void_p),
        ("cs_out", C.c_int), ("out_mode", C.c_int), ("c_out", C.c_int), ("nchw_dtype", C.c_int),
        ("sc", C.c_void_p), ("sc_dtype", C.c_int), ("pool", C.c_void_p), ("oscale", C.c_void_p), ("oscale_stride", C.c_int), ("res2", C.c_void_p),
        ("flags", C.c_int), ("clip_n", C.c_int), ("clip_T", C.c_int), ("clip_lo", C.c_int),
    ]


SN_CONV_TILE_KERNEL = 1

SN_CONV_K_GENERIC, SN_CONV_K_FAST, SN_CONV_K_STATS, SN_CONV_K_STREAM = 1, 2, 3, 4
CONV_KERNEL_NAMES = {SN_CONV_K_GENERIC: "conv_mfma", SN_CONV_K_FAST: "conv3_fast", SN_CONV_K_STATS: "conv3_fast_stats", SN_CONV_K_STREAM: "conv3p"}
CONV_PLAN_FIELDS = ("ntx", "nty", "S", "nseg", "nsg", "qs", "grid", "pool_rows")


def conv_route(kernel: int, mt: int, a: int, d: int = 0, mode: int = 0, rl: int = 0) -> int:
    return (kernel << 24) | (mt << 20) | (a << 12) | (d << 8) | (mode << 4) | rl


def conv_route_name(r: int) -> str:
    if r < 0:
        return f"EINVAL({r})"
    k, mt, a, d, mode, rl = r >> 24, (r >> 20) & 15, (r >> 12) & 255, (r >> 8) & 15, (r >> 4) & 15, r & 15
    name = CONV_KERNEL_NAMES.get(k, str(k))
    if k == SN_CONV_K_GENERIC:
        return f"{name}<{mt},{a},{4 * a}>"
    if k == SN_CONV_K_STREAM:
        return f"{name}<{mt},{a},D{d},MODE{mode},RL{rl}>"
    return f"{name}<{mt},{a}>"


class Conv32Desc(C.Structure):
    _fields_ = [
        ("inp", C.c_void_p * 3), ("c_in", C.c_int * 3), ("cs_in", C.c_int * 3), ("n_in", C.c_int),
        ("T", C.c_int), ("h_in", C.c_int), ("w_in", C.c_int), ("in_mode", C.c_int),
        ("k", C.c_int), ("stride", C.c_int), ("pad", C.c_int), ("groups", C.c_int),
        ("h_out", C.c_int), ("w_out", C.c_int), ("c_out", C.c_int),
        ("w", C.c_void_p), ("bias", C.c_void_p), ("act", C.c_int), ("prelu", C.c_float),
        ("oscale", C.c_void_p), ("oscale_stride", C.c_int), ("res", C.c_void_p), ("cs_res", C.c_int),
        ("out", C.c_void_p), ("cs_out", C.c_int), ("out_mode", C.c_int), ("nchw_dtype", C.c_int), ("sc", C.c_void_p),
        ("wsplit", C.c_void_p), ("iscale", C.c_void_p), ("iscale_stride", C.c_int), ("rscale", C.c_void_p), ("rscale_stride", C.c_int),
        ("ln_w", C.c_void_p), ("ln_b", C.c_void_p), ("csum", C.c_void_p), ("csum_cpad", C.c_int),
        ("clip_n", C.c_int), ("clip_T", C.c_int), ("clip_lo", C.c_int),
    ]


class UnitSrc(C.Structure):
    _fields_ = [("x", C.c_void_p), ("T", C.c_int), ("h", C.c_int), ("w", C.c_int), ("C", C.c_int),
                ("mode", C.c_int), ("wrap", C.c_int), ("halo", C.c_void_p), ("t0", C.c_int), ("nt", C.c_int),
                ("clip", C.c_int)]


SN_YUV_444, SN_YUV_420_CENTER, SN_YUV_420_LEFT = 0, 1, 2
SN_YUV_BT601, SN_YUV_BT709 = 0, 1
SN_YUV_LIMITED, SN_YUV_FULL = 0, 1


class YuvFmt(C.Structure):
    _fields_ = [("bits", C.c_int), ("chroma", C.c_int), ("matrix", C.c_int), ("range", C.c_int)]

    def frame_bytes(self, H: int, W: int) -> int:
        c = H * W if self.chroma == SN_YUV_444 else ((H + 1) // 2) * ((W + 1) // 2)
        return (H * W + 2 * c) * (1 if self.bits == 8 else 2)


class ShiftNetLibError(RuntimeError):
    pass


_lib: Optional[C.CDLL] = None


def load() -> C.CDLL:
    global _lib
    if _lib is not None:
        return _lib
    import torch
    if not os.path.exists(LIB_PATH):
        raise ShiftNetLibError(
            f"{LIB_PATH} not found: build it with `python shift-net_amd/build.py` (hipcc, gfx950). "
            "There is no CPU fallback for the Shift-Net HIP path.")
    lib = C.CDLL(LIB_PATH)
    missing = [s for s in SYMBOLS if not hasattr(lib, s)]
    if missing:
        raise ShiftNetLibError(f"{LIB_PATH} lacks symbols {missing}")
    vp, ci, cf = C.c_void_p, C.c_int, C.c_float
    lib.sn_abi_version.restype = ci
    lib.sn_selftest_mfma.argtypes = [vp, vp, vp, vp]
    lib.sn_ingest.argtypes = [vp, ci, vp, vp, ci, ci, ci, ci, vp]
    lib.sn_conv2d.argtypes = [C.POINTER(ConvDesc), vp]
    lib.sn_conv_pool_blocks.argtypes = [C.POINTER(ConvDesc)]
    lib.sn_conv2d_route.argtypes = [C.POINTER(ConvDesc), ci, ci, C.POINTER(ci * 8)]
    lib.sn_upsample2_add.argtypes = [vp, vp, vp, ci, ci, ci, ci, vp]
    lib.sn_ca_mlp.argtypes = [vp, ci, ci, ci, ci, cf, vp, vp, vp, ci, vp, vp]
    lib.sn_planar_pitch.argtypes = [ci]
    lib.sn_nhwc_to_planar.argtypes = [vp, vp, ci, ci, ci, ci, vp]
    lib.sn_dw5m_blocks.argtypes = [ci, ci]
    lib.sn_dw5m_gemm_gate.argtypes = [vp, vp, vp, vp, vp, vp, ci, ci, ci, ci, vp]
    lib.sn_cab_ca.argtypes = [vp, ci, ci, vp, ci, ci, ci, ci, ci, vp, vp, vp, vp, vp, ci, vp]
    lib.sn_cab_ca_scratch_floats.argtypes = [ci]
    lib.sn_cab_fused_supported.argtypes = [C.POINTER(ConvDesc), C.POINTER(ConvDesc)]
    lib.sn_cab_stats.argtypes = [C.POINTER(ConvDesc), ci, vp]
    lib.sn_cab_ca_lines.argtypes = [vp, ci, ci, vp, ci, ci, ci, ci, ci, ci, vp, vp, vp, vp, vp, ci, vp]
    lib.sn_cab_fused.argtypes = [C.POINTER(ConvDesc), C.POINTER(ConvDesc), ci, vp]
    lib.sn32_cab_ca.argtypes = [vp, ci, ci, vp, ci, ci, ci, ci, vp, vp, vp, vp, vp, ci, vp]
    lib.sn_gsts_gather.argtypes = [C.POINTER(UnitSrc), vp, vp, vp]
    lib.sn_temporal_roll.argtypes = [C.POINTER(UnitSrc), vp, vp]
    lib.sn_gsts_shiftconv.argtypes = [C.POINTER(UnitSrc), vp, vp, vp, vp]
    lib.sn_gsts_shiftconv_mfma.argtypes = [C.POINTER(UnitSrc), vp, vp, vp, vp]
    lib.sn_ln_gemm_gate.argtypes = [C.POINTER(UnitSrc), vp, vp, vp, vp, vp, vp, ci, vp]
    lib.sn_lngate_blocks.argtypes = [ci, ci]
    lib.sn_grp5_gemm_gate.argtypes = [vp, vp, vp, vp, vp, vp, ci, ci, ci, ci, vp]
    lib.sn_grp5_blocks.argtypes = [ci, ci]
    lib.sn_phase1_pool_blocks.argtypes = [ci, ci, ci]
    lib.sn_phase1_g1_store_bytes.argtypes = [ci, ci, ci, ci, C.POINTER(C.c_longlong)]
    lib.sn_p1r_plan.argtypes = [ci, ci, ci, ci, ci, C.POINTER(ci * 7)]
    lib.sn_p1r_strip_begin.argtypes = [C.POINTER(ci * 7), ci, ci]
    lib.sn_gsts_cab2_phase1.argtypes = [C.POINTER(UnitSrc), vp, C.POINTER(Phase1Weights), vp, vp, C.POINTER(SeFold), C.POINTER(Phase1Opts), vp]
    lib.sn_cab1_phase1.argtypes = [C.POINTER(UnitSrc), C.POINTER(Phase1Weights), vp, vp, C.POINTER(SeFold), C.POINTER(Phase1Opts), vp]
    lib.sn_gsts_cab2_phase2.argtypes = [C.POINTER(UnitSrc), vp, vp, vp, vp, vp, vp]
    lib.sn_cab1_phase2.argtypes = [C.POINTER(UnitSrc), vp, vp, vp, vp, vp, vp]
    lib.sn_cab2_phase2_cab1_phase1_supported.argtypes = [C.POINTER(UnitSrc)]
    lib.sn_cab2_phase2_cab1_phase1.argtypes = [C.POINTER(UnitSrc), vp, vp, vp, vp, vp, C.POINTER(Phase1Weights), vp, vp, C.POINTER(SeFold), C.POINTER(Phase1Opts), vp]
    lib.sn_ingest_u8.argtypes = [vp, vp, ci, ci, ci, ci, vp]
    lib.sn_egress_blocks.argtypes = []
    lib.sn_egress_u8.argtypes = [vp, ci, vp, vp, vp, ci, ci, ci, vp]
    lib.sn_ssim_blocks.argtypes = []
    lib.sn_ssim_u8.argtypes = [vp, ci, vp, vp, vp, ci, ci, ci, vp]
    lib.sn_ingest_yuv.argtypes = [vp, C.POINTER(YuvFmt), vp, ci, ci, ci, ci, ci, ci, vp]
    lib.sn_egress_yuv.argtypes = [vp, ci, C.POINTER(YuvFmt), vp, ci, ci, ci, ci, ci, vp]
    lib.sn_yuv_thumb.argtypes = [vp, C.POINTER(YuvFmt), vp, ci, ci, ci, vp]
    lib.sn_yuv_noise_hist.argtypes = [vp, C.POINTER(YuvFmt), vp, ci, ci, ci, ci, ci, vp]
    ll = C.c_longlong
    lib.sn32_conv2d.argtypes = [C.POINTER(Conv32Desc), vp]
    lib.sn32_conv2d_route.argtypes = [C.POINTER(Conv32Desc)]
    lib.sn32_gsts_gather.argtypes = [C.POINTER(UnitSrc), vp, vp, vp, vp]
    lib.sn32_layernorm.argtypes = [vp, ci, ci, vp, vp, vp, ci, ll, vp]
    lib.sn32_gate.argtypes = [vp, ci, ci, vp, ll, vp]
    lib.sn32_gate_sum.argtypes = [vp, ci, ci, ci, vp, ci, ci, ci, vp, vp]
    lib.sn32_dw_gate.argtypes = [vp, ci, vp, ci, ci, vp, ci, ci, ci, ci, vp, vp]
    lib.sn32_conv_csum_tiles.argtypes = [ci, ci]
    lib.sn32_gsts_shiftconv.argtypes = [vp, vp, vp, vp, vp, vp]
    lib.sn32_conv1x1_gate2.argtypes = [vp, ci, ci, vp, ci, ci, vp, ci, ci, vp, vp]
    lib.sn32_chan_sum.argtypes = [vp, ci, ci, ci, ci, ci, ci, vp, vp]
    lib.sn32_scale_residual.argtypes = [vp, vp, vp, ci, vp, ci, ci, ci, vp]
    lib.sn32_ingest.argtypes = [vp, ci, vp, vp, ci, ci, ci, ci, vp]
    for s in SYMBOLS:
        getattr(lib, s).restype = ci
    if lib.sn_abi_version() != ABI_VERSION:
        raise ShiftNetLibError(f"ABI version mismatch: {LIB_PATH} reports {lib.sn_abi_version()}, shiftnet_amd/lib.py expects {ABI_VERSION} "
                               "(stale build: run `python shift-net_amd/build.py`)")
    _lib = lib
    return lib


def check(rc: int, what: str) -> None:
    if rc != 0:
        raise ShiftNetLibError(f"{what} failed with code {rc}")
```

Before: 166.1 frames/s.

## Fold CAB channel-attention reduction into conv tail via last-arriving-block tickets

Adds a fold path where the conv3p streaming kernel (and the stats kernel) computes the CAB channel-attention gate in-kernel. Each block takes an atomic ticket and the last block to arrive for a frame reduces the pool and line partials, runs the folded 3x3 tap math and the MLP, and writes ca. This removes the separate sn_cab_ca launch and its scratch pass. In exchange it adds atomic loads and stores, a tail serialised on one block per frame, and ticket state that must be reset correctly. It is enabled by default through SN_CAB_CA_FOLD.

```diff
diff --git a/include/shiftnet_hip.h b/include/shiftnet_hip.h
--- a/include/shiftnet_hip.h
+++ b/include/shiftnet_hip.h
@@ -69,6 +69,18 @@
 int sn_cab_ca_lines(const float* partial, int nblk, int cpad, const void* lines, int lines_len, int cs, int c, int cr, int h, int w,
                     const float* w2, const float* wa, const float* wb, float* scratch, float* ca, int T, void* stream);
 int sn_cab_fused(const sn_conv_desc* conv1, const sn_conv_desc* conv2, int tile_rows, void* stream);
+
+typedef struct sn_cab_fold {
+    const float* w2; const float* wa; const float* wb;
+    float* ca;
+    unsigned* tickets;
+    void* lines; int lines_len;
+    int c, cr;
+} sn_cab_fold;
+int sn_cab_fold_supported(const sn_conv_desc* d, int lines_len);
+int sn_cab_fold_narrive(const int* plan, int t);
+int sn_conv2d_fold(const sn_conv_desc* d, const sn_cab_fold* f, void* stream);
+int sn_cab_stats_fold(const sn_conv_desc* conv1, int lines_len, const sn_cab_fold* f, void* stream);
 
 int sn32_cab_ca(const float* partial, int nblk, int cpad, const float* mid, int c, int cr, int h, int w,
                 const float* w2, const float* wa, const float* wb, float* scratch, float* ca, int T, void* stream);
diff --git a/shift-net_amd/csrc/sn_common.h b/shift-net_amd/csrc/sn_common.h
--- a/shift-net_amd/csrc/sn_common.h
+++ b/shift-net_amd/csrc/sn_common.h
@@ -160,6 +160,167 @@
         }
         S.ca[(size_t)t * cpad + tid] = o;
     }
+}
+
+__device__ __forceinline__ float sn_cabca_taps(const float* S, const float* wk, int cin, int cpad, float r) {
+    const float tot = S[cin], r0 = S[128 + cin], r1 = S[2 * 128 + cin], c0 = S[3 * 128 + cin], c1 = S[4 * 128 + cin];
+    const float k00 = S[5 * 128 + cin], k01 = S[6 * 128 + cin], k10 = S[7 * 128 + cin], k11 = S[8 * 128 + cin];
+    const float rowex[3] = {r1, 0.f, r0}, colex[3] = {c1, 0.f, c0};
+    const float cor[3][3] = {{k11, 0.f, k10}, {0.f, 0.f, 0.f}, {k01, 0.f, k00}};
+#pragma unroll
+    for (int ky = 0; ky < 3; ++ky)
+#pragma unroll
+        for (int kx = 0; kx < 3; ++kx) r += wk[(ky * 3 + kx) * cpad] * (tot - rowex[ky] - colex[kx] + cor[ky][kx]);
+    return r;
+}
+__device__ __forceinline__ float sn_cabca_hidden(const float* wa, const float* mean, int c, int row) {
+    float hh = 0.f;
+    for (int j = 0; j < c; ++j) hh += wa[row * c + j] * mean[j];
+    return hh > 0.f ? hh : 0.f;
+}
+__device__ __forceinline__ float sn_cabca_gate(const float* wb, const float* hid, int cr, int row) {
+    float o = 0.f;
+    for (int j = 0; j < cr; ++j) o += wb[row * cr + j] * hid[j];
+    return sigmoidf_(o);
+}
+
+#define SN_CABCA_NS 16
+struct CabFold { const float* w2; const float* wa; const float* wb; float* ca; unsigned* ticket; const bf16_t* lines; int lines_len, c, cr; };
+__host__ __device__ inline int sn_cabfold_narrive(int t, int fsegs, int qs) { return (t * fsegs + fsegs - 1) / qs - (t * fsegs) / qs + 1; }
+__host__ __device__ inline int sn_cabfold_lds_floats(int cpad, int cs) {
+    const int scr = SN_CABCA_NS * (cpad + 4 * cs);
+    return 16 + 9 * 128 + 2 * 128 + (scr > 1024 ? scr : 1024);
+}
+__device__ __forceinline__ void sn_cabfold_chains(const float* col, int i0, int nq, int step, int n, int stride, float (&sm)[4]) {
+#pragma unroll
+    for (int a = 0; a < 4; ++a) sm[a] = 0.f;
+    for (int b = i0; b < n; b += 8 * step) {
+        float v[4][8];
+#pragma unroll
+        for (int a = 0; a < 4; ++a)
+#pragma unroll
+            for (int j = 0; j < 8; ++j) {
+                const int k = b + a + j * step;
+                const bool ok = a < nq && k < n;
+                const float x = __hip_atomic_load(col + (size_t)(ok ? k : 0) * stride, __ATOMIC_RELAXED, __HIP_MEMORY_SCOPE_AGENT);
+                v[a][j] = ok ? x : 0.f;
+            }
+#pragma unroll
+        for (int a = 0; a < 4; ++a)
+#pragma unroll
+            for (int j = 0; j < 8; ++j) sm[a] += v[a][j];
+    }
+}
+__device__ __forceinline__ void sn_cabfold_chains(const bf16_t* col, int i0, int nq, int step, int n, int stride, float (&sm)[4][4]) {
+#pragma unroll
+    for (int a = 0; a < 4; ++a)
+#pragma unroll
+        for (int c = 0; c < 4; ++c) sm[a][c] = 0.f;
+    for (int b = i0; b < n; b += 6 * step) {
+        unsigned long long v[4][6];
+#pragma unroll
+        for (int a = 0; a < 4; ++a)
+#pragma unroll
+            for (int j = 0; j < 6; ++j) {
+                const int k = b + a + j * step;
+                const bool ok = a < nq && k < n;
+                const unsigned long long x = __hip_atomic_load((const unsigned long long*)(col + (size_t)(ok ? k : 0) * stride), __ATOMIC_RELAXED, __HIP_MEMORY_SCOPE_AGENT);
+                v[a][j] = ok ? x : 0ull;
+            }
+#pragma unroll
+        for (int a = 0; a < 4; ++a)
+#pragma unroll
+            for (int j = 0; j < 6; ++j) {
+                const uint32_t lo = (uint32_t)v[a][j], hi = (uint32_t)(v[a][j] >> 32);
+                sm[a][0] += bf_lo(lo); sm[a][1] += bf_hi(lo); sm[a][2] += bf_lo(hi); sm[a][3] += bf_hi(hi);
+            }
+    }
+}
+__device__ __forceinline__ void sn_cabfold_tail(const CabFold& F, const float* pool_t, int nblk, int narrive, int cpad, int cs, int h, int w, int t,
+                                                float* lds, int tid) {
+    asm volatile("s_waitcnt vmcnt(0)" ::: "memory");
+    __syncthreads();
+    unsigned* flag = (unsigned*)lds;
+    if (tid == 0) *flag = __hip_atomic_fetch_add(F.ticket + t, 1u, __ATOMIC_RELAXED, __HIP_MEMORY_SCOPE_AGENT) == (unsigned)(narrive - 1) ? 1u : 0u;
+    __syncthreads();
+    if (!*flag) return;
+    if (tid == 0) {
+        __builtin_amdgcn_fence(__ATOMIC_ACQUIRE, "agent");
+        __hip_atomic_store(F.ticket + t, 0u, __ATOMIC_RELAXED, __HIP_MEMORY_SCOPE_AGENT);
+    }
+    __syncthreads();
+    float* S = lds + 16; float* mean = S + 9 * 128; float* hid = mean + 128; float* scr = hid + 128; float* acc = scr;
+    const int SW = cpad + 4 * cs, L = F.lines_len;
+    const bf16_t* lt = F.lines + (size_t)t * 4 * L * cs;
+    if (tid < 256) {
+        const int nsplit = 256 / cpad;
+        for (int i = tid; i < SN_CABCA_NS * cpad; i += 256) {
+            const int s = i / cpad, ch = i - s * cpad;
+            float m = 0.f;
+            for (int q = 0; q < nsplit; q += 4) {
+                float sm[4];
+                sn_cabfold_chains(pool_t + ch, s * nsplit + q, nsplit - q, SN_CABCA_NS * nsplit, nblk, cpad, sm);
+#pragma unroll
+                for (int a = 0; a < 4; ++a) m += sm[a];
+            }
+            scr[s * SW + ch] = m;
+        }
+        const int nseg = 256 / cs, c4s = cs >> 2;
+        for (int i = tid; i < 4 * SN_CABCA_NS * c4s; i += 256) {
+            const int line = i / (SN_CABCA_NS * c4s), r = i - line * (SN_CABCA_NS * c4s), s = r / c4s, ch = (r - s * c4s) * 4;
+            float m[4] = {0.f, 0.f, 0.f, 0.f};
+            for (int q = 0; q < nseg; q += 4) {
+                float sm[4][4];
+                sn_cabfold_chains(lt + (size_t)line * L * cs + ch, s * nseg + q, nseg - q, SN_CABCA_NS * nseg, line < 2 ? w : h, cs, sm);
+#pragma unroll
+                for (int a = 0; a < 4; ++a)
+#pragma unroll
+                    for (int c = 0; c < 4; ++c) m[c] += sm[a][c];
+            }
+#pragma unroll
+            for (int c = 0; c < 4; ++c) scr[s * SW + cpad + line * cs + ch + c] = m[c];
+        }
+    }
+    __syncthreads();
+    if (tid < 256) {
+        for (int i = tid; i < 5 * 128; i += 256) {
+            const int k = i >> 7, ch = i & 127;
+            float m = 0.f;
+            if (ch < (k == 0 ? cpad : cs)) {
+                const float* sp = scr + (k == 0 ? 0 : cpad + (k - 1) * cs) + ch;
+                for (int q = 0; q < SN_CABCA_NS; ++q) m += sp[q * SW];
+            }
+            S[i] = m;
+        }
+        if (tid < cs) {
+            const bf16_t* lc = lt + tid;
+            S[5 * 128 + tid] = bf_to_f(__hip_atomic_load(lc, __ATOMIC_RELAXED, __HIP_MEMORY_SCOPE_AGENT));
+            S[6 * 128 + tid] = bf_to_f(__hip_atomic_load(lc + (size_t)(w - 1) * cs, __ATOMIC_RELAXED, __HIP_MEMORY_SCOPE_AGENT));
+            S[7 * 128 + tid] = bf_to_f(__hip_atomic_load(lc + (size_t)L * cs, __ATOMIC_RELAXED, __HIP_MEMORY_SCOPE_AGENT));
+            S[8 * 128 + tid] = bf_to_f(__hip_atomic_load(lc + ((size_t)L + w - 1) * cs, __ATOMIC_RELAXED, __HIP_MEMORY_SCOPE_AGENT));
+        }
+    }
+    __syncthreads();
+    const int nsplit2 = 1024 / cpad;
+    if (tid < 256) {
+        for (int v = tid; v < 1024; v += 256) {
+            const int co = v % cpad, part = v / cpad;
+            float r = 0.f;
+            if (part < nsplit2)
+                for (int cin = part; cin < F.c; cin += nsplit2) r = sn_cabca_taps(S, F.w2 + (size_t)cin * 9 * cpad + co, cin, cpad, r);
+            acc[v] = r;
+        }
+    }
+    __syncthreads();
+    if (tid < cpad) {
+        float m = 0.f;
+        for (int q = 0; q < nsplit2; ++q) m += acc[q * cpad + tid];
+        mean[tid] = m / ((float)h * (float)w);
+    }
+    __syncthreads();
+    if (tid < F.cr) hid[tid] = sn_cabca_hidden(F.wa, mean, F.c, tid);
+    __syncthreads();
+    if (tid < cpad) F.ca[(size_t)t * cpad + tid] = tid < F.c ? sn_cabca_gate(F.wb, hid, F.cr, tid) : 0.f;
 }
 
 __device__ __forceinline__ int wave_id() { return __builtin_amdgcn_readfirstlane((int)(threadIdx.x >> 6)); }
diff --git a/shift-net_amd/csrc/sn_conv.hip b/shift-net_amd/csrc/sn_conv.hip
--- a/shift-net_amd/csrc/sn_conv.hip
+++ b/shift-net_amd/csrc/sn_conv.hip
@@ -4,7 +4,8 @@
 int sn_conv3p_key(const sn_conv_desc* d, bool want_pool);
 int sn_conv3p_pool_rows(const sn_conv_desc* d);
 int sn_conv3p_route(const sn_conv_desc* d, int lines_len, int ncu, int* plan8);
-int sn_conv3p_launch(const sn_conv_desc* d, int lines_len, int route, const int* plan8, void* stream);
+int sn_conv3p_launch(const sn_conv_desc* d, int lines_len, int route, const int* plan8, const sn_cab_fold* f, void* stream);
+bool sn_conv3p_fold_ok(const sn_conv_desc* d, int lines_len, int route, const sn_cab_fold* f);
 
 namespace {
 
@@ -576,7 +577,6 @@
     }
 }
 
-#define SN_CABCA_NS 16
 __device__ __forceinline__ float cab_ldf(const bf16_t* p) { return bf_to_f(*p); }
 __device__ __forceinline__ float cab_ldf(const float* p) { return *p; }
 template <typename E>
@@ -655,17 +655,7 @@
         const int nsplit = 1024 / cpad, co = tid % cpad, part = tid / cpad;
         float r = 0.f;
         if (part < nsplit)
-            for (int cin = part; cin < c; cin += nsplit) {
-                const float tot = S[0][cin], r0 = S[1][cin], r1 = S[2][cin], c0 = S[3][cin], c1 = S[4][cin];
-                const float k00 = S[5][cin], k01 = S[6][cin], k10 = S[7][cin], k11 = S[8][cin];
-                const float* wk = w2 + (size_t)cin * 9 * cpad + co;
-                const float rowex[3] = {r1, 0.f, r0}, colex[3] = {c1, 0.f, c0};
-                const float cor[3][3] = {{k11, 0.f, k10}, {0.f, 0.f, 0.f}, {k01, 0.f, k00}};
-#pragma unroll
-                for (int ky = 0; ky < 3; ++ky)
-#pragma unroll
-                    for (int kx = 0; kx < 3; ++kx) r += wk[(ky * 3 + kx) * cpad] * (tot - rowex[ky] - colex[kx] + cor[ky][kx]);
-            }
+            for (int cin = part; cin < c; cin += nsplit) r = sn_cabca_taps(&S[0][0], w2 + (size_t)cin * 9 * cpad + co, cin, cpad, r);
         acc[tid] = r;
         __syncthreads();
         if (tid < cpad) {
@@ -675,20 +665,9 @@
         }
     }
     __syncthreads();
-    if (tid < cr) {
-        float hh = 0.f;
-        for (int j = 0; j < c; ++j) hh += wa[tid * c + j] * mean[j];
-        hid[tid] = hh > 0.f ? hh : 0.f;
-    }
+    if (tid < cr) hid[tid] = sn_cabca_hidden(wa, mean, c, tid);
     __syncthreads();
-    if (tid < cpad) {
-        float o = 0.f;
-        if (tid < c) {
-            for (int j = 0; j < cr; ++j) o += wb[tid * cr + j] * hid[j];
-            o = sigmoidf_(o);
-        }
-        ca[(size_t)t * cpad + tid] = o;
-    }
+    if (tid < cpad) ca[(size_t)t * cpad + tid] = tid < c ? sn_cabca_gate(wb, hid, cr, tid) : 0.f;
 }
 
 __global__ void selftest_mfma_kernel(const float* a, const float* b, float* d) {
@@ -823,11 +802,24 @@
     return conv_route(d, lines_len, ncu, plan);
 }
 
-int sn_conv2d(const sn_conv_desc* d, void* stream) {
+int sn_cab_fold_supported(const sn_conv_desc* d, int lines_len) {
+    sn_clear_error();
+    int plan8[8];
+    const int route = conv_route(d, lines_len, 0, plan8);
+    return route >= 0 && sn_conv3p_fold_ok(d, lines_len, route, nullptr) ? 1 : 0;
+}
+
+int sn_cab_fold_narrive(const int* plan8, int t) {
+    if (!plan8 || t < 0 || plan8[0] < 1 || plan8[3] < 1 || plan8[5] < 1 || (long)(t + 1) * plan8[0] * plan8[3] > plan8[4]) return SN_EINVAL;
+    return sn_cabfold_narrive(t, plan8[0] * plan8[3], plan8[5]);
+}
+
+static int conv2d_run(const sn_conv_desc* d, const sn_cab_fold* f, void* stream) {
     sn_clear_error();
     int plan8[8];
     const int route = conv_route(d, 0, 0, plan8);
     if (route < 0) return route;
+    if (f && !sn_conv3p_fold_ok(d, 0, route, f)) return SN_EINVAL;
     ConvK K;
     K.in0 = (const bf16_t*)d->in[0]; K.in1 = (const bf16_t*)d->in[1]; K.in2 = (const bf16_t*)d->in[2];
     K.n_in = d->n_in; K.cs = d->cs_in; K.cv = d->n_in * d->cs_in;
@@ -842,7 +834,7 @@
     hipStream_t st = (hipStream_t)stream;
     const int mt = (route >> 20) & 15, a = (route >> 12) & 255;
     switch (route >> 24) {
-        case SN_CONV_K_STREAM: return sn_conv3p_launch(d, 0, route, plan8, stream);
+        case SN_CONV_K_STREAM: return sn_conv3p_launch(d, 0, route, plan8, f, stream);
         case SN_CONV_K_FAST:
             switch (mt * 1000 + a) {
                 case 1016: return launch_conv3_fast<1, 16>(K, d->T, st);
@@ -858,6 +850,8 @@
     }
 }
 
+int sn_conv2d(const sn_conv_desc* d, void* stream) { return conv2d_run(d, nullptr, stream); }
+int sn_conv2d_fold(const sn_conv_desc* d, const sn_cab_fold* f, void* stream) { return f ? conv2d_run(d, f, stream) : SN_EINVAL; }
 
 int sn_ca_mlp(const float* partial, int nblk, int cpad, int c, int cr, float inv_hw,
               const float* wa, const float* wb, float* ca, int T, unsigned* bad, void* stream) {
@@ -892,13 +886,14 @@
     return cab_ca_launch(partial, nblk, cpad, lines, lines_len, cs, c, cr, h, w, w2, wa, wb, scratch, ca, T, stream);
 }
 
-int sn_cab_stats(const sn_conv_desc* d, int lines_len, void* stream) {
+static int cab_stats_run(const sn_conv_desc* d, int lines_len, const sn_cab_fold* f, void* stream) {
     sn_clear_error();
     if (lines_len < 1) return SN_EINVAL;
     int plan8[8];
     const int route = conv_route(d, lines_len, 0, plan8);
     if (route < 0) return route;
-    if ((route >> 24) == SN_CONV_K_STREAM) return sn_conv3p_launch(d, lines_len, route, plan8, stream);
+    if (f && !sn_conv3p_fold_ok(d, lines_len, route, f)) return SN_EINVAL;
+    if ((route >> 24) == SN_CONV_K_STREAM) return sn_conv3p_launch(d, lines_len, route, plan8, f, stream);
     const int key = ((route >> 20) & 15) * 1000 + ((route >> 12) & 255);
     ConvK K;
     K.in0 = (const bf16_t*)d->in[0]; K.in1 = K.in2 = nullptr;
@@ -912,6 +907,9 @@
     return key == 1016 ? launch_conv3_fast<1, 16, true>(K, d->T, st) : launch_conv3_fast<2, 24, true>(K, d->T, st);
 }
 
+int sn_cab_stats(const sn_conv_desc* d, int lines_len, void* stream) { return cab_stats_run(d, lines_len, nullptr, stream); }
+int sn_cab_stats_fold(const sn_conv_desc* d, int lines_len, const sn_cab_fold* f, void* stream) { return f ? cab_stats_run(d, lines_len, f, stream) : SN_EINVAL; }
+
 int sn32_cab_ca(const float* partial, int nblk, int cpad, const float* mid, int c, int cr, int h, int w,
                 const float* w2, const float* wa, const float* wb, float* scratch, float* ca, int T, void* stream) {
     sn_clear_error();
diff --git a/shift-net_amd/csrc/sn_conv3p.hip b/shift-net_amd/csrc/sn_conv3p.hip
--- a/shift-net_amd/csrc/sn_conv3p.hip
+++ b/shift-net_amd/csrc/sn_conv3p.hip
@@ -15,6 +15,8 @@
     int dbg;
     int lines_len;
     int S, nseg, nsg, qs;
+    bf16_t* lines;
+    CabFold fold;
 };
 
 __device__ __forceinline__ float max_bare(float a, float b) {
@@ -80,6 +82,17 @@
         for (int i = (int)threadIdx.x; i < MT * KS * 64; i += 320) *(uint4*)(smem + i * 16) = P.wfrag[i];
         __syncthreads();
     }
+    const int tfirst = t;
+    auto fold_tail = [&]() __attribute__((always_inline)) {
+        if constexpr (MODE == 1 || MODE == 3) {
+            if (P.fold.ticket) {
+                const int fsegs = P.ntx * P.nseg, tlast = (fseg + nsegs - 1) / fsegs;
+                for (int f = tfirst; f <= tlast; ++f)
+                    sn_cabfold_tail(P.fold, P.pool + (size_t)f * P.pool_rows * (16 * MT), P.pool_rows, sn_cabfold_narrive(f, fsegs, P.qs), 16 * MT, CS,
+                                    P.h, P.w, f, (float*)smem, (int)threadIdx.x);
+            }
+        }
+    };
 
     if (wv == 4) {
         int voff[NDMA], pxk[NDMA];
@@ -127,6 +140,7 @@
                 if (++fty == P.nty) { fty = 0; if (++ftx == P.ntx) { ftx = 0; ++ft; } }
             }
         }
+        fold_tail();
         return;
     }
 
@@ -224,7 +238,7 @@
 #pragma unroll
                 for (int r = 0; r < 4; ++r) {
                     const float sm = row_sum16(psum[m][r]);
-                    if (p == 0) dst[c0 + m * 4 + r] = sm;
+                    if (p == 0) sn_pool_store(dst + c0 + m * 4 + r, sm);
                     psum[m][r] = 0.f;
                 }
         }
@@ -266,10 +280,10 @@
 #pragma unroll
                     for (int r = 0; r < 4; ++r) psum[m][r] += (MASKED && !ok) ? 0.f : v[m][r];
             }
-            if constexpr (MODE == 3) {
-                if (MASKED && ok && c0 < CS) {
+            if constexpr (MODE == 1 || MODE == 3) {
+                if (MASKED && ok && c0 < CS && (MODE == 3 || P.lines)) {
                     const int oy = ty * TH + wv * RPW + rr, ox = tx * TW + xb * 16 + p;
-                    bf16_t* const lb = P.out + (size_t)t * 4 * P.lines_len * CS + c0;
+                    bf16_t* const lb = P.lines + (size_t)t * 4 * P.lines_len * CS + c0;
                     bf16_t* tgt[4] = {oy == 0 ? lb + (size_t)ox * CS : nullptr, oy == P.h - 1 ? lb + ((size_t)P.lines_len + ox) * CS : nullptr,
                                       ox == 0 ? lb + ((size_t)2 * P.lines_len + oy) * CS : nullptr, ox == P.w - 1 ? lb + ((size_t)3 * P.lines_len + oy) * CS : nullptr};
 #pragma unroll
@@ -277,10 +291,12 @@
                         if (!tgt[e]) continue;
 #pragma unroll
                         for (int m = 0; m < MT; ++m)
-                            if (c0 + m * 4 < CS) *(uint2*)(tgt[e] + m * 4) = make_uint2(pack_bf2(v[m][0], v[m][1]), pack_bf2(v[m][2], v[m][3]));
+                            if (c0 + m * 4 < CS)
+                                __hip_atomic_store((unsigned long long*)(tgt[e] + m * 4), (unsigned long long)pack_bf2(v[m][0], v[m][1]) | ((unsigned long long)pack_bf2(v[m][2], v[m][3]) << 32),
+                                                   __ATOMIC_RELAXED, __HIP_MEMORY_SCOPE_AGENT);
                     }
                 }
-                continue;
+                if constexpr (MODE == 3) continue;
             }
 #pragma unroll
             for (int q = 0; q < NP; ++q) {
@@ -348,7 +364,7 @@
                 __builtin_amdgcn_sched_barrier(0);
             }
             }
-            const bool plain = full && !(MODE == 3 && (ty == 0 || ty == P.nty - 1 || tx == 0 || tx == P.ntx - 1));
+            const bool plain = full && !((MODE == 3 || (MODE == 1 && P.lines)) && (ty == 0 || ty == P.nty - 1 || tx == 0 || tx == P.ntx - 1));
             if (plain) finish(acc, rres, xs, N0, ro, o2, false, 0, 0);
             else finish(acc, rres, xs, N0, ro, o2, true, P.h - oy0 - wv * RPW, P.w - ox0 - p);
         }
@@ -377,6 +393,7 @@
         tile(i, rA, rB);
         if (i + 1 < n) tile(i + 1, rB, rA);
     }
+    fold_tail();
 }
 
 template <int MT, int CS, int TH, int D, int WR>
@@ -818,18 +835,38 @@
     return SN_CONV_ROUTE(SN_CONV_K_STREAM, mt, cs, D, mode, rl ? 1 : 0);
 }
 
+bool sn_conv3p_fold_ok(const sn_conv_desc* d, int lines_len, int route, const sn_cab_fold* f) {
+    if ((route >> 24) != SN_CONV_K_STREAM) return false;
+    const int mt = (route >> 20) & 15, cs = (route >> 12) & 255, D = (route >> 8) & 15, mode = (route >> 4) & 15;
+    if (mode != (lines_len > 0 ? 3 : 1) || (d->flags & (7 << 12))) return false;
+    const int npb = cs / 8, ndma = (10 * 34 * npb + 63) / 64, ks = (9 * cs + 31) / 32;
+    const size_t lds = (size_t)(D + 1) * ndma * 1024 + (mt * ks > 16 ? mt * ks * 1024 : 0);
+    if ((size_t)sn_cabfold_lds_floats(16 * mt, cs) * 4 > lds || d->h_out < 2 || d->w_out < 2) return false;
+    if (!f) return true;
+    if (!f->w2 || !f->wa || !f->wb || !f->ca || !f->tickets || f->c < 1 || f->c > cs || f->c > 16 * mt || f->cr < 1 || f->cr > 128) return false;
+    if (lines_len == 0 && (!f->lines || f->lines_len < (d->h_out > d->w_out ? d->h_out : d->w_out))) return false;
+    return true;
+}
+
 template <int MT, int CS, int D>
 int launch_conv3p_rf(const C3P& K, const C3PPlan& pl, int mode, hipStream_t st) {
     return launch_conv3p<MT, CS, 8, D, D, false>(K, pl, mode, st);
 }
 
-int sn_conv3p_launch(const sn_conv_desc* d, int lines_len, int route, const int* plan8, void* stream) {
+int sn_conv3p_launch(const sn_conv_desc* d, int lines_len, int route, const int* plan8, const sn_cab_fold* f, void* stream) {
     if ((route >> 24) != SN_CONV_K_STREAM || !plan8) return SN_EINVAL;
+    if (f && !sn_conv3p_fold_ok(d, lines_len, route, f)) return SN_EINVAL;
     C3P K;
     K.in = (const bf16_t*)d->in[0]; K.res = (const bf16_t*)d->res; K.out = (bf16_t*)d->out;
     K.wfrag = (const uint4*)d->wfrag; K.bias = d->bias; K.oscale = d->oscale; K.oscale_stride = d->oscale_stride;
     K.pool = d->pool; K.pool_rows = 0; K.act = d->act; K.prelu = d->prelu;
     K.T = d->T; K.h = d->h_out; K.w = d->w_out; K.lines_len = lines_len; K.dbg = (d->flags >> 12) & 7;
+    K.lines = lines_len > 0 ? K.out : nullptr;
+    K.fold = CabFold{nullptr, nullptr, nullptr, nullptr, nullptr, nullptr, 0, 0, 0};
+    if (f) {
+        if (lines_len == 0) { K.lines = (bf16_t*)f->lines; K.lines_len = f->lines_len; }
+        K.fold = CabFold{f->w2, f->wa, f->wb, f->ca, f->tickets, K.lines, K.lines_len, f->c, f->cr};
+    }
     const C3PPlan pl = {plan8[0], plan8[1], plan8[2], plan8[3], plan8[4], plan8[5], plan8[6], plan8[7]};
     hipStream_t st = (hipStream_t)stream;
     const int mt = (route >> 20) & 15, cs = (route >> 12) & 255, D = (route >> 8) & 15, mode = (route >> 4) & 15;
@@ -856,6 +893,7 @@
     K.wfrag = (const uint4*)a->wfrag; K.bias = a->bias; K.w2 = (const uint4*)b->wfrag; K.b2 = b->bias;
     K.oscale = b->oscale; K.oscale_stride = b->oscale_stride; K.pool = nullptr; K.pool_rows = 0; K.act = 1; K.prelu = a->prelu;
     K.T = a->T; K.h = a->h_out; K.w = a->w_out; K.lines_len = 0; K.dbg = 0;
+    K.lines = nullptr; K.fold = CabFold{nullptr, nullptr, nullptr, nullptr, nullptr, nullptr, 0, 0, 0};
     const int o = (a->flags >> 4) & 15;
     const bool shallow = ((a->flags >> 10) & 3) == 3;
     const C3PPlan pl = c3p_plan(a->T, a->h_out, a->w_out, 8, ncu, o ? o : (key == 1016 ? (shallow ? 3 : 2) : 1), c3p_segment(a->h_out, a->w_out, 8, c3p_wgs_default(key)));
diff --git a/shift-net_amd/shiftnet_amd/engine.py b/shift-net_amd/shiftnet_amd/engine.py
--- a/shift-net_amd/shiftnet_amd/engine.py
+++ b/shift-net_amd/shiftnet_amd/engine.py
@@ -199,6 +199,7 @@
         self._side = None
         self._tickets = None
         self._old_tickets: List[torch.Tensor] = []
+        self._cab_tickets = None
         self._clip = 0
         self._bad = None
         self.fallbacks = 0
@@ -214,8 +215,12 @@
     def _stream(self) -> int:
         return torch.cuda.current_stream(self.dev).cuda_stream
 
+    _entry: Optional[str] = None
+    _last_ca: Optional[torch.Tensor] = None
+
     def _call(self, fn: str, label: str, *args) -> None:
-        f = getattr(self.lib, fn)
+        f = getattr(self.lib, self._entry or fn)
+        self._entry = None
         if self.prof is None:
             L.check(f(*args), label)
             return
@@ -247,7 +252,7 @@
     def conv(self, name: str, ins: Sequence[Act], *, stride: int = 1, pad: Optional[int] = None, prelu: Optional[float] = None,
              res: Optional[Act] = None, out_mode: int = 0, pool: bool = False, in_mode: int = 0, oscale: Optional[torch.Tensor] = None,
              nchw_out: Optional[torch.Tensor] = None, nchw_sc: Optional[torch.Tensor] = None, res2: Optional[Act] = None,
-             remap: Optional[Tuple[int, int, int]] = None):
+             remap: Optional[Tuple[int, int, int]] = None, fold: Optional[Dict[str, object]] = None):
         p = self.P.convs[name]
         k, cout = int(p["k"]), int(p["cout"])
         T, hs, ws, cs_in = ins[0].dims
@@ -298,10 +303,36 @@
             pool_buf = torch.empty((T, nblk, 16 * d.mt), dtype=torch.float32, device=self.dev)
             d.pool = pool_buf.data_ptr()
         self._meta = ("conv", T, h_out, w_out, len(ins) * cs_in, int(d.cs_out), k, stride, in_mode, out_mode)
+        if fold is not None:
+            assert pool and out_mode == 0
+            ca = None
+            if self._cab_fold_ok(T) and self.lib.sn_cab_fold_supported(C.byref(d), 0):
+                ll = max(h_out, w_out)
+                lines = torch.empty((T, 4, ll, int(d.cs_out)), dtype=self.act_dtype, device=self.dev)
+                ca = torch.empty((T, 16 * d.mt), dtype=torch.float32, device=self.dev)
+                f = L.CabFold(fold["w2"].data_ptr(), fold["wa"].data_ptr(), fold["wb"].data_ptr(), ca.data_ptr(), self._cab_ticket_ptr(T),
+                              lines.data_ptr(), ll, fold["c"], fold["cr"])
+                self._entry = "sn_conv2d_fold"
+                self._call("sn_conv2d", f"sn_conv2d[{name}]", C.byref(d), C.byref(f), self._stream())
+            else:
+                self._call("sn_conv2d", f"sn_conv2d[{name}]", C.byref(d), self._stream())
+            return out_act, pool_buf, h_out * w_out, ca
         self._call("sn_conv2d", f"sn_conv2d[{name}]", C.byref(d), self._stream())
         if pool:
             return out_act, pool_buf, h_out * w_out
         return out_act
+
+    cab_ca_fold = os.environ.get("SN_CAB_CA_FOLD", "1") != "0"
+
+    def _cab_fold_ok(self, T: int) -> bool:
+        return self.cab_ca_fold and T <= self.MAX_TICKETS
+
+    def _cab_ticket_ptr(self, T: int) -> int:
+        if self._cab_tickets is None or self._cab_tickets.numel() < T:
+            if self._cab_tickets is not None:
+                self._old_tickets.append(self._cab_tickets)
+            self._cab_tickets = torch.zeros((max(self.MAX_TICKETS, T),), dtype=torch.int32, device=self.dev)
+        return self._cab_tickets.data_ptr()
 
     def ca_mlp(self, name: str, pool: torch.Tensor, npix: int) -> torch.Tensor:
         p = self.P.cas[name]
@@ -330,12 +361,14 @@
                 out = self._cab_fused(pre, x, extra, slope)
                 if out is not None:
                     return out
-            scratch = torch.empty((self.lib.sn_cab_ca_scratch_floats(T),), dtype=torch.float32, device=self.dev)
-            mid, pool, _ = self.conv(pre + "body.0", [x], prelu=slope, pool=True)
-            _, nblk, cpad = pool.shape
-            ca = torch.empty((T, cpad), dtype=torch.float32, device=self.dev)
-            self._call("sn_cab_ca", f"sn_cab_ca[{pre}]", pool.data_ptr(), nblk, cpad, mid.t.data_ptr(), cs, p["c"], p["cr"], h, w,
-                       p["w2"].data_ptr(), p["wa"].data_ptr(), p["wb"].data_ptr(), scratch.data_ptr(), ca.data_ptr(), T, self._stream())
+            mid, pool, _, ca = self.conv(pre + "body.0", [x], prelu=slope, pool=True, fold=p)
+            if ca is None:
+                _, nblk, cpad = pool.shape
+                scratch = torch.empty((self.lib.sn_cab_ca_scratch_floats(T),), dtype=torch.float32, device=self.dev)
+                ca = torch.empty((T, cpad), dtype=torch.float32, device=self.dev)
+                self._call("sn_cab_ca", f"sn_cab_ca[{pre}]", pool.data_ptr(), nblk, cpad, mid.t.data_ptr(), cs, p["c"], p["cr"], h, w,
+                           p["w2"].data_ptr(), p["wa"].data_ptr(), p["wb"].data_ptr(), scratch.data_ptr(), ca.data_ptr(), T, self._stream())
+            self._last_ca = ca
             return self.conv(pre + "body.2", [mid], res=x, oscale=ca, res2=extra)
         r = self.conv(pre + "body.0", [x], prelu=self.P.scalar(pre + "body.1.weight"))
         r, pool, npix = self.conv(pre + "body.2", [r], pool=True)
@@ -379,7 +412,6 @@
         lines = torch.empty((T, 4, ll, cs), dtype=self.act_dtype, device=self.dev)
         nblk = lib.sn_conv_pool_blocks(C.byref(d1))
         pool = torch.empty((T, nblk, 16 * d1.mt), dtype=torch.float32, device=self.dev)
-        scratch = torch.empty((lib.sn_cab_ca_scratch_floats(T),), dtype=torch.float32, device=self.dev)
         ca = torch.empty((T, 16 * d1.mt), dtype=torch.float32, device=self.dev)
         out = self._new(T, h, w, cs)
         d1.out, d1.pool = lines.data_ptr(), pool.data_ptr()
@@ -390,10 +422,17 @@
         rows = 0 if self.cab_fused[0] == "p" else 16 if self.cab_fused.endswith("16") else 8
         st = self._stream()
         self._meta = ("cabf", T, h, w, cs, 1)
-        self._call("sn_cab_stats", f"sn_cab_stats[{pre}]", C.byref(d1), ll, st)
-        self._meta = ()
-        self._call("sn_cab_ca_lines", f"sn_cab_ca[{pre}]", pool.data_ptr(), nblk, 16 * d1.mt, lines.data_ptr(), ll, cs, p["c"], p["cr"], h, w,
-                   p["w2"].data_ptr(), p["wa"].data_ptr(), p["wb"].data_ptr(), scratch.data_ptr(), ca.data_ptr(), T, st)
+        if self._cab_fold_ok(T) and lib.sn_cab_fold_supported(C.byref(d1), ll):
+            f = L.CabFold(p["w2"].data_ptr(), p["wa"].data_ptr(), p["wb"].data_ptr(), ca.data_ptr(), self._cab_ticket_ptr(T), None, 0, p["c"], p["cr"])
+            self._entry = "sn_cab_stats_fold"
+            self._call("sn_cab_stats", f"sn_cab_stats[{pre}]", C.byref(d1), ll, C.byref(f), st)
+        else:
+            scratch = torch.empty((lib.sn_cab_ca_scratch_floats(T),), dtype=torch.float32, device=self.dev)
+            self._call("sn_cab_stats", f"sn_cab_stats[{pre}]", C.byref(d1), ll, st)
+            self._meta = ()
+            self._call("sn_cab_ca_lines", f"sn_cab_ca[{pre}]", pool.data_ptr(), nblk, 16 * d1.mt, lines.data_ptr(), ll, cs, p["c"], p["cr"], h, w,
+                       p["w2"].data_ptr(), p["wa"].data_ptr(), p["wb"].data_ptr(), scratch.data_ptr(), ca.data_ptr(), T, st)
+        self._last_ca = ca
         self._meta = ("cabf", T, h, w, cs, 3 if extra is not None else 2)
         self._call("sn_cab_fused", f"sn_cab_fused[{pre}]", C.byref(d1), C.byref(d2), rows, st)
         return Act(out, x.c)
diff --git a/shift-net_amd/shiftnet_amd/lib.py b/shift-net_amd/shiftnet_amd/lib.py
--- a/shift-net_amd/shiftnet_amd/lib.py
+++ b/shift-net_amd/shiftnet_amd/lib.py
@@ -20,7 +20,9 @@
     "sn32_conv2d", "sn32_conv2d_route", "sn32_gsts_gather", "sn32_layernorm", "sn32_gate", "sn32_gate_sum", "sn32_chan_sum", "sn32_scale_residual", "sn32_ingest", "sn32_cab_ca", "sn32_dw_gate", "sn32_conv1x1_gate2", "sn32_gsts_shiftconv", "sn32_conv_csum_tiles",
     "sn_ln_gemm_gate", "sn_lngate_blocks", "sn_grp5_gemm_gate", "sn_grp5_blocks", "sn_gsts_cab2_phase1", "sn_cab1_phase1", "sn_phase1_pool_blocks", "sn_phase1_g1_store_bytes", "sn_p1r_plan", "sn_p1r_strip_begin",
     "sn_cab2_phase2_cab1_phase1", "sn_cab2_phase2_cab1_phase1_supported",
+    "sn_cab_fold_supported", "sn_cab_fold_narrive", "sn_conv2d_fold", "sn_cab_stats_fold",
 ]
+FOLD_SYMBOLS = ["sn_cab_fold_supported", "sn_cab_fold_narrive", "sn_conv2d_fold", "sn_cab_stats_fold"]
 
 
 class Phase1Weights(C.Structure):
@@ -29,6 +31,11 @@
 
 class SeFold(C.Structure):
     _fields_ = [("wa", C.c_void_p), ("wb", C.c_void_p), ("c", C.c_int), ("cr", C.c_int), ("ticket", C.c_void_p), ("ca", C.c_void_p), ("bad", C.c_void_p)]
+
+
+class CabFold(C.Structure):
+    _fields_ = [("w2", C.c_void_p), ("wa", C.c_void_p), ("wb", C.c_void_p), ("ca", C.c_void_p), ("tickets", C.c_void_p),
+                ("lines", C.c_void_p), ("lines_len", C.c_int), ("c", C.c_int), ("cr", C.c_int)]
 
 
 class Phase1Opts(C.Structure):
@@ -130,7 +137,9 @@
             f"{LIB_PATH} not found: build it with `python shift-net_amd/build.py` (hipcc, gfx950). "
             "There is no CPU fallback for the Shift-Net HIP path.")
     lib = C.CDLL(LIB_PATH)
-    missing = [s for s in SYMBOLS if not hasattr(lib, s)]
+    fold = [s for s in FOLD_SYMBOLS if hasattr(lib, s)]
+    need_fold = os.environ.get("SN_CAB_CA_FOLD", "1") != "0"
+    missing = [s for s in SYMBOLS if not hasattr(lib, s) and (need_fold or fold or s not in FOLD_SYMBOLS)]
     if missing:
         raise ShiftNetLibError(f"{LIB_PATH} lacks symbols {missing}")
     vp, ci, cf = C.c_void_p, C.c_int, C.c_float
@@ -194,8 +203,14 @@
     lib.sn32_chan_sum.argtypes = [vp, ci, ci, ci, ci, ci, ci, vp, vp]
     lib.sn32_scale_residual.argtypes = [vp, vp, vp, ci, vp, ci, ci, ci, vp]
     lib.sn32_ingest.argtypes = [vp, ci, vp, vp, ci, ci, ci, ci, vp]
+    if fold:
+        lib.sn_cab_fold_supported.argtypes = [C.POINTER(ConvDesc), ci]
+        lib.sn_cab_fold_narrive.argtypes = [C.POINTER(ci * 8), ci]
+        lib.sn_conv2d_fold.argtypes = [C.POINTER(ConvDesc), C.POINTER(CabFold), vp]
+        lib.sn_cab_stats_fold.argtypes = [C.POINTER(ConvDesc), ci, C.POINTER(CabFold), vp]
     for s in SYMBOLS:
-        getattr(lib, s).restype = ci
+        if hasattr(lib, s):
+            getattr(lib, s).restype = ci
     if lib.sn_abi_version() != ABI_VERSION:
         raise ShiftNetLibError(f"ABI version mismatch: {LIB_PATH} reports {lib.sn_abi_version()}, shiftnet_amd/lib.py expects {ABI_VERSION} "
                                "(stale build: run `python shift-net_amd/build.py`)")
```

Measured after the change: 147.9 frames/s. 0.89x the previous value.
